# SelennLamson/AntsRL

Hardware: AMD Instinct MI355X
Metric: ant-steps/sec (ants x envs x steps/s), 256^2 grid (higher is better)
Workload: dtype f64 ant kinematics / f32 grids

## Files before the change

### antsrl_amd/_lib.py

```python
from __future__ import annotations

import ctypes as C
import os

from .config import AntsCfg, AntsGen, AntsInit

LIB_PATH = os.environ.get("ANTSRL_LIB") or os.path.join(os.path.dirname(os.path.abspath(__file__)), "lib",
                                                        "libantsrl_hip.so")

EXPORTS = ("antsrl_abi_version", "antsrl_cfg_size", "antsrl_last_error", "antsrl_workspace_bytes", "antsrl_create",
           "antsrl_destroy", "antsrl_reset", "antsrl_generate", "antsrl_step", "antsrl_observe", "antsrl_update", "antsrl_flush",
           "antsrl_step_update", "antsrl_set_timing_events", "antsrl_set_activation", "antsrl_policy_mlp", "antsrl_read_state", "antsrl_state_bytes",
           "antsrl_set_obs_format", "antsrl_query", "antsrl_bench_copy", "antsrl_set_inloop_policy", "antsrl_set_obs_row_stride", "antsrl_mem_alloc", "antsrl_mem_free",
           "antsrl_mem_trim", "antsrl_mem_stats", "antsrl_update_phase",
           "antsrl_perceptive_field", "antsrl_memnet_packed_bytes", "antsrl_memnet_pack", "antsrl_policy_memory",
           "antsrl_memtrain_sizes", "antsrl_memtrain_init", "antsrl_memtrain_unpack", "antsrl_memtrain_copy",
           "antsrl_memtrain_grad", "antsrl_memtrain_apply", "antsrl_memnet_packed_bytes_ex", "antsrl_memnet_pack_ex",
           "antsrl_policy_memory_ex", "antsrl_agent_select", "antsrl_replay_record_pre", "antsrl_replay_record_post",
           "antsrl_policy_memory_tiles", "antsrl_agent_plan", "antsrl_agent_select_actions",
           "antsrl_replay_record_pre_plain", "antsrl_replay_record_post_plain", "antsrl_lintrain_sizes",
           "antsrl_lintrain_grad", "antsrl_lintrain_apply", "antsrl_lintrain_step", "antsrl_exptrain_sizes",
           "antsrl_exptrain_grad", "antsrl_exptrain_apply", "antsrl_exptrain_step", "antsrl_rework_collapsed_bytes",
           "antsrl_rework_collapse", "antsrl_policy_rework", "antsrl_reworktrain_sizes", "antsrl_reworktrain_grad",
           "antsrl_reworktrain_apply", "antsrl_reworktrain_step", "antsrl_policy_rework_select")

_lib = None


class AntsMemNetShape(C.Structure):
    _fields_ = [(n, C.c_int32) for n in ("n_features", "agent_dim", "mem_size", "h1", "h2", "h3", "n_rot", "n_ph")]


class AntsReworkShape(C.Structure):
    _fields_ = [(n, C.c_int32) for n in ("n_features", "agent_dim", "g1", "g2", "g3", "r1", "r2", "r3", "p1", "n_rot", "n_ph")]


class AntsRecordSpec(C.Structure):
    _fields_ = [(n, C.c_int32) for n in ("n_envs", "n_ants", "env_id_base", "n_features", "agent_dim", "mem_size", "n_rot",
                                         "obs_format", "obs_pitch", "reserved")] + [
        (n, C.c_int64) for n in ("K", "head", "max_len")] + [(n, C.c_uint64) for n in ("seed", "step")]


class AntsrlError(RuntimeError):
    pass


def load() -> C.CDLL:
    global _lib
    if _lib is not None:
        return _lib
    if not os.path.exists(LIB_PATH):
        raise AntsrlError(
            "libantsrl_hip.so is missing (%s): build it with `python -m antsrl_amd.build` "
            "(hipcc, gfx950).  There is no CPU fallback." % LIB_PATH)
    import torch
    lib = C.CDLL(LIB_PATH)
    vp, i32 = C.c_void_p, C.c_int
    lib.antsrl_abi_version.restype = i32
    lib.antsrl_last_error.restype = C.c_char_p
    lib.antsrl_workspace_bytes.argtypes = [C.POINTER(AntsCfg), C.POINTER(C.c_size_t)]
    lib.antsrl_create.argtypes = [C.POINTER(AntsCfg), vp, C.c_size_t, C.POINTER(vp)]
    lib.antsrl_destroy.argtypes = [vp]
    lib.antsrl_destroy.restype = None
    lib.antsrl_reset.argtypes = [vp, C.POINTER(AntsInit), vp]
    lib.antsrl_generate.argtypes = [vp, C.POINTER(AntsGen), C.c_uint64, vp]
    lib.antsrl_step.argtypes = [vp, vp, vp, vp, vp, vp, vp, vp]
    lib.antsrl_observe.argtypes = [vp, vp, vp, vp, vp]
    lib.antsrl_update.argtypes = [vp, vp, vp]
    lib.antsrl_flush.argtypes = [vp, vp]
    lib.antsrl_update_phase.argtypes = [vp, i32, vp, vp]
    lib.antsrl_perceptive_field.argtypes = [vp, vp, vp]
    lib.antsrl_step_update.argtypes = [vp, vp, vp, vp, vp, vp, vp, vp, vp]
    lib.antsrl_set_timing_events.argtypes = [vp, C.POINTER(vp)]
    lib.antsrl_set_activation.argtypes = [vp, vp, C.c_double, vp]
    lib.antsrl_policy_mlp.argtypes = [vp, vp, vp, C.c_int64, C.c_int32, vp, vp, vp, vp, vp, vp, vp, vp, vp, vp]
    lib.antsrl_read_state.argtypes = [vp, i32, vp, vp]
    lib.antsrl_state_bytes.argtypes = [vp, i32, C.POINTER(C.c_size_t)]
    lib.antsrl_query.argtypes = [vp, i32, C.POINTER(C.c_longlong)]
    lib.antsrl_set_inloop_policy.argtypes = [vp, i32] + [vp] * 9
    lib.antsrl_bench_copy.argtypes = [vp, vp, C.c_size_t, vp]
    lib.antsrl_set_obs_row_stride.argtypes = [vp, i32]
    lib.antsrl_mem_alloc.argtypes = [C.c_size_t, i32, C.POINTER(vp)]
    lib.antsrl_mem_free.argtypes = [vp]
    lib.antsrl_mem_trim.argtypes = []
    lib.antsrl_mem_stats.argtypes = [C.POINTER(C.c_size_t)] * 4
    lib.antsrl_memnet_packed_bytes.argtypes = [C.POINTER(AntsMemNetShape), C.POINTER(C.c_size_t)]
    lib.antsrl_memnet_pack.argtypes = [C.POINTER(AntsMemNetShape), C.POINTER(vp), vp, vp]
    lib.antsrl_policy_memory.argtypes = [C.POINTER(AntsMemNetShape), vp, vp, i32, vp, vp, C.c_int64, vp, vp, vp, vp, vp]
    lib.antsrl_memnet_packed_bytes_ex.argtypes = [C.POINTER(AntsMemNetShape), i32, C.POINTER(C.c_size_t)]
    lib.antsrl_memnet_pack_ex.argtypes = [C.POINTER(AntsMemNetShape), i32, C.POINTER(vp), vp, vp]
    lib.antsrl_policy_memory_ex.argtypes = [C.POINTER(AntsMemNetShape), i32, vp, vp, i32, vp, vp, C.c_int64, vp, vp, vp,
                                            vp, vp]
    lib.antsrl_policy_memory_tiles.argtypes = [C.POINTER(AntsMemNetShape), i32, vp, vp, i32, vp, vp, C.c_int64, vp, vp, vp,
                                               vp, vp, vp, vp]
    sz = C.POINTER(C.c_size_t)
    lib.antsrl_memtrain_sizes.argtypes = [C.POINTER(AntsMemNetShape), C.c_int64, sz, sz, sz, sz]
    lib.antsrl_memtrain_init.argtypes = [C.POINTER(AntsMemNetShape), C.POINTER(vp), vp, vp]
    lib.antsrl_memtrain_unpack.argtypes = [C.POINTER(AntsMemNetShape), vp, C.POINTER(vp), vp]
    lib.antsrl_memtrain_copy.argtypes = [C.POINTER(AntsMemNetShape), vp, vp, vp]
    lib.antsrl_memtrain_grad.argtypes = [C.POINTER(AntsMemNetShape), vp, vp, vp, vp, vp, vp, vp, vp, vp, vp, C.c_int64,
                                         C.c_float, vp, vp, vp, vp]
    lib.antsrl_memtrain_apply.argtypes = [C.POINTER(AntsMemNetShape), vp, vp, C.c_int64, C.c_double, C.c_double,
                                          C.c_double, C.c_double, vp]
    lib.antsrl_agent_select.argtypes = [C.c_uint64, C.c_uint64, i32, i32, i32, C.c_double, i32, i32, i32, vp, vp, vp, vp,
                                        vp, vp]
    lib.antsrl_agent_plan.argtypes = [C.c_uint64, C.c_uint64, i32, i32, i32, C.c_double, vp, vp, vp]
    lib.antsrl_replay_record_pre.argtypes = [C.POINTER(AntsRecordSpec)] + [vp] * 9
    lib.antsrl_replay_record_post.argtypes = [C.POINTER(AntsRecordSpec)] + [vp] * 10
    lib.antsrl_agent_select_actions.argtypes = [C.c_uint64, C.c_uint64, i32, i32, i32, C.c_double, i32, i32, vp, vp, vp, vp]
    lib.antsrl_replay_record_pre_plain.argtypes = [C.POINTER(AntsRecordSpec)] + [vp] * 8
    lib.antsrl_replay_record_post_plain.argtypes = [C.POINTER(AntsRecordSpec)] + [vp] * 9
    lib.antsrl_lintrain_sizes.argtypes = [i32, C.c_int64, sz, sz, C.POINTER(C.c_int32)]
    lib.antsrl_lintrain_grad.argtypes = [i32] + [vp] * 11 + [C.c_int64, vp, C.c_int64, C.c_float, vp, vp, vp, vp]
    lib.antsrl_lintrain_apply.argtypes = [vp, vp, vp, vp, C.c_int64, C.c_double, C.c_double, C.c_double, C.c_double, vp]
    lib.antsrl_lintrain_step.argtypes = [i32] + [vp] * 13 + [C.c_int64, vp, C.c_int64, C.c_float, C.c_int64, C.c_double,
                                                             C.c_double, C.c_double, C.c_double, vp, vp, vp, vp]
    lib.antsrl_exptrain_sizes.argtypes = [i32, C.c_int64, sz, sz, C.POINTER(C.c_int32)]
    lib.antsrl_exptrain_grad.argtypes = [i32] + [vp] * 9 + [C.c_int64, vp, C.c_int64, C.c_float, vp, vp, vp, vp]
    lib.antsrl_exptrain_apply.argtypes = [i32, vp, vp, vp, vp, C.c_int64, C.c_double, C.c_double, C.c_double, C.c_double, vp]
    lib.antsrl_exptrain_step.argtypes = [i32] + [vp] * 11 + [C.c_int64, vp, C.c_int64, C.c_float, C.c_int64, C.c_double,
                                                             C.c_double, C.c_double, C.c_double, vp, vp, vp, vp]
    lib.antsrl_rework_collapsed_bytes.argtypes = [C.POINTER(AntsReworkShape), sz]
    lib.antsrl_rework_collapse.argtypes = [C.POINTER(AntsReworkShape), C.POINTER(vp), vp, vp]
    lib.antsrl_policy_rework.argtypes = [C.POINTER(AntsReworkShape), vp, vp, i32, vp, C.c_int64, vp, vp, vp, vp]
    rs = C.POINTER(AntsReworkShape)
    lib.antsrl_policy_rework_select.argtypes = [rs, vp, vp, i32, vp, C.c_uint64, C.c_uint64, i32, i32, i32, C.c_double, vp, vp,
                                                vp, vp, vp]
    lib.antsrl_reworktrain_sizes.argtypes = [rs, C.c_int64, sz, sz, C.POINTER(C.c_int32)]
    lib.antsrl_reworktrain_grad.argtypes = [rs] + [vp] * 9 + [C.c_int64, vp, C.c_int64, C.c_float, vp, vp, vp, vp]
    lib.antsrl_reworktrain_apply.argtypes = [rs, vp, vp, vp, vp, C.c_int64, C.c_double, C.c_double, C.c_double, C.c_double, vp]
    lib.antsrl_reworktrain_step.argtypes = [rs] + [vp] * 11 + [C.c_int64, vp, C.c_int64, C.c_float, C.c_int64, C.c_double,
                                                               C.c_double, C.c_double, C.c_double, vp, vp, vp, vp]
    for name in EXPORTS:
        getattr(lib, name)
    lib.antsrl_cfg_size.restype = C.c_size_t
    from .config import ABI_VERSION
    if lib.antsrl_abi_version() != ABI_VERSION:
        raise AntsrlError("ABI version mismatch: library %d, binding %d" % (lib.antsrl_abi_version(), ABI_VERSION))
    if lib.antsrl_cfg_size() != C.sizeof(AntsCfg):
        raise AntsrlError("AntsCfg layout mismatch: library %d bytes, binding %d" % (
            lib.antsrl_cfg_size(), C.sizeof(AntsCfg)))
    _lib = lib
    return lib


def hip_runtime() -> C.CDLL:
    load()
    for line in open("/proc/self/maps"):
        path = line.split()[-1]
        if "libamdhip64" in path:
            return C.CDLL(path)
    raise AntsrlError("no libamdhip64 mapped in this process")


def check(rc: int, what: str = "antsrl") -> None:
    if rc != 0:
        msg = load().antsrl_last_error().decode("utf-8", "replace")
        raise AntsrlError("%s failed (%d): %s" % (what, rc, msg))


def ptr(t):
    return None if t is None else C.c_void_p(t.data_ptr())


def stream(device):
    import torch
    return C.c_void_p(torch.cuda.current_stream(device).cuda_stream)


class HipEvents:

    def __init__(self, n):
        self.hip = hip_runtime()
        self.ev = []
        for _ in range(n):
            e = C.c_void_p()
            rc = self.hip.hipEventCreate(C.byref(e))
            assert rc == 0, "hipEventCreate failed: %d" % rc
            self.ev.append(e)

    def elapsed_ms(self, a, b):
        ms = C.c_float()
        rc = self.hip.hipEventElapsedTime(C.byref(ms), self.ev[a], self.ev[b])
        assert rc == 0, "hipEventElapsedTime failed: %d" % rc
        return ms.value

    def destroy(self):
        for e in self.ev:
            self.hip.hipEventDestroy(e)
```

### antsrl_amd/batched.py

```python
from __future__ import annotations

import ctypes as C
from typing import Dict, Optional

import numpy as np
import torch

from . import _lib
from . import config as cfgmod
from . import vmm
from .config import AntsCfg, AntsInit

_STATE_DTYPES = {
    cfgmod.S_ANTS_XYT: torch.float64, cfgmod.S_PREV_XY: torch.float64, cfgmod.S_HOLDING: torch.float32,
    cfgmod.S_MANDIBLES: torch.uint8, cfgmod.S_ACTIVATION: torch.float32, cfgmod.S_PHERO: torch.float32,
    cfgmod.S_FOOD: torch.float32, cfgmod.S_EXPLORED: torch.uint8, cfgmod.S_ANTHILL_FOOD: torch.float64,
    cfgmod.S_ROCK_CENTERS: torch.float64, cfgmod.S_TIMESTEP: torch.int32, cfgmod.S_REWARD_STATE: torch.uint8,
    cfgmod.S_WALLS: torch.uint8, cfgmod.S_ANTHILL_AREA: torch.uint8, cfgmod.S_SEED: torch.float32,
    cfgmod.S_ANTHILL_XYR: torch.int32, cfgmod.S_ROCK_RW: torch.float64,
    cfgmod.S_PHERO_C0: torch.float32, cfgmod.S_PHERO_C1: torch.float32, cfgmod.S_PHERO_C2: torch.float32,
    cfgmod.S_PHERO_C3: torch.float32,
}


import contextlib

_NULL_CTX = contextlib.nullcontext()
_RAW_STREAM = getattr(torch._C, "_cuda_getCurrentRawStream", None)


def _ptr(t: Optional[torch.Tensor]):
    return None if t is None else C.c_void_p(t.data_ptr())


def placement_levels_seen(times) -> bool:
    ok = [t for t in times if t < 1.25 * min(times)]
    return max(ok) >= 1.06 * min(ok)


class BatchedAntsEnv:
    def __init__(self, cfg: AntsCfg, device: Optional[torch.device] = None, obs_dtype: torch.dtype = torch.float32,
                 obs_row_stride=None, pieced_memory: bool = True):
        if obs_dtype not in (torch.float32, torch.bfloat16):
            raise ValueError("obs_dtype must be torch.float32 or torch.bfloat16")
        if not torch.cuda.is_available():
            raise _lib.AntsrlError("BatchedAntsEnv needs an MI355X (torch.cuda.is_available() is False); "
                                   "there is no CPU fallback")
        self.lib = _lib.load()
        self.cfg = cfg.copy()
        self.device = torch.device(device if device is not None else "cuda:%d" % torch.cuda.current_device())
        self._dev_index = self.device.index if self.device.index is not None else torch.cuda.current_device()
        need = C.c_size_t()
        _lib.check(self.lib.antsrl_workspace_bytes(C.byref(self.cfg), C.byref(need)), "workspace_bytes")
        self.workspace_bytes = need.value
        with torch.cuda.device(self.device):
            big = (lambda n: vmm.empty_u8(n, self.device)) if pieced_memory else (lambda n: torch.empty(n, dtype=torch.uint8, device=self.device))
            self._pieced = bool(pieced_memory)
            self._h = None
            self._make_handle(torch.empty(need.value + 256, dtype=torch.uint8, device=self.device))
            E, N, P, K = cfg.n_envs, cfg.n_ants, cfg.pside, cfg.n_channels
            esz = 4 if obs_dtype == torch.float32 else 2
            row = P * P * K
            if obs_row_stride not in (None, "line"):
                raise ValueError("obs_row_stride must be None or 'line'")
            pitch = row if obs_row_stride is None else (row * esz + 127) // 128 * 128 // esz
            sizes = [("agent_state", E * N * 2 * 4), ("reward", E * N * 4), ("done", E), ("obs", E * N * pitch * esz)]
            offs, total = {}, 0
            for name, nbytes in sizes:
                offs[name] = total
                total += (nbytes + 255) // 256 * 256
            self._out_sizes, self._out_offs, self._out_total, self._small_bytes = sizes, offs, total, offs["obs"]
            self._obs_dtype, self._obs_pitch_row = obs_dtype, (pitch, row)
            if obs_dtype == torch.bfloat16:
                _lib.check(self.lib.antsrl_set_obs_format(self._h, 1), "set_obs_format")
            if pitch != row:
                _lib.check(self.lib.antsrl_set_obs_row_stride(self._h, pitch), "set_obs_row_stride")
            self.obs_row_pitch = pitch
            self._bind_outputs(big(total + 256).zero_())
        self._keep = None
        self._loaded = None
        self._host_out = None
        self._host_act = None
        self._act_event = None

    def __del__(self):
        h = getattr(self, "_h", None)
        if h:
            self.lib.antsrl_destroy(h)
            self._h = None

    def _bind_outputs(self, flat: torch.Tensor) -> None:
        c = self.cfg
        E, N, P, K = c.n_envs, c.n_ants, c.pside, c.n_channels
        sizes, offs, total = self._out_sizes, self._out_offs, self._out_total
        pitch, row = self._obs_pitch_row
        base = (-flat.data_ptr()) % 256
        self._out_flat = flat[base:base + total]

        def piece(name, nbytes, dtype, shape):
            return self._out_flat[offs[name]:offs[name] + nbytes].view(dtype).view(shape)
        if pitch == row:
            self.obs = piece("obs", sizes[3][1], self._obs_dtype, (E, N, P, P, K))
            self.obs_padded = None
        else:
            self.obs_padded = piece("obs", sizes[3][1], self._obs_dtype, (E, N, pitch))
            self.obs = self.obs_padded[..., :row].unflatten(-1, (P, P, K))
        self.agent_state = piece("agent_state", sizes[0][1], torch.float32, (E, N, 2))
        self.reward = piece("reward", sizes[1][1], torch.float32, (E, N))
        self.done = piece("done", sizes[2][1], torch.uint8, (E,))
        self._host_out = None

    def _make_handle(self, ws: torch.Tensor) -> None:
        if getattr(self, "_h", None):
            self.lib.antsrl_destroy(self._h)
        self._ws = ws
        self._ws_ptr = ws.data_ptr() + (-ws.data_ptr()) % 256
        self._h = C.c_void_p()
        _lib.check(self.lib.antsrl_create(C.byref(self.cfg), C.c_void_p(self._ws_ptr), self.workspace_bytes, C.byref(self._h)), "create")
        if getattr(self, "_obs_dtype", torch.float32) == torch.bfloat16:
            _lib.check(self.lib.antsrl_set_obs_format(self._h, 1), "set_obs_format")
        pitch, row = getattr(self, "_obs_pitch_row", (0, 0))
        if pitch != row:
            _lib.check(self.lib.antsrl_set_obs_row_stride(self._h, pitch), "set_obs_row_stride")

    def tune_placement(self, age: int = 150, steps: int = 30, verbose: bool = False, extra_outputs: int = 4,
                       walk_spacers: int = 3, spacer_gib: float = 24.0, force_walk: bool = False):
        if self._out_total < vmm.SMALL_BYTES:
            return None
        if self._loaded:
            raise _lib.AntsrlError("tune_placement() must run right after construction: this handle has already been %s" % self._loaded)
        c = self.cfg
        E, N = c.n_envs, c.n_ants
        dev = self.device

        def torch_u8(n):
            return torch.empty(n, dtype=torch.uint8, device=dev)
        with torch.cuda.device(dev):
            g = torch.Generator(device=dev)
            g.manual_seed(7)
            rot = torch.randint(-1, 2, (4, E, N), generator=g, device=dev, dtype=torch.int8)
            ph = torch.randint(0, 3, (4, E, N), generator=g, device=dev, dtype=torch.int8) if c.n_phero == 2 else [None] * 4
            e0, e1 = torch.cuda.Event(enable_timing=True), torch.cuda.Event(enable_timing=True)

            def scratch_episode():
                self.generate(cfgmod.make_gen(), episode_seed=0x7A11)
                for t in range(age):
                    self.step_update(rot[t % 4], ph[t % 4], None)

            NEV, PSTEPS = cfgmod.TIMING_EVENTS, 8
            evs = _lib.HipEvents(NEV * PSTEPS)
            prc_times = []

            def measure():
                for t in range(4):
                    self.step_update(rot[t % 4], ph[t % 4], None)
                e0.record()
                for t in range(steps):
                    self.step_update(rot[t % 4], ph[t % 4], None)
                e1.record()
                for t in range(PSTEPS):
                    self.set_timing_events([evs.ev[NEV * t + i].value for i in range(NEV)])
                    self.step_update(rot[t % 4], ph[t % 4], None)
                torch.cuda.current_stream(dev).synchronize()
                prc_times.append(float(np.mean([evs.elapsed_ms(NEV * t + 2, NEV * t + 3) for t in range(PSTEPS)])))
                return e0.elapsed_time(e1) / steps
            own_ws, own_out = self._ws, self._out_flat
            n_ws, n_out = self.workspace_bytes + 256, self._out_total + 256
            pairs, times = [], []
            for ws_kind in ("own", "other"):
                if ws_kind == "other":
                    self._make_handle(vmm.empty_u8(n_ws, dev))
                scratch_episode()
                for out_kind in ("own", "other"):
                    if out_kind == "other":
                        self._bind_outputs((torch_u8(n_out) if self._pieced else vmm.empty_u8(n_out, dev)).zero_())
                    elif ws_kind == "other":
                        self._bind_outputs(own_out)
                    pairs.append((self._ws, self._out_flat))
                    times.append(measure())
            labels = ["ws torch / out %s" % ("pieced" if self._pieced else "torch"),
                      "ws torch / out %s" % ("torch" if self._pieced else "pieced"),
                      "ws pieced / out %s" % ("pieced" if self._pieced else "torch"),
                      "ws pieced / out %s" % ("torch" if self._pieced else "pieced")]
            if extra_outputs > 0 and self._pieced:
                self._make_handle(own_ws)
                scratch_episode()
                for k in range(int(extra_outputs)):
                    self._bind_outputs(vmm.empty_u8(n_out, dev).zero_())
                    pairs.append((self._ws, self._out_flat))
                    times.append(measure())
                    labels.append("ws torch / out pieced (draw %d)" % (k + 2))
            spacers = []
            walked = 0
            both_levels = placement_levels_seen
            while self._pieced and walked < int(walk_spacers) and (force_walk or not both_levels(prc_times)):
                free_b = torch.cuda.mem_get_info(dev)[0]
                want = int(min(spacer_gib * 2 ** 30, free_b / 5))
                if want < (4 << 30):
                    break
                try:
                    spacers.append(torch_u8(want))
                    spacers.append(vmm.empty_u8(want, dev))
                except (RuntimeError, _lib.AntsrlError):
                    break
                walked += 1
                depth = sum(x.numel() for x in spacers) / 2 ** 30
                if self._ws.data_ptr() != own_ws.data_ptr():
                    self._make_handle(own_ws)
                scratch_episode()
                for kind, mk in (("pieced", lambda: vmm.empty_u8(n_out, dev)), ("torch", lambda: torch_u8(n_out))):
                    self._bind_outputs(mk().zero_())
                    pairs.append((self._ws, self._out_flat))
                    times.append(measure())
                    labels.append("ws torch / out %s (walk %d: +%.0f GiB)" % (kind, walked, depth))
                self._make_handle(torch_u8(n_ws))
                scratch_episode()
                self._bind_outputs(own_out)
                pairs.append((self._ws, self._out_flat))
                times.append(measure())
                labels.append("ws torch (walk %d: +%.0f GiB) / out %s" % (walked, depth, "pieced" if self._pieced else "torch"))
            best = min(range(len(times)), key=prc_times.__getitem__)
            evs.destroy()
            if verbose:
                print("tune_placement: ms/step per (workspace, outputs) pair %s -> %d" % (["%.4f" % t for t in times], best))
            ws, out = pairs[best]
            del pairs, spacers
            if ws.data_ptr() != self._ws.data_ptr():
                self._make_handle(ws)
            self._bind_outputs(out)
            if walked:
                vmm.trim()
            torch.cuda.empty_cache()
            self._out_flat.zero_()
            del own_ws, own_out, ws, out
        self.placement_trials = dict(ms_per_step=[round(t, 5) for t in times], observation_kernel_ms=[round(t, 5) for t in prc_times],
                                     chosen=best, pairs=labels, both_levels_seen=bool(both_levels(prc_times)), walk_steps=walked)
        self._loaded = None
        return times

    @property
    def _obs_buf(self):
        return self.obs if self.obs_padded is None else self.obs_padded

    def _stream(self):
        if _RAW_STREAM is not None:
            return C.c_void_p(_RAW_STREAM(self._dev_index))
        return C.c_void_p(torch.cuda.current_stream(self.device).cuda_stream)

    def _on_device(self):
        return _NULL_CTX if torch.cuda.current_device() == self._dev_index else torch.cuda.device(self.device)

    def _dev(self, a, dtype, shape=None):
        if a is None:
            return None
        t = torch.as_tensor(np.ascontiguousarray(a) if isinstance(a, np.ndarray) else a)
        t = t.to(device=self.device, dtype=dtype).contiguous()
        if shape is not None:
            assert tuple(t.shape) == tuple(shape), "expected shape %s, got %s" % (shape, tuple(t.shape))
        return t

    def reset(self, init: Dict[str, object]) -> None:
        c = self.cfg
        E, N, W, H, Cn, R = c.n_envs, c.n_ants, c.w, c.h, c.n_phero, c.n_rocks
        t = dict(
            ants_xyt=self._dev(init["ants_xyt"], torch.float64, (E, N, 3)),
            seed=self._dev(init["seed"], torch.float64, (E, N)),
            walls=self._dev(init["walls"], torch.uint8, (E, W, H)),
            food=self._dev(init["food"], torch.float32, (E, W, H)),
            anthill_xyr=self._dev(init["anthill_xyr"], torch.int32, (E, 3)),
            rocks=self._dev(init.get("rocks"), torch.float64, (E, R, 4)) if R > 0 else None,
            phero=self._dev(init.get("phero"), torch.float32, (E, Cn, W, H)),
        )
        ai = AntsInit(*[None if t[k] is None else t[k].data_ptr()
                        for k in ("ants_xyt", "seed", "walls", "food", "anthill_xyr", "rocks", "phero")])
        with torch.cuda.device(self.device):
            _lib.check(self.lib.antsrl_reset(self._h, C.byref(ai), self._stream()), "reset")
        self._loaded = "reset"
        self._keep = t

    def generate(self, gen=None, episode_seed: int = 0, walls=None) -> None:
        g = gen if gen is not None else cfgmod.make_gen()
        if walls is not None:
            c = self.cfg
            self._gen_walls = self._dev(np.asarray(walls).astype(np.uint8) if not torch.is_tensor(walls) else walls,
                                        torch.uint8, (c.n_envs, c.w, c.h))
            g.walls_input = self._gen_walls.data_ptr()
        with torch.cuda.device(self.device):
            _lib.check(self.lib.antsrl_generate(self._h, C.byref(g), int(episode_seed), self._stream()), "generate")
        self._loaded = "given an episode (generate)"

    def _actions(self, rotation, phero):
        c = self.cfg
        if isinstance(rotation, np.ndarray) and isinstance(phero, np.ndarray):
            n = c.n_envs * c.n_ants
            if self._host_act is None:
                self._host_act = torch.empty((2, c.n_envs, c.n_ants), dtype=torch.int8, pin_memory=True)
                self._dev_act = torch.empty((2, c.n_envs, c.n_ants), dtype=torch.int8, device=self.device)
                self._act_event = torch.cuda.Event()
            else:
                self._act_event.synchronize()
            assert rotation.size == n and phero.size == n, "expected %d actions per array" % n
            h = self._host_act.numpy()
            h[0] = self._integral(rotation, "rotation").reshape(c.n_envs, c.n_ants)
            h[1] = self._integral(phero, "pheromone").reshape(c.n_envs, c.n_ants)
            with torch.cuda.device(self.device):
                self._dev_act.copy_(self._host_act, non_blocking=True)
                self._act_event.record()
            return self._dev_act[0], self._dev_act[1]
        rot = self._dev(self._integral(rotation, "rotation"), torch.int8, (c.n_envs, c.n_ants))
        ph = self._dev(self._integral(phero, "pheromone"), torch.int8, (c.n_envs, c.n_ants))
        return rot, ph

    validate_actions = True

    def _integral(self, a, what):
        if a is None:
            return None
        if torch.is_tensor(a):
            if a.dtype == torch.int8 or a.numel() == 0:
                return a
            if self.validate_actions:
                fl = a.is_floating_point()
                frac = (a != a.round()).any() if fl else torch.zeros((), dtype=torch.bool, device=a.device)
                lo, hi, bad = torch.stack([a.min().to(torch.float64), a.max().to(torch.float64), frac.to(torch.float64)]).tolist()
                if bad:
                    raise ValueError("%s actions must be whole numbers (the kernels take them as int8)" % what)
                if lo < -128 or hi > 127:
                    raise ValueError("%s actions out of the int8 range" % what)
            return a.to(torch.int8) if a.is_floating_point() else a
        arr = np.asarray(a)
        if arr.dtype.kind == "f":
            if not np.array_equal(arr, np.rint(arr)):
                raise ValueError("%s actions must be whole numbers (the kernels take them as int8)" % what)
            arr = arr.astype(np.int64)
        if arr.size and (arr.min() < -128 or arr.max() > 127):
            raise ValueError("%s actions out of the int8 range" % what)
        return arr

    def outputs_to_host(self, want_obs: bool = True):
        if self.obs.dtype != torch.float32 and want_obs:
            raise _lib.AntsrlError("outputs_to_host: bfloat16 observations have no numpy dtype; use the device tensors")
        base, o = self._out_flat.data_ptr(), self._out_offs
        if any(t.data_ptr() != base + o[k] for k, t in (("obs", self._obs_buf), ("agent_state", self.agent_state),
                                                         ("reward", self.reward), ("done", self.done))):
            return (self.obs.cpu().numpy() if want_obs else None, self.agent_state.cpu().numpy(),
                    self.reward.cpu().numpy(), self.done.cpu().numpy())
        if self._host_out is None:
            self._host_out = torch.empty((self._out_flat.numel(),), dtype=torch.uint8, pin_memory=True)
        n = self._out_flat.numel() if want_obs else self._small_bytes
        with torch.cuda.device(self.device):
            self._host_out[:n].copy_(self._out_flat[:n], non_blocking=True)
            torch.cuda.current_stream(self.device).synchronize()
        hb, o = self._host_out.numpy(), self._out_offs

        def piece(name, t):
            nb = t.numel() * t.element_size()
            return hb[o[name]:o[name] + nb].view(np.float32 if t.dtype == torch.float32 else np.uint8).reshape(tuple(t.shape)).copy()
        obs_h = None
        if want_obs:
            obs_h = piece("obs", self._obs_buf)
            if self.obs_padded is not None:
                c = self.cfg
                obs_h = np.ascontiguousarray(obs_h[..., :c.pside * c.pside * c.n_channels]).reshape(tuple(self.obs.shape))
        return (obs_h, piece("agent_state", self.agent_state),
                piece("reward", self.reward), piece("done", self.done))

    def step(self, rotation, phero, want_obs: bool = True):
        rot, ph = self._actions(rotation, phero)
        with self._on_device():
            _lib.check(self.lib.antsrl_step(self._h, _ptr(rot), _ptr(ph), _ptr(self._obs_buf if want_obs else None),
                                            _ptr(self.agent_state), _ptr(self.reward), _ptr(self.done),
                                            self._stream()), "step")
        return self.obs, self.agent_state, self.reward, self.done

    def observe(self, want_obs: bool = True):
        with self._on_device():
            _lib.check(self.lib.antsrl_observe(self._h, _ptr(self._obs_buf if want_obs else None),
                                               _ptr(self.agent_state), _ptr(self.reward), self._stream()),
                       "observe")
        return self.obs, self.agent_state, self.reward

    def update(self, wall_jitter=None) -> None:
        c = self.cfg
        j = self._dev(wall_jitter, torch.float64, (c.n_envs, c.n_ants))
        with self._on_device():
            _lib.check(self.lib.antsrl_update(self._h, _ptr(j), self._stream()), "update")

    def update_phase(self, phase: int, wall_jitter=None) -> None:
        c = self.cfg
        j = self._dev(wall_jitter, torch.float64, (c.n_envs, c.n_ants)) if phase == cfgmod.PHASE_WALLS else None
        with self._on_device():
            _lib.check(self.lib.antsrl_update_phase(self._h, int(phase), _ptr(j), self._stream()), "update_phase")

    def flush(self) -> None:
        with self._on_device():
            _lib.check(self.lib.antsrl_flush(self._h, self._stream()), "flush")

    def step_update(self, rotation, phero, wall_jitter=None, want_obs: bool = True):
        c = self.cfg
        rot, ph = self._actions(rotation, phero)
        j = self._dev(wall_jitter, torch.float64, (c.n_envs, c.n_ants))
        with self._on_device():
            _lib.check(self.lib.antsrl_step_update(self._h, _ptr(rot), _ptr(ph), _ptr(j),
                                                   _ptr(self._obs_buf if want_obs else None), _ptr(self.agent_state),
                                                   _ptr(self.reward), _ptr(self.done), self._stream()),
                       "step_update")
        return self.obs, self.agent_state, self.reward, self.done

    def set_timing_events(self, events) -> None:
        if events is None:
            _lib.check(self.lib.antsrl_set_timing_events(self._h, None), "set_timing_events")
        else:
            n = cfgmod.TIMING_EVENTS
            assert len(events) == n, "antsrl_set_timing_events takes %d events" % n
            arr = (C.c_void_p * n)(*[C.c_void_p(int(e)) for e in events])
            _lib.check(self.lib.antsrl_set_timing_events(self._h, arr), "set_timing_events")

    def query(self, what: int) -> int:
        v = C.c_longlong()
        _lib.check(self.lib.antsrl_query(self._h, int(what), C.byref(v)), "query")
        return int(v.value)

    def set_activation(self, act, new_deposit_strength: float = 0.0) -> None:
        c = self.cfg
        a = self._dev(act, torch.float32, (c.n_envs, c.n_ants, c.n_phero))
        with torch.cuda.device(self.device):
            _lib.check(self.lib.antsrl_set_activation(self._h, _ptr(a), float(new_deposit_strength),
                                                      self._stream()), "set_activation")
        self._loaded = "given an activation matrix"

    def perceptive_field(self) -> torch.Tensor:
        c = self.cfg
        out = torch.empty((c.n_envs, c.w, c.h), dtype=torch.uint8, device=self.device)
        with self._on_device():
            _lib.check(self.lib.antsrl_perceptive_field(self._h, _ptr(out), self._stream()), "perceptive_field")
        return out.to(torch.bool)

    def read_state(self, which: int) -> torch.Tensor:
        c = self.cfg
        E, N, W, H, Cn, R = c.n_envs, c.n_ants, c.w, c.h, c.n_phero, c.n_rocks
        shapes = {
            cfgmod.S_ANTS_XYT: (E, N, 3), cfgmod.S_PREV_XY: (E, N, 2), cfgmod.S_HOLDING: (E, N),
            cfgmod.S_MANDIBLES: (E, N), cfgmod.S_ACTIVATION: (E, N, Cn), cfgmod.S_PHERO: (E, Cn, W, H),
            cfgmod.S_FOOD: (E, W, H), cfgmod.S_EXPLORED: (E, W, H), cfgmod.S_ANTHILL_FOOD: (E,),
            cfgmod.S_ROCK_CENTERS: (E, R, 2), cfgmod.S_TIMESTEP: (E,), cfgmod.S_REWARD_STATE: (E, N),
            cfgmod.S_WALLS: (E, W, H), cfgmod.S_ANTHILL_AREA: (E, W, H), cfgmod.S_SEED: (E, N),
            cfgmod.S_ANTHILL_XYR: (E, 3), cfgmod.S_ROCK_RW: (E, R, 2),
            cfgmod.S_PHERO_C0: (E, W, H), cfgmod.S_PHERO_C1: (E, W, H), cfgmod.S_PHERO_C2: (E, W, H),
            cfgmod.S_PHERO_C3: (E, W, H),
        }
        if cfgmod.S_PHERO_C0 <= which <= cfgmod.S_PHERO_C3 and which - cfgmod.S_PHERO_C0 >= Cn:
            raise _lib.AntsrlError("pheromone channel %d of %d" % (which - cfgmod.S_PHERO_C0, Cn))
        out = torch.empty(shapes[which], dtype=_STATE_DTYPES[which], device=self.device)
        if out.numel():
            with torch.cuda.device(self.device):
                _lib.check(self.lib.antsrl_read_state(self._h, which, _ptr(out), self._stream()), "read_state")
        return out
```

### antsrl_amd/config.py

```python
from __future__ import annotations

import ctypes as C
import math
from typing import Optional, Sequence

import numpy as np

ABI_VERSION = 5
MAX_CHANNELS = 16
MAX_PSIDE = 15
MAX_PCELLS = MAX_PSIDE * MAX_PSIDE
MAX_FILTER_RADIUS = 3
MAX_FILTER_TAPS = 49
MAX_PHERO = 4

CH_ANTS, CH_PHERO, CH_ANTHILL, CH_WALLS, CH_FOOD, CH_ROCKS = range(6)
REWARD_NONE, REWARD_EXPLORATION, REWARD_FOOD, REWARD_ALL = range(4)
PHERO_AUTO, PHERO_EXPLICIT_SWEEP = 0, 1
ACT_AUTO, ACT_CELL_META, ACT_SINGLE_KERNEL = 0, 1, 2
TIMING_EVENTS = 5
Q_CELL_META, Q_SCALED_UNITS, Q_INTERLEAVED, Q_FILTER_SEPARABLE, Q_PERCEIVE_RUN, Q_TIMESTEP, Q_DEFERRED_UPDATE = range(7)

(S_ANTS_XYT, S_PREV_XY, S_HOLDING, S_MANDIBLES, S_ACTIVATION, S_PHERO, S_FOOD, S_EXPLORED,
 S_ANTHILL_FOOD, S_ROCK_CENTERS, S_TIMESTEP, S_REWARD_STATE, S_WALLS, S_ANTHILL_AREA,
 S_SEED, S_ANTHILL_XYR, S_ROCK_RW, S_PHERO_C0, S_PHERO_C1, S_PHERO_C2, S_PHERO_C3) = range(21)


class AntsCfg(C.Structure):
    _fields_ = [
        ("abi_version", C.c_int32),
        ("n_envs", C.c_int32),
        ("n_ants", C.c_int32),
        ("w", C.c_int32),
        ("h", C.c_int32),
        ("n_phero", C.c_int32),
        ("n_rocks", C.c_int32),
        ("max_time", C.c_int32),
        ("perception_radius", C.c_int32),
        ("n_channels", C.c_int32),
        ("channel_kind", C.c_int32 * MAX_CHANNELS),
        ("channel_arg", C.c_int32 * MAX_CHANNELS),
        ("has_mask", C.c_int32),
        ("mask", C.c_uint8 * MAX_PCELLS),
        ("_pad0", C.c_uint8 * 7),
        ("delta", C.c_double),
        ("fwd_delta", C.c_double),
        ("max_speed", C.c_double),
        ("max_rot_speed", C.c_double),
        ("carry_speed_reduction", C.c_double),
        ("backward_speed_reduction", C.c_double),
        ("max_hold", C.c_double),
        ("has_max_val", C.c_int32),
        ("filter_radius", C.c_int32),
        ("phero_max_val", C.c_double),
        ("deposit_strength", C.c_double),
        ("phero_threshold", C.c_double),
        ("filter", C.c_double * MAX_FILTER_TAPS),
        ("reward_kind", C.c_int32),
        ("phero_mode", C.c_int32),
        ("reward_threshold", C.c_double),
        ("fct_explore", C.c_double),
        ("fct_food", C.c_double),
        ("fct_anthill", C.c_double),
        ("fct_explore_holding", C.c_double),
        ("fct_headinganthill", C.c_double),
        ("rng_seed", C.c_uint64),
        ("act_path", C.c_int32),
        ("env_id_base", C.c_int32),
        ("n_envs_total", C.c_int32),
        ("_pad1", C.c_int32),
    ]

    @property
    def pside(self) -> int:
        return 2 * self.perception_radius + 1

    def copy(self) -> "AntsCfg":
        out = AntsCfg()
        C.memmove(C.byref(out), C.byref(self), C.sizeof(AntsCfg))
        return out

    def obs_shape(self):
        p = self.pside
        return (self.n_envs, self.n_ants, p, p, self.n_channels)


class AntsGen(C.Structure):
    _fields_ = [("wall_density", C.c_double), ("n_food_discs", C.c_int32), ("food_rmin", C.c_int32),
                ("food_rmax", C.c_int32), ("auto_reset", C.c_int32), ("wall_kind", C.c_int32),
                ("perlin_octaves", C.c_int32), ("perlin_scale", C.c_double), ("perlin_persistence", C.c_double),
                ("perlin_lacunarity", C.c_double), ("rng_kind", C.c_int32), ("_pad", C.c_int32),
                ("walls_input", C.c_void_p)]


WALLS_BERNOULLI, WALLS_PERLIN, WALLS_INPUT = 0, 1, 2
PHASE_WALLS, PHASE_ROCKS_PHEROMONE, PHASE_ANTS, PHASE_ANTHILL = 0, 1, 2, 3
RNG_COUNTER, RNG_REFERENCE = 0, 1


def make_gen(wall_density=0.05, n_food_discs=20, food_rmin=5, food_rmax=10, auto_reset=False, walls="bernoulli",
             perlin_scale=22.0, perlin_octaves=2, perlin_persistence=0.5, perlin_lacunarity=2.0, rng="counter",
             walls_input_ptr=None) -> AntsGen:
    kind = {"bernoulli": WALLS_BERNOULLI, "perlin": WALLS_PERLIN, "input": WALLS_INPUT}[walls]
    return AntsGen(wall_density, n_food_discs, food_rmin, food_rmax, 1 if auto_reset else 0, kind,
                   int(perlin_octaves), float(perlin_scale), float(perlin_persistence), float(perlin_lacunarity),
                   {"counter": RNG_COUNTER, "reference": RNG_REFERENCE}[rng], 0, walls_input_ptr)


class AntsInit(C.Structure):
    _fields_ = [
        ("ants_xyt", C.c_void_p),
        ("seed", C.c_void_p),
        ("walls", C.c_void_p),
        ("food", C.c_void_p),
        ("anthill_xyr", C.c_void_p),
        ("rocks", C.c_void_p),
        ("phero", C.c_void_p),
    ]


DEFAULT_MASK = np.array([[0, 0, 1, 1, 1, 0, 0],
                         [0, 1, 1, 1, 1, 1, 0],
                         [1, 1, 1, 1, 1, 1, 1],
                         [1, 1, 1, 1, 1, 1, 1],
                         [1, 1, 1, 1, 1, 1, 1],
                         [0, 1, 1, 1, 1, 1, 0],
                         [0, 0, 1, 1, 1, 0, 0]], dtype=np.uint8)


def diffuse_filter(diffuse_factor: float = 0.0, evap_factor: float = 0.001) -> np.ndarray:
    f = np.ones((3, 3)) * diffuse_factor
    f[1, 1] = 1 - 8 * diffuse_factor
    f *= 1 - evap_factor
    return f


def default_channels(n_phero: int, n_rocks: int):
    kinds = [CH_ANTS] + [CH_PHERO] * n_phero + [CH_ANTHILL, CH_WALLS, CH_FOOD]
    args = [0] + list(range(n_phero)) + [0, 0, 0]
    if n_rocks > 0:
        kinds.append(CH_ROCKS)
        args.append(0)
    return kinds, args


def make_cfg(n_envs: int, n_ants: int, w: int, h: int, *, n_phero: int = 2, n_rocks: int = 0,
             max_time: int = 2000, mask: Optional[np.ndarray] = DEFAULT_MASK,
             perception_radius: Optional[int] = None, fwd_delta: float = 4.0, delta: float = 1.1,
             channels: Optional[Sequence] = None,
             max_speed: float = 1.0, max_rot_speed: float = 40 / 180 * np.pi,
             carry_speed_reduction: float = 0.05, backward_speed_reduction: float = 0.5,
             max_hold: float = 5.0, phero_max_val: Optional[float] = 255.0,
             deposit_strength: float = 1.0, phero_threshold: float = 0.01,
             filt: Optional[np.ndarray] = None, reward_kind: int = REWARD_EXPLORATION,
             reward_threshold: float = 1.0, fct_explore: float = 1.0, fct_food: float = 1.0,
             fct_anthill: float = 5.0, fct_explore_holding: float = 0.0,
             fct_headinganthill: float = 1.0, rng_seed: int = 0x5EED,
             phero_mode: int = PHERO_AUTO, act_path: int = ACT_AUTO, env_id_base: int = 0,
             n_envs_total: int = 0) -> AntsCfg:
    c = AntsCfg()
    c.abi_version = ABI_VERSION
    c.n_envs, c.n_ants, c.w, c.h = n_envs, n_ants, w, h
    c.n_phero, c.n_rocks, c.max_time = n_phero, n_rocks, max_time
    if mask is not None:
        mask = np.asarray(mask)
        assert mask.ndim == 2 and mask.shape[0] == mask.shape[1] and mask.shape[0] % 2 == 1
        r = mask.shape[0] // 2 if perception_radius is None else perception_radius
        assert mask.shape[0] == 2 * r + 1
        c.has_mask = 1
        flat = mask.astype(np.uint8).reshape(-1)
        for i, v in enumerate(flat):
            c.mask[i] = int(v)
    else:
        r = 3 if perception_radius is None else perception_radius
        c.has_mask = 0
    assert 2 * r + 1 <= MAX_PSIDE
    c.perception_radius = r
    if channels is None:
        kinds, args = default_channels(n_phero, n_rocks)
    else:
        kinds = [k if isinstance(k, int) else k[0] for k in channels]
        args = [0 if isinstance(k, int) else k[1] for k in channels]
    assert len(kinds) <= MAX_CHANNELS
    c.n_channels = len(kinds)
    for i, (k, a) in enumerate(zip(kinds, args)):
        c.channel_kind[i] = k
        c.channel_arg[i] = a
    c.delta, c.fwd_delta = delta, fwd_delta
    c.max_speed, c.max_rot_speed = max_speed, max_rot_speed
    c.carry_speed_reduction, c.backward_speed_reduction = carry_speed_reduction, backward_speed_reduction
    c.max_hold = max_hold
    c.has_max_val = 0 if phero_max_val is None else 1
    c.phero_max_val = 0.0 if phero_max_val is None else phero_max_val
    c.deposit_strength = deposit_strength
    c.phero_threshold = phero_threshold
    if filt is None:
        filt = diffuse_filter()
    filt = np.asarray(filt, dtype=np.float64)
    assert filt.ndim == 2 and filt.shape[0] == filt.shape[1] and filt.shape[0] % 2 == 1
    fr = filt.shape[0] // 2
    off = filt.copy()
    off[fr, fr] = 0.0
    if not off.any():
        filt = filt[fr:fr + 1, fr:fr + 1]
        fr = 0
    assert fr <= MAX_FILTER_RADIUS
    c.filter_radius = fr
    for i, v in enumerate(filt.reshape(-1)):
        c.filter[i] = float(v)
    c.reward_kind = reward_kind
    c.reward_threshold = reward_threshold
    c.fct_explore, c.fct_food, c.fct_anthill = fct_explore, fct_food, fct_anthill
    c.fct_explore_holding, c.fct_headinganthill = fct_explore_holding, fct_headinganthill
    c.rng_seed = rng_seed
    c.phero_mode = phero_mode
    c.act_path = act_path
    c.env_id_base = env_id_base
    c.n_envs_total = n_envs_total
    return c


def mask_array(cfg: AntsCfg) -> Optional[np.ndarray]:
    if not cfg.has_mask:
        return None
    p = cfg.pside
    return np.array(list(cfg.mask[: p * p]), dtype=bool).reshape(p, p)


__all__ = [n for n in dir() if n.isupper() or n in (
    "AntsCfg", "AntsInit", "AntsGen", "make_gen", "make_cfg", "diffuse_filter", "default_channels", "mask_array")]
_ = math


def uses_scaled_units(cfg: AntsCfg) -> bool:
    return (cfg.phero_mode == PHERO_AUTO and cfg.filter_radius == 0 and 0.5 < cfg.filter[0] <= 1.0
            and cfg.phero_threshold >= 0.0)
```

### antsrl_amd/csrc/antsrl_capi.hip

```cpp
#include <hip/hip_runtime.h>
#include <stdarg.h>
#include <stdio.h>
#include <math.h>
#include <stdlib.h>
#include <string.h>
#include <new>

#include "antsrl_device.h"
#include "antsrl_fail.h"

hipError_t antsrl_launch_act(const KP &p, const int8_t *rot, const int8_t *ph, int cur, float *obs,
                             float *agent_state, float *reward, uint8_t *done, int flags, hipStream_t st);
bool antsrl_act_fits(const KP &p);
bool antsrl_act_needs_hbm_maps(const KP &p);
hipError_t antsrl_launch_sweep(const KP &p, int cur, hipStream_t st);
hipError_t antsrl_launch_update(const KP &p, const double *jitter, int out_buf, hipStream_t st, int phases = 15);
hipError_t antsrl_launch_collect_full(const KP &p, hipStream_t st);
hipError_t antsrl_launch_reset(const KP &p, const AntsInit *in, hipStream_t st);
hipError_t antsrl_launch_set_activation(const KP &p, const float *act, hipStream_t st);
hipError_t antsrl_launch_read_state(const KP &p, int which, int cur, void *dst, hipStream_t st);
hipError_t antsrl_launch_perceptive_field(const KP &p, uint8_t *dst, hipStream_t st);
hipError_t antsrl_launch_generate(const KP &p, const AntsGen &g, uint64_t seed, hipStream_t st);
hipError_t antsrl_launch_phero_wall_clear(const KP &p, hipStream_t st, int buf = 0);
hipError_t antsrl_launch_phero_renorm(const KP &p, hipStream_t st);
bool antsrl_meta_supported(const KP &p);
hipError_t antsrl_launch_move(const KP &p, const int8_t *rot, const int8_t *ph, uint8_t *done, int do_step, uint32_t seq,
                              hipStream_t st);
hipError_t antsrl_launch_perceive(const KP &p, int cur, float *obs, float *agent_state, float *reward, int flags,
                                  uint32_t seq, hipStream_t st, const PolArgs *pol, uint32_t obs_pitch);
bool antsrl_inloop_policy_supported(const KP &p);
hipError_t antsrl_launch_policy_pack(unsigned char *pack, const float *w1, const float *b1, const float *w2, const float *b2,
                                     const float *w3, const float *b3, int F, hipStream_t st);
hipError_t antsrl_launch_meta_rebase(const KP &p, hipStream_t st);
bool antsrl_update_move_supported(const KP &p);
hipError_t antsrl_launch_update_move(const KP &p, int out_buf, double g_dep, double inv_g_dep, const int8_t *rot,
                                     const int8_t *ph, uint8_t *done, uint32_t seq, hipStream_t st, bool with_frames);
int antsrl_perceive_run(const KP &p);
hipError_t antsrl_launch_copy16(void *dst, const void *src, size_t bytes, hipStream_t st);

struct AntsHandle {
    AntsCfg cfg;
    KP p;
    int cur;
    int steps_since_update;
    bool need_full_collect;
    bool is_reset;
    bool episode_over;
    size_t ws_bytes;
    AntsGen gen;
    bool has_gen;
    uint64_t episode_seed;
    int host_timestep;
    long long sweeps;
    bool obs_bf16;
    uint32_t obs_pitch;
    bool need_wall_clear;
    hipEvent_t ev[ANTSRL_TIMING_EVENTS];
    bool ev_armed;
    uint32_t obs_seq;
    PolArgs pol;
    bool pend_update;
    KP pend_p;
    int pend_out_buf;
    int phase_next;
};

static thread_local char g_err[512] = "";

int fail(int code, const char *fmt, ...)
{
    va_list ap;
    va_start(ap, fmt);
    vsnprintf(g_err, sizeof(g_err), fmt, ap);
    va_end(ap);
    return code;
}

int hip_fail(hipError_t e, const char *what)
{
    return fail(ANTSRL_E_DEVICE, "%s: %s", what, hipGetErrorString(e));
}

extern "C" int antsrl_abi_version(void) { return ANTSRL_ABI_VERSION; }
extern "C" size_t antsrl_cfg_size(void) { return sizeof(AntsCfg); }
extern "C" const char *antsrl_last_error(void) { return g_err; }

static void fill_kp(const AntsCfg *c, KP *p);

static int validate(const AntsCfg *c)
{
    if (!c) return fail(ANTSRL_E_INVALID, "cfg is NULL");
    if (c->abi_version != ANTSRL_ABI_VERSION)
        return fail(ANTSRL_E_INVALID, "AntsCfg.abi_version %d != library %d", c->abi_version, ANTSRL_ABI_VERSION);
    if (c->n_envs < 1 || c->n_ants < 1 || c->w < 1 || c->h < 1)
        return fail(ANTSRL_E_INVALID, "n_envs, n_ants, w, h must be >= 1");
    if ((long long)c->w * c->h > (1ll << 30)) return fail(ANTSRL_E_INVALID, "grid too large");
    if (c->n_envs > 65535)
        return fail(ANTSRL_E_INVALID, "n_envs must be <= 65535 per handle (shard larger batches over handles / GPUs)");
    if (c->n_phero < 1 || c->n_phero > ANTSRL_MAX_PHERO)
        return fail(ANTSRL_E_INVALID, "n_phero must be in 1..%d", ANTSRL_MAX_PHERO);
    if (c->n_rocks < 0 || c->n_rocks > 32) return fail(ANTSRL_E_INVALID, "n_rocks must be in 0..32");
    if (c->perception_radius < 0 || 2 * c->perception_radius + 1 > ANTSRL_MAX_PSIDE)
        return fail(ANTSRL_E_INVALID, "perception side must be <= %d", ANTSRL_MAX_PSIDE);
    if (c->n_channels < 1 || c->n_channels > ANTSRL_MAX_CHANNELS)
        return fail(ANTSRL_E_INVALID, "n_channels must be in 1..%d", ANTSRL_MAX_CHANNELS);
    for (int k = 0; k < c->n_channels; ++k) {
        const int kind = c->channel_kind[k];
        if (kind < ANTSRL_CH_ANTS || kind > ANTSRL_CH_ROCKS) return fail(ANTSRL_E_INVALID, "bad channel kind");
        if (kind == ANTSRL_CH_PHERO && (c->channel_arg[k] < 0 || c->channel_arg[k] >= c->n_phero))
            return fail(ANTSRL_E_INVALID, "pheromone channel index out of range");
        if (kind == ANTSRL_CH_PHERO && !c->has_max_val)
            return fail(ANTSRL_E_INVALID, "a perceived pheromone needs max_val (RL_api.py:125 divides by it)");
        if (kind == ANTSRL_CH_ROCKS && c->n_rocks == 0)
            return fail(ANTSRL_E_INVALID, "rocks perceived but n_rocks == 0");
    }
    if (c->filter_radius < 0 || c->filter_radius > ANTSRL_MAX_FILTER_RADIUS)
        return fail(ANTSRL_E_INVALID, "filter_radius must be in 0..%d", ANTSRL_MAX_FILTER_RADIUS);
    if (c->reward_kind < ANTSRL_REWARD_NONE || c->reward_kind > ANTSRL_REWARD_ALL)
        return fail(ANTSRL_E_INVALID, "bad reward_kind");
    if (c->has_max_val && !(c->phero_max_val > 0)) return fail(ANTSRL_E_INVALID, "phero_max_val must be > 0");
    if (c->act_path < ANTSRL_ACT_AUTO || c->act_path > ANTSRL_ACT_SINGLE_KERNEL) return fail(ANTSRL_E_INVALID, "bad act_path");
    if (c->env_id_base < 0 || (long long)c->env_id_base + c->n_envs > 0x7fffffffll)
        return fail(ANTSRL_E_INVALID, "env_id_base must be >= 0 and env_id_base + n_envs must fit 31 bits");
    if (c->n_envs_total != 0 && (long long)c->n_envs_total < (long long)c->env_id_base + c->n_envs)
        return fail(ANTSRL_E_INVALID, "n_envs_total %d < env_id_base + n_envs = %lld (0 = that sum)", c->n_envs_total,
                    (long long)c->env_id_base + c->n_envs);
    if (c->act_path == ANTSRL_ACT_CELL_META) {
        KP kp;
        fill_kp(c, &kp);
        if (!kp.meta)
            return fail(ANTSRL_E_UNSUPPORTED, "ANTSRL_ACT_CELL_META needs 2 pheromone channels, the generator's channel order "
                                              "([Ants, Phero0, Phero1, Anthill, Walls, Food(, Rocks)]), a perception of 128..368 values "
                                              "per ant over at most 64 cells, and at most 4096 ants per env");
    }
    return ANTSRL_OK;
}

static bool use_scaled(const AntsCfg *c)
{
    return c->phero_mode == ANTSRL_PHERO_AUTO && c->filter_radius == 0 && c->filter[0] > 0.5 &&
           c->filter[0] <= 1.0 && c->phero_threshold >= 0.0;
}

static bool use_interleaved(const AntsCfg *c)
{
    return use_scaled(c) && c->n_phero == 2;
}

static size_t carve(const AntsCfg *c, DState *s, unsigned char *base)
{
    const size_t E = c->n_envs, N = c->n_ants, G = (size_t)c->w * c->h, Cn = c->n_phero, R = c->n_rocks;
    const size_t words = (G + 31) / 32;
    size_t off = 0;
    auto take = [&](size_t bytes) -> unsigned char * {
        unsigned char *ptr = base ? base + off : nullptr;
        off = (off + bytes + 255) / 256 * 256;
        return ptr;
    };
    KP kp;
    fill_kp(c, &kp);
    DState d;
    d.x = (double *)take(8 * E * N); d.y = (double *)take(8 * E * N); d.theta = (double *)take(8 * E * N);
    d.prev_x = (double *)take(8 * E * N); d.prev_y = (double *)take(8 * E * N);
    d.prev_dist = (double *)take(8 * E * N);
    d.holding = (float *)take(4 * E * N); d.seed = (float *)take(4 * E * N);
    d.prev_holding = (float *)take(4 * E * N);
    d.activation = (float *)take(4 * E * N * Cn);
    d.mandibles = (uint8_t *)take(E * N); d.reward_state = (uint8_t *)take(E * N);
    d.dirty_cell = (int32_t *)take(4 * E * N);
    d.walldep_cell = (int32_t *)take(4 * E * N);
    if (use_interleaved(c)) {
        d.phero[0] = d.phero[1] = (float *)take(16 * E * G);
        d.food = d.phero[0] ? d.phero[0] + 2 : nullptr;
    } else {
        d.phero[0] = (float *)take(4 * E * G * Cn);
        d.phero[1] = use_scaled(c) ? d.phero[0] : (float *)take(4 * E * G * Cn);
        d.food = (float *)take(4 * E * G * (size_t)kp.fs);
    }
    d.walls_bits = (uint32_t *)take(4 * E * words); d.area_bits = (uint32_t *)take(4 * E * words);
    d.explored_bits = (uint32_t *)take(4 * E * words);
    d.big_pres = d.big_old = nullptr;
    if (!kp.meta && antsrl_act_needs_hbm_maps(kp)) {
        d.big_pres = (uint32_t *)take(4 * E * words);
        d.big_old = (uint32_t *)take(4 * E * words);
    }
    d.primed_cur = kp.meta ? (uint8_t *)take(E) : nullptr;
    d.frames = kp.meta ? (AntFrame *)take(sizeof(AntFrame) * E * N) : nullptr;
    d.anthill_xyr = (int32_t *)take(4 * E * 3);
    d.anthill_food = (double *)take(8 * E);
    d.rock_cx = (double *)take(8 * E * (R ? R : 1)); d.rock_cy = (double *)take(8 * E * (R ? R : 1));
    d.rock_r = (double *)take(8 * E * (R ? R : 1)); d.rock_w = (double *)take(8 * E * (R ? R : 1));
    d.timestep = (int32_t *)take(4 * E);
    d.reward_primed = (uint8_t *)take(E);
    d.gen_discs = (int32_t *)take(4 * E * ANTSRL_MAX_FOOD_DISCS * 3);
    d.gen_perlin = (int32_t *)take(4 * E * 2);
    d.pol_pack = (unsigned char *)take(ANTSRL_POL_PACK_BYTES);
    if (s) *s = d;
    return off;
}

static void fill_kp(const AntsCfg *c, KP *p)
{
    memset(p, 0, sizeof(*p));
    p->E = c->n_envs; p->N = c->n_ants; p->W = c->w; p->H = c->h; p->C = c->n_phero; p->R = c->n_rocks;
    p->K = c->n_channels; p->r = c->perception_radius; p->P = 2 * p->r + 1; p->PP = p->P * p->P;
    p->words = (int)(((size_t)c->w * c->h + 31) / 32);
    int ht = 64;
    while (ht < 2 * c->n_ants) ht <<= 1;
    p->HT = ht;
    p->has_mask = c->has_mask; p->has_max_val = c->has_max_val; p->reward_kind = c->reward_kind;
    p->max_time = c->max_time; p->filter_radius = c->filter_radius;
    p->explore_on = c->reward_kind == ANTSRL_REWARD_EXPLORATION ||
                    (c->reward_kind == ANTSRL_REWARD_ALL &&
                     (c->fct_explore != 0.0 || c->fct_explore_holding != 0.0));
    for (int k = 0; k < ANTSRL_MAX_CHANNELS; ++k) {
        p->ch_kind[k] = c->channel_kind[k];
        p->ch_arg[k] = c->channel_arg[k];
    }
    p->mand_first = p->mand_last = 0;
    for (int k = 0; k < c->n_channels; ++k) {
        const int op = c->channel_kind[k] == ANTSRL_CH_FOOD ? 1 : c->channel_kind[k] == ANTSRL_CH_ANTHILL ? 2 : 0;
        if (op && op != p->mand_last) {
            p->mand_first = p->mand_last;
            p->mand_last = op;
        }
    }
    memcpy(p->mask, c->mask, ANTSRL_MAX_PCELLS);
    p->delta = c->delta; p->fwd_delta = c->fwd_delta; p->max_speed = c->max_speed;
    p->max_rot_speed = c->max_rot_speed; p->carry = c->carry_speed_reduction;
    p->backward = c->backward_speed_reduction; p->max_hold = c->max_hold;
    p->max_val = c->phero_max_val; p->deposit_strength = c->deposit_strength;
    p->threshold = c->phero_threshold; p->reward_threshold = c->reward_threshold;
    p->fct_explore = c->fct_explore; p->fct_food = c->fct_food; p->fct_anthill = c->fct_anthill;
    p->fct_explore_holding = c->fct_explore_holding; p->fct_heading = c->fct_headinganthill;
    memcpy(p->filter, c->filter, sizeof(p->filter));
    {
        const int S = 2 * c->filter_radius + 1;
        for (int a = 0; a < S; ++a)
            for (int b = 0; b < S; ++b) {
                const double f = c->filter[a * S + b];
                const float hi = (float)f;
                p->ftap[(b * S + a) * 2 + 0] = hi;
                p->ftap[(b * S + a) * 2 + 1] = (float)(f - (double)hi);
            }
    }
    {
        const int S = 2 * c->filter_radius + 1;
        p->filter_sep = 0;
        if (S > 1) {
            int i0 = 0, j0 = 0;
            double big = 0.0;
            for (int a = 0; a < S; ++a)
                for (int b = 0; b < S; ++b)
                    if (fabs(c->filter[a * S + b]) > big) { big = fabs(c->filter[a * S + b]); i0 = a; j0 = b; }
            bool sep = big > 0.0;
            double u[2 * ANTSRL_MAX_FILTER_RADIUS + 1], v[2 * ANTSRL_MAX_FILTER_RADIUS + 1];
            for (int a = 0; a < S && sep; ++a) u[a] = c->filter[a * S + j0];
            for (int b = 0; b < S && sep; ++b) v[b] = c->filter[i0 * S + b] / c->filter[i0 * S + j0];
            for (int a = 0; a < S && sep; ++a)
                for (int b = 0; b < S; ++b)
                    if (fabs(u[a] * v[b] - c->filter[a * S + b]) > 1e-15 * big) sep = false;
            if (sep) {
                p->filter_sep = 1;
                for (int k = 0; k < S; ++k) {
                    const float uh = (float)u[k], vh = (float)v[k];
                    p->fsep_u[2 * k] = uh; p->fsep_u[2 * k + 1] = (float)(u[k] - (double)uh);
                    p->fsep_v[2 * k] = vh; p->fsep_v[2 * k + 1] = (float)(v[k] - (double)vh);
                }
            }
        }
    }
    p->rng_seed = c->rng_seed;
    p->env_id_base = (uint32_t)c->env_id_base;
    p->scaled = use_scaled(c) ? 1 : 0;
    p->ps = use_interleaved(c) ? 4 : c->n_phero;
    p->fs = use_interleaved(c) ? 4 : 1;
    p->g_now = p->g_dep = p->inv_g_dep = 1.0;
    p->meta = antsrl_meta_supported(*p) && c->act_path != ANTSRL_ACT_SINGLE_KERNEL ? 1 : 0;
    if (p->meta && p->fs == 1) p->fs = 2;
    p->tiled = (p->meta && p->ps == 4 && p->fs == 4 && (c->w & 1) == 0 && (c->h & 3) == 0) ? 1 : 0;
    p->ftile = (p->meta && p->fs == 2 && (c->w & 3) == 0 && (c->h & 3) == 0) ? 1 : 0;
}

static void set_decay(AntsHandle *h)
{
    if (!h->p.scaled) return;
    const double f0 = h->cfg.filter[0];
    h->p.g_now = pow(f0, (double)h->sweeps);
    h->p.g_dep = pow(f0, (double)(h->sweeps + 1));
    h->p.inv_g_dep = 1.0 / h->p.g_dep;
}

extern "C" int antsrl_workspace_bytes(const AntsCfg *cfg, size_t *bytes)
{
    int rc = validate(cfg);
    if (rc) return rc;
    if (!bytes) return fail(ANTSRL_E_INVALID, "bytes is NULL");
    *bytes = carve(cfg, nullptr, nullptr);
    return ANTSRL_OK;
}

extern "C" int antsrl_create(const AntsCfg *cfg, void *workspace, size_t workspace_bytes, AntsHandle **out)
{
    int rc = validate(cfg);
    if (rc) return rc;
    if (!out) return fail(ANTSRL_E_INVALID, "out is NULL");
    if (!workspace) return fail(ANTSRL_E_INVALID, "workspace is NULL");
    if (((uintptr_t)workspace & 255) != 0) return fail(ANTSRL_E_INVALID, "workspace must be 256-byte aligned");
    const size_t need = carve(cfg, nullptr, nullptr);
    if (workspace_bytes < need)
        return fail(ANTSRL_E_NOMEM, "workspace too small: %zu < %zu bytes", workspace_bytes, need);
    AntsHandle *h = new (std::nothrow) AntsHandle();
    if (!h) return fail(ANTSRL_E_NOMEM, "out of host memory");
    h->cfg = *cfg;
    fill_kp(cfg, &h->p);
    carve(cfg, &h->p.s, (unsigned char *)workspace);
    h->cur = 0; h->steps_since_update = 0; h->need_full_collect = true; h->is_reset = false; h->episode_over = false; h->pend_update = false;
    h->phase_next = 0;
    h->pol = PolArgs{};
    h->sweeps = 0; h->need_wall_clear = false;
    h->has_gen = false; h->episode_seed = 0; h->host_timestep = 1; h->obs_bf16 = false; h->obs_pitch = 0;
    h->ws_bytes = need;
    h->ev_armed = false;
    h->obs_seq = 0;
    if (!h->p.meta && !antsrl_act_fits(h->p)) {
        delete h;
        return fail(ANTSRL_E_UNSUPPORTED,
                    "%d ants with a %dx%d perception need more than 160 KiB of LDS per workgroup "
                    "(per-ant frames, the collision hash and the row staging are kept in LDS)", cfg->n_ants,
                    2 * cfg->perception_radius + 1, 2 * cfg->perception_radius + 1);
    }
    *out = h;
    return ANTSRL_OK;
}

extern "C" void antsrl_destroy(AntsHandle *h) { delete h; }

extern "C" int antsrl_reset(AntsHandle *h, const AntsInit *init, void *stream)
{
    if (!h || !init) return fail(ANTSRL_E_INVALID, "NULL handle or init");
    if (!init->ants_xyt || !init->seed || !init->walls || !init->food || !init->anthill_xyr)
        return fail(ANTSRL_E_INVALID, "AntsInit: ants_xyt, seed, walls, food, anthill_xyr are required");
    if (h->p.R > 0 && !init->rocks) return fail(ANTSRL_E_INVALID, "AntsInit.rocks is NULL but n_rocks > 0");
    h->pend_update = false;
    h->phase_next = 0;
    hipError_t e = antsrl_launch_reset(h->p, init, (hipStream_t)stream);
    if (e != hipSuccess) return hip_fail(e, "reset");
    h->p.deposit_strength = h->cfg.deposit_strength;
    h->cur = 0; h->steps_since_update = 0; h->need_full_collect = true; h->is_reset = true; h->episode_over = false;
    h->sweeps = 0; h->need_wall_clear = h->p.scaled && init->phero != nullptr;
    h->host_timestep = 1; h->obs_seq = 0;
    set_decay(h);
    return ANTSRL_OK;
}

static int check_gen_seed(const AntsHandle *h, const AntsGen &g, uint64_t seed)
{
    const uint64_t top = (uint64_t)h->p.env_id_base + (uint64_t)h->p.E;
    const uint64_t lim = 0xFFFFFFFFull / 5u;
    if (g.rng_kind == ANTSRL_RNG_REFERENCE && (top > lim || seed > lim - top))
        return fail(ANTSRL_E_INVALID, "ANTSRL_RNG_REFERENCE: (episode_seed + env_id_base + n_envs) * 5 must stay below 2^32 (np.random.seed)");
    return ANTSRL_OK;
}

static int do_generate(AntsHandle *h, uint64_t seed, hipStream_t st)
{
    int rc = check_gen_seed(h, h->gen, seed);
    if (rc) return rc;
    h->pend_update = false;
    h->phase_next = 0;
    hipError_t e = antsrl_launch_generate(h->p, h->gen, seed, st);
    if (e != hipSuccess) return hip_fail(e, "generate");
    h->p.deposit_strength = h->cfg.deposit_strength;
    h->cur = 0; h->steps_since_update = 0; h->need_full_collect = true; h->is_reset = true; h->episode_over = false;
    h->sweeps = 0; h->need_wall_clear = false; h->host_timestep = 1; h->obs_seq = 0;
    h->episode_seed = seed;
    set_decay(h);
    return ANTSRL_OK;
}

extern "C" int antsrl_generate(AntsHandle *h, const AntsGen *gen, uint64_t episode_seed, void *stream)
{
    if (!h || !gen) return fail(ANTSRL_E_INVALID, "NULL handle or gen");
    if (gen->n_food_discs < 0 || gen->n_food_discs > ANTSRL_MAX_FOOD_DISCS)
        return fail(ANTSRL_E_INVALID, "n_food_discs must be in 0..%d", ANTSRL_MAX_FOOD_DISCS);
    if (gen->food_rmin < 0 || gen->food_rmax < gen->food_rmin) return fail(ANTSRL_E_INVALID, "bad food radii");
    if (gen->wall_kind == ANTSRL_WALLS_BERNOULLI) {
        if (!(gen->wall_density >= 0.0 && gen->wall_density <= 1.0)) return fail(ANTSRL_E_INVALID, "bad wall_density");
    } else if (gen->wall_kind == ANTSRL_WALLS_PERLIN) {
        if (!(gen->wall_density >= -1.0 && gen->wall_density <= 1.0) || gen->perlin_octaves < 1 || gen->perlin_octaves > 8 ||
            !(gen->perlin_scale > 0.0) || !(gen->perlin_persistence > 0.0) || !(gen->perlin_lacunarity > 0.0))
            return fail(ANTSRL_E_INVALID, "bad Perlin wall parameters (density in [-1, 1], 1..8 octaves, positive "
                                          "scale / persistence / lacunarity)");
    } else if (gen->wall_kind == ANTSRL_WALLS_INPUT) {
        if (!gen->walls_input) return fail(ANTSRL_E_INVALID, "ANTSRL_WALLS_INPUT needs AntsGen.walls_input");
    } else {
        return fail(ANTSRL_E_INVALID, "bad wall_kind %d", gen->wall_kind);
    }
    if (gen->rng_kind != ANTSRL_RNG_COUNTER && gen->rng_kind != ANTSRL_RNG_REFERENCE)
        return fail(ANTSRL_E_INVALID, "bad rng_kind %d", gen->rng_kind);
    if (gen->rng_kind == ANTSRL_RNG_REFERENCE) {
        if (gen->wall_kind == ANTSRL_WALLS_BERNOULLI && gen->wall_density != 0.0)
            return fail(ANTSRL_E_UNSUPPORTED, "the reference has no Bernoulli walls generator: with ANTSRL_RNG_REFERENCE use "
                                              "ANTSRL_WALLS_PERLIN, ANTSRL_WALLS_INPUT or wall_density 0");
    }
    int rc = check_gen_seed(h, *gen, episode_seed);
    if (rc) return rc;
    h->gen = *gen;
    h->has_gen = true;
    return do_generate(h, episode_seed, (hipStream_t)stream);
}

static int bf16_unsupported()
{
    return fail(ANTSRL_E_UNSUPPORTED, "bfloat16 observations on the single-kernel path (k_act) need 2 pheromone channels, the "
                                      "generator's channel order ([Ants, Phero0, Phero1, Anthill, Walls, Food(, Rocks)]), a perception of "
                                      "at most 64 cells and a grid whose bit maps fit LDS (up to ~600k cells); the cell-meta path "
                                      "(ANTSRL_Q_CELL_META) has no grid limit");
}

extern "C" int antsrl_set_obs_format(AntsHandle *h, int format)
{
    if (!h) return fail(ANTSRL_E_INVALID, "NULL handle");
    if (format != ANTSRL_OBS_F32 && format != ANTSRL_OBS_BF16) return fail(ANTSRL_E_INVALID, "bad observation format %d", format);
    if ((format == ANTSRL_OBS_BF16) != h->obs_bf16) h->obs_pitch = 0;
    h->obs_bf16 = format == ANTSRL_OBS_BF16;
    if (!h->obs_bf16) h->pol = PolArgs{};
    return ANTSRL_OK;
}

extern "C" int antsrl_set_obs_row_stride(AntsHandle *h, int32_t stride_elems)
{
    if (!h) return fail(ANTSRL_E_INVALID, "NULL handle");
    const int32_t row = h->p.PP * h->p.K, esz = h->obs_bf16 ? 2 : 4;
    if (stride_elems == 0 || stride_elems == row) {
        h->obs_pitch = 0;
        return ANTSRL_OK;
    }
    if (stride_elems < row || ((long long)stride_elems * esz) % 128 != 0 || stride_elems > row + 128 / esz)
        return fail(ANTSRL_E_INVALID, "obs row stride %d: 0 (dense) or the row's %d elements rounded up to whole 128-byte lines (%d)",
                    stride_elems, row, (row * esz + 127) / 128 * 128 / esz);
    if (!h->p.meta) return fail(ANTSRL_E_UNSUPPORTED, "antsrl_set_obs_row_stride needs the cell-meta path (ANTSRL_Q_CELL_META)");
    if (h->pol.pack)
        return fail(ANTSRL_E_UNSUPPORTED, "a padded observation row stride and the in-loop policy exclude each other (the net reads a "
                                          "dense tile image): switch the policy off first (antsrl_set_inloop_policy with w1 == NULL)");
    h->obs_pitch = (uint32_t)stride_elems;
    return ANTSRL_OK;
}

static int flush_pending(AntsHandle *h, hipStream_t st)
{
    if (!h->pend_update) return ANTSRL_OK;
    h->pend_update = false;
    hipError_t e = antsrl_launch_update(h->pend_p, nullptr, h->pend_out_buf, st);
    if (e != hipSuccess) return hip_fail(e, "deferred update");
    return ANTSRL_OK;
}

static int not_reset(const AntsHandle *h)
{
    if (h->episode_over)
        return fail(ANTSRL_E_INVALID, "the episode is over and its auto-reset was refused (episode seed past np.random.seed's 32 bits): "
                                      "call antsrl_reset or antsrl_generate");
    return fail(ANTSRL_E_INVALID, "antsrl_reset has not been called on this handle");
}

static int mid_update(const AntsHandle *h)
{
    return fail(ANTSRL_E_INVALID, "an Environment.update is in progress (antsrl_update_phase %d of 4 is next): finish it first", h->phase_next);
}

static int meta_observe(AntsHandle *h, const int8_t *rot, const int8_t *ph, float *obs, float *agent_state,
                        float *reward, uint8_t *done, bool stepping, hipStream_t st, bool timed)
{
    hipError_t e;
    if (obs && h->obs_pitch != 0 && h->obs_pitch != (uint32_t)(h->p.PP * h->p.K) && h->pol.pack && h->obs_bf16)
        return fail(ANTSRL_E_UNSUPPORTED, "a padded observation row stride and the in-loop policy exclude each other");
    if (h->obs_seq >= META_NEVER - 2) {
        e = antsrl_launch_meta_rebase(h->p, st);
        if (e != hipSuccess) return hip_fail(e, "explored-stamp rebase");
        h->obs_seq = 0;
    }
    h->obs_seq++;
    bool frames = false;
    if (h->pend_update && stepping) {
        h->pend_update = false;
        frames = h->pol.pack != nullptr;
        e = antsrl_launch_update_move(h->p, h->pend_out_buf, h->pend_p.g_dep, h->pend_p.inv_g_dep, rot, ph, done, h->obs_seq, st, frames);
        if (e != hipSuccess) return hip_fail(e, "update + move");
    } else {
        int rc = flush_pending(h, st);
        if (rc) return rc;
        e = antsrl_launch_move(h->p, rot, ph, done, stepping ? 1 : 0, h->obs_seq, st);
        if (e != hipSuccess) return hip_fail(e, "move");
    }
    if (timed) (void)hipEventRecord(h->ev[2], st);
    e = antsrl_launch_perceive(h->p, h->cur, obs, agent_state, reward,
                               (stepping ? ACT_STEP : 0) | (obs ? ACT_HAS_OBS : 0) | (frames ? ACT_FRAMES : 0) |
                                   ((obs || h->pol.pack) && h->obs_bf16 ? ACT_OBS_BF16 : 0),
                               h->obs_seq, st, &h->pol, h->obs_pitch);
    if (e == hipErrorNotSupported)
        return fail(ANTSRL_E_UNSUPPORTED, "a padded observation row stride and the in-loop policy exclude each other (the net reads a dense tile image)");
    if (e != hipSuccess) return hip_fail(e, "perceive");
    return ANTSRL_OK;
}

static int do_step(AntsHandle *h, const int8_t *rot, const int8_t *ph, float *obs, float *agent_state,
                   float *reward, uint8_t *done, hipStream_t st, bool timed = false)
{
    if (ph && h->p.C != 2)
        return fail(ANTSRL_E_INVALID, "pheromone actions need exactly 2 pheromone channels (ants.py:89-96)");
    if (h->steps_since_update > 0) h->need_full_collect = true;
    if (h->p.meta) {
        int rc = meta_observe(h, rot, ph, obs, agent_state, reward, done, true, st, timed);
        if (rc) return rc;
        h->steps_since_update++;
        return ANTSRL_OK;
    }
    if (obs && h->obs_pitch) return fail(ANTSRL_E_UNSUPPORTED, "antsrl_set_obs_row_stride needs the cell-meta path (ANTSRL_Q_CELL_META)");
    if (timed) (void)hipEventRecord(h->ev[2], st);
    hipError_t e = antsrl_launch_act(h->p, rot, ph, h->cur, obs, agent_state, reward, done,
                                     ACT_STEP | (obs ? ACT_HAS_OBS : 0) | (obs && h->obs_bf16 ? ACT_OBS_BF16 : 0), st);
    if (e == hipErrorNotSupported) return bf16_unsupported();
    if (e != hipSuccess) return hip_fail(e, "step");
    h->steps_since_update++;
    return ANTSRL_OK;
}

static int do_update(AntsHandle *h, const double *jitter, hipStream_t st, bool sweep_done, bool may_defer)
{
    hipError_t e;
    int frc = flush_pending(h, st);
    if (frc) return frc;
    if (h->p.scaled) {
        if (h->p.g_dep < 1e-20) {
            e = antsrl_launch_phero_renorm(h->p, st);
            if (e != hipSuccess) return hip_fail(e, "pheromone renorm");
            h->sweeps = 0;
            set_decay(h);
        }
        if (h->need_wall_clear) {
            e = antsrl_launch_phero_wall_clear(h->p, st);
            if (e != hipSuccess) return hip_fail(e, "pheromone wall clear");
            h->need_wall_clear = false;
        }
    } else if (!sweep_done) {
        e = antsrl_launch_sweep(h->p, h->cur, st);
        if (e != hipSuccess) return hip_fail(e, "pheromone sweep");
    }
    if (may_defer && !jitter && !h->need_full_collect && antsrl_update_move_supported(h->p)) {
        h->pend_update = true;
        h->pend_p = h->p;
        h->pend_out_buf = h->p.scaled ? 0 : h->cur ^ 1;
    } else {
        e = antsrl_launch_update(h->p, jitter, h->p.scaled ? 0 : h->cur ^ 1, st);
        if (e != hipSuccess) return hip_fail(e, "update");
    }
    if (h->p.scaled) {
        h->sweeps++;
        set_decay(h);
    }
    if (h->need_full_collect) {
        e = antsrl_launch_collect_full(h->p, st);
        if (e != hipSuccess) return hip_fail(e, "anthill collect");
        h->need_full_collect = false;
    }
    if (!h->p.scaled) h->cur ^= 1;
    h->steps_since_update = 0;
    h->host_timestep++;
    return ANTSRL_OK;
}

extern "C" int antsrl_step(AntsHandle *h, const int8_t *rotation, const int8_t *phero, float *obs,
                           float *agent_state, float *reward, uint8_t *done, void *stream)
{
    if (!h) return fail(ANTSRL_E_INVALID, "NULL handle");
    if (!h->is_reset) return not_reset(h);
    if (h->phase_next) return mid_update(h);
    if (!agent_state || !reward || !done) return fail(ANTSRL_E_INVALID, "agent_state, reward, done are required");
    return do_step(h, rotation, phero, obs, agent_state, reward, done, (hipStream_t)stream);
}

extern "C" int antsrl_observe(AntsHandle *h, float *obs, float *agent_state, float *reward, void *stream)
{
    if (!h) return fail(ANTSRL_E_INVALID, "NULL handle");
    if (!h->is_reset) return not_reset(h);
    if (h->phase_next) return mid_update(h);
    if (h->p.meta)
        return meta_observe(h, nullptr, nullptr, obs, agent_state, reward, nullptr, false, (hipStream_t)stream, false);
    if (obs && h->obs_pitch) return fail(ANTSRL_E_UNSUPPORTED, "antsrl_set_obs_row_stride needs the cell-meta path (ANTSRL_Q_CELL_META)");
    hipError_t e = antsrl_launch_act(h->p, nullptr, nullptr, h->cur, obs, agent_state, reward, nullptr,
                                     obs ? ACT_HAS_OBS | (h->obs_bf16 ? ACT_OBS_BF16 : 0) : 0, (hipStream_t)stream);
    if (e == hipErrorNotSupported) return bf16_unsupported();
    if (e != hipSuccess) return hip_fail(e, "observe");
    return ANTSRL_OK;
}

extern "C" int antsrl_update(AntsHandle *h, const double *wall_jitter, void *stream)
{
    if (!h) return fail(ANTSRL_E_INVALID, "NULL handle");
    if (!h->is_reset) return not_reset(h);
    if (h->phase_next) return mid_update(h);
    return do_update(h, wall_jitter, (hipStream_t)stream, false, true);
}

extern "C" int antsrl_update_phase(AntsHandle *h, int phase, const double *wall_jitter, void *stream)
{
    if (!h) return fail(ANTSRL_E_INVALID, "NULL handle");
    if (!h->is_reset) return not_reset(h);
    if (phase < ANTSRL_PHASE_WALLS || phase > ANTSRL_PHASE_ANTHILL) return fail(ANTSRL_E_INVALID, "bad phase %d", phase);
    if (phase != h->phase_next)
        return fail(ANTSRL_E_INVALID, "antsrl_update_phase: phase %d is next, got %d (WALLS, ROCKS_PHEROMONE, ANTS, ANTHILL in order)", h->phase_next, phase);
    hipStream_t st = (hipStream_t)stream;
    hipError_t e;
    if (phase == ANTSRL_PHASE_WALLS) {
        int frc = flush_pending(h, st);
        if (frc) return frc;
        if (h->p.scaled) {
            if (h->p.g_dep < 1e-20) {
                e = antsrl_launch_phero_renorm(h->p, st);
                if (e != hipSuccess) return hip_fail(e, "pheromone renorm");
                h->sweeps = 0;
                set_decay(h);
            }
            if (h->need_wall_clear) {
                e = antsrl_launch_phero_wall_clear(h->p, st);
                if (e != hipSuccess) return hip_fail(e, "pheromone wall clear");
                h->need_wall_clear = false;
            }
        } else {
            e = antsrl_launch_phero_wall_clear(h->p, st, h->cur);
            if (e != hipSuccess) return hip_fail(e, "pheromone wall clear");
        }
        e = antsrl_launch_update(h->p, wall_jitter, h->p.scaled ? 0 : h->cur, st, 1 );
        if (e != hipSuccess) return hip_fail(e, "update: walls");
    } else if (phase == ANTSRL_PHASE_ROCKS_PHEROMONE) {
        e = antsrl_launch_update(h->p, nullptr, h->p.scaled ? 0 : h->cur, st, 2 );
        if (e != hipSuccess) return hip_fail(e, "update: rocks");
        if (h->p.scaled) {
            h->sweeps++;
            set_decay(h);
        } else {
            e = antsrl_launch_sweep(h->p, h->cur, st);
            if (e != hipSuccess) return hip_fail(e, "pheromone sweep");
            h->cur ^= 1;
        }
    } else if (phase == ANTSRL_PHASE_ANTS) {
        KP kp = h->p;
        if (kp.scaled) {
            kp.g_dep = kp.g_now;
            kp.inv_g_dep = 1.0 / kp.g_dep;
        }
        e = antsrl_launch_update(kp, nullptr, kp.scaled ? 0 : h->cur, st, 4 );
        if (e != hipSuccess) return hip_fail(e, "update: ants");
    } else {
        e = antsrl_launch_update(h->p, nullptr, h->p.scaled ? 0 : h->cur, st, 8 );
        if (e != hipSuccess) return hip_fail(e, "update: anthill");
        if (h->need_full_collect) {
            e = antsrl_launch_collect_full(h->p, st);
            if (e != hipSuccess) return hip_fail(e, "anthill collect");
            h->need_full_collect = false;
        }
        h->steps_since_update = 0;
        h->host_timestep++;
    }
    h->phase_next = (phase + 1) % 4;
    return ANTSRL_OK;
}

extern "C" int antsrl_flush(AntsHandle *h, void *stream)
{
    if (!h) return fail(ANTSRL_E_INVALID, "NULL handle");
    return flush_pending(h, (hipStream_t)stream);
}

extern "C" int antsrl_step_update(AntsHandle *h, const int8_t *rotation, const int8_t *phero,
                                  const double *wall_jitter, float *obs, float *agent_state, float *reward,
                                  uint8_t *done, void *stream)
{
    if (!h) return fail(ANTSRL_E_INVALID, "NULL handle");
    if (!h->is_reset) return not_reset(h);
    if (h->phase_next) return mid_update(h);
    if (!agent_state || !reward || !done) return fail(ANTSRL_E_INVALID, "agent_state, reward, done are required");
    hipStream_t st = (hipStream_t)stream;
    const bool timed = h->ev_armed;
    h->ev_armed = false;
    if (timed) (void)hipEventRecord(h->ev[0], st);
    const bool sweep_late = !h->p.scaled && h->pend_update;
    if (!h->p.scaled && !sweep_late) {
        hipError_t e = antsrl_launch_sweep(h->p, h->cur, st);
        if (e != hipSuccess) return hip_fail(e, "pheromone sweep");
    }
    if (timed) (void)hipEventRecord(h->ev[1], st);
    int rc = do_step(h, rotation, phero, obs, agent_state, reward, done, st, timed);
    if (rc) return rc;
    if (timed) (void)hipEventRecord(h->ev[3], st);
    if (sweep_late) {
        hipError_t e = antsrl_launch_sweep(h->p, h->cur, st);
        if (e != hipSuccess) return hip_fail(e, "pheromone sweep");
    }
    const bool was_done = h->host_timestep == h->cfg.max_time;
    const bool regen = was_done && h->has_gen && h->gen.auto_reset;
    rc = do_update(h, wall_jitter, st, true, !regen);
    if (timed) (void)hipEventRecord(h->ev[4], st);
    if (rc == ANTSRL_OK && regen) {
        const uint64_t total = h->cfg.n_envs_total ? (uint64_t)h->cfg.n_envs_total : (uint64_t)h->p.env_id_base + (uint64_t)h->p.E;
        rc = do_generate(h, h->episode_seed + (h->gen.rng_kind == ANTSRL_RNG_REFERENCE ? total : 1u), st);
        if (rc != ANTSRL_OK) {
            h->is_reset = false;
            h->episode_over = true;
        }
    }
    return rc;
}

extern "C" int antsrl_query(const AntsHandle *h, int what, long long *value)
{
    if (!h || !value) return fail(ANTSRL_E_INVALID, "NULL handle or value");
    switch (what) {
    case ANTSRL_Q_CELL_META: *value = h->p.meta; break;
    case ANTSRL_Q_SCALED_UNITS: *value = h->p.scaled; break;
    case ANTSRL_Q_INTERLEAVED: *value = h->p.ps == 4 && h->p.fs == 4; break;
    case ANTSRL_Q_FILTER_SEPARABLE: *value = h->p.filter_sep; break;
    case ANTSRL_Q_PERCEIVE_RUN: *value = h->p.meta ? antsrl_perceive_run(h->p) : 0; break;
    case ANTSRL_Q_TIMESTEP: *value = h->host_timestep; break;
    case ANTSRL_Q_DEFERRED_UPDATE: *value = antsrl_update_move_supported(h->p); break;
    default: return fail(ANTSRL_E_INVALID, "bad query selector %d", what);
    }
    return ANTSRL_OK;
}

extern "C" int antsrl_bench_copy(void *dst, const void *src, size_t bytes, void *stream)
{
    if (!dst || !src || (bytes & 15) || ((uintptr_t)dst & 15) || ((uintptr_t)src & 15))
        return fail(ANTSRL_E_INVALID, "bench_copy: 16-byte aligned pointers and a multiple of 16 bytes");
    hipError_t e = antsrl_launch_copy16(dst, src, bytes, (hipStream_t)stream);
    if (e != hipSuccess) return hip_fail(e, "bench_copy");
    return ANTSRL_OK;
}

extern "C" int antsrl_set_timing_events(AntsHandle *h, void *const *events)
{
    if (!h) return fail(ANTSRL_E_INVALID, "NULL handle");
    h->ev_armed = events != nullptr;
    if (events)
        for (int i = 0; i < ANTSRL_TIMING_EVENTS; ++i) h->ev[i] = (hipEvent_t)events[i];
    return ANTSRL_OK;
}

extern "C" int antsrl_set_activation(AntsHandle *h, const float *act, double new_deposit_strength, void *stream)
{
    if (!h || !act) return fail(ANTSRL_E_INVALID, "NULL handle or act");
    if (!h->is_reset) return not_reset(h);
    if (h->phase_next) return mid_update(h);
    int frc = flush_pending(h, (hipStream_t)stream);
    if (frc) return frc;
    hipError_t e = antsrl_launch_set_activation(h->p, act, (hipStream_t)stream);
    if (e != hipSuccess) return hip_fail(e, "set_activation");
    if (new_deposit_strength > 0) h->p.deposit_strength = new_deposit_strength;
    return ANTSRL_OK;
}

hipError_t antsrl_launch_policy(const float *obs, const float *agent_state, const float *w1, const float *b1,
                                const float *w2, const float *b2, const float *w3, const float *b3, int8_t *rot,
                                int8_t *ph, float *logits, int M, int F, hipStream_t st, bool obs_bf16);

extern "C" int antsrl_policy_mlp(AntsHandle *h, const float *obs, const float *agent_state, int64_t n_ants,
                                 int32_t n_features, const float *w1, const float *b1, const float *w2,
                                 const float *b2, const float *w3, const float *b3, int8_t *rotation,
                                 int8_t *pheromone, float *logits, void *stream)
{
    if (!obs || !agent_state || !w1 || !b1 || !w2 || !b2 || !rotation)
        return fail(ANTSRL_E_INVALID, "policy_mlp: obs, agent_state, w1, b1, w2, b2, rotation are required");
    if ((w3 == nullptr) != (b3 == nullptr) || (pheromone && !w3))
        return fail(ANTSRL_E_INVALID, "policy_mlp: w3/b3 go together and are needed for a pheromone output");
    if (n_ants < 1 || n_ants > 0x7fffffff || n_features < 1 || n_features + 2 > 1024)
        return fail(ANTSRL_E_INVALID, "policy_mlp: n_ants >= 1 and 1 <= n_features <= 1022");
    hipError_t e = antsrl_launch_policy(obs, agent_state, w1, b1, w2, b2, w3, b3, rotation, pheromone, logits,
                                        (int)n_ants, n_features, (hipStream_t)stream, h && h->obs_bf16);
    if (e != hipSuccess) return hip_fail(e, "policy_mlp");
    return ANTSRL_OK;
}

extern "C" int antsrl_set_inloop_policy(AntsHandle *h, int32_t n_features, const float *w1, const float *b1, const float *w2,
                                        const float *b2, const float *w3, const float *b3, int8_t *rotation_next,
                                        int8_t *pheromone_next, void *stream)
{
    if (!h) return fail(ANTSRL_E_INVALID, "NULL handle");
    if (!w1) {
        h->pol = PolArgs{};
        return ANTSRL_OK;
    }
    if (!b1 || !w2 || !b2 || !rotation_next)
        return fail(ANTSRL_E_INVALID, "inloop_policy: w1, b1, w2, b2, rotation_next are required");
    if ((w3 == nullptr) != (b3 == nullptr) || (pheromone_next && !w3))
        return fail(ANTSRL_E_INVALID, "inloop_policy: w3/b3 go together and are needed for a pheromone output");
    if (n_features != h->p.PP * h->p.K)
        return fail(ANTSRL_E_INVALID, "inloop_policy: n_features must be P*P*K = %d", h->p.PP * h->p.K);
    if (!h->obs_bf16 || !antsrl_inloop_policy_supported(h->p))
        return fail(ANTSRL_E_UNSUPPORTED, "inloop_policy needs the cell-meta path (ANTSRL_Q_CELL_META) with bfloat16 "
                                          "observations (antsrl_set_obs_format) — use antsrl_policy_mlp otherwise");
    if (h->obs_pitch != 0 && h->obs_pitch != (uint32_t)(h->p.PP * h->p.K))
        return fail(ANTSRL_E_UNSUPPORTED, "the in-loop policy and a padded observation row stride exclude each other (the net reads a "
                                          "dense tile image): antsrl_set_obs_row_stride(h, 0) first");
    hipError_t e = antsrl_launch_policy_pack(h->p.s.pol_pack, w1, b1, w2, b2, w3, b3, n_features, (hipStream_t)stream);
    if (e != hipSuccess) return hip_fail(e, "inloop_policy pack");
    h->pol.pack = h->p.s.pol_pack;
    h->pol.rot = rotation_next;
    h->pol.ph = pheromone_next;
    h->pol.ks = (n_features + 15) / 16;
    return ANTSRL_OK;
}

static size_t state_bytes(const AntsHandle *h, int which)
{
    const size_t E = h->p.E, N = h->p.N, G = (size_t)h->p.W * h->p.H, C = h->p.C, R = h->p.R;
    switch (which) {
    case ANTSRL_S_ANTS_XYT: return 8 * E * N * 3;
    case ANTSRL_S_PREV_XY: return 8 * E * N * 2;
    case ANTSRL_S_HOLDING: case ANTSRL_S_SEED: return 4 * E * N;
    case ANTSRL_S_MANDIBLES: case ANTSRL_S_REWARD_STATE: return E * N;
    case ANTSRL_S_ACTIVATION: return 4 * E * N * C;
    case ANTSRL_S_PHERO: return 4 * E * C * G;
    case ANTSRL_S_FOOD: return 4 * E * G;
    case ANTSRL_S_EXPLORED: case ANTSRL_S_WALLS: case ANTSRL_S_ANTHILL_AREA: return E * G;
    case ANTSRL_S_ANTHILL_FOOD: return 8 * E;
    case ANTSRL_S_ROCK_CENTERS: return 8 * E * R * 2;
    case ANTSRL_S_TIMESTEP: return 4 * E;
    case ANTSRL_S_ANTHILL_XYR: return 4 * E * 3;
    case ANTSRL_S_ROCK_RW: return 8 * E * R * 2;
    case ANTSRL_S_PHERO_C0: case ANTSRL_S_PHERO_C1: case ANTSRL_S_PHERO_C2: case ANTSRL_S_PHERO_C3:
        return (size_t)(which - ANTSRL_S_PHERO_C0) < C ? 4 * E * G : 0;
    default: return 0;
    }
}

extern "C" int antsrl_state_bytes(const AntsHandle *h, int which, size_t *bytes)
{
    if (!h || !bytes) return fail(ANTSRL_E_INVALID, "NULL handle or bytes");
    if (which < 0 || which >= ANTSRL_S_COUNT_) return fail(ANTSRL_E_INVALID, "bad state selector %d", which);
    *bytes = state_bytes(h, which);
    return ANTSRL_OK;
}

extern "C" int antsrl_perceptive_field(AntsHandle *h, uint8_t *dst, void *stream)
{
    if (!h || !dst) return fail(ANTSRL_E_INVALID, "NULL handle or dst");
    if (!h->is_reset) return not_reset(h);
    hipError_t e = antsrl_launch_perceptive_field(h->p, dst, (hipStream_t)stream);
    if (e != hipSuccess) return hip_fail(e, "perceptive_field");
    return ANTSRL_OK;
}

extern "C" int antsrl_read_state(AntsHandle *h, int which, void *dst, void *stream)
{
    if (!h || !dst) return fail(ANTSRL_E_INVALID, "NULL handle or dst");
    if (!h->is_reset) return not_reset(h);
    if (which < 0 || which >= ANTSRL_S_COUNT_) return fail(ANTSRL_E_INVALID, "bad state selector %d", which);
    if (state_bytes(h, which) == 0) return ANTSRL_OK;
    int frc = flush_pending(h, (hipStream_t)stream);
    if (frc) return frc;
    hipError_t e = antsrl_launch_read_state(h->p, which, h->cur, dst, (hipStream_t)stream);
    if (e != hipSuccess) return hip_fail(e, "read_state");
    return ANTSRL_OK;
}
```

### antsrl_amd/csrc/antsrl_device.h

```cpp
#pragma once
#include <stdint.h>
#include "../../include/antsrl.h"

#define META_PRES_MASK 0xFFFFu
#define META_WALL 0x10000u
#define META_AREA 0x20000u
#define META_STAMP_SHIFT 18
#define META_NEVER 0x3FFFu

struct __align__(16) AntFrame { double cx, cy, ct, st; };
#define UMFWD_WIN 0x100
struct UmFwd {
    double x, y, th;
    double th_new, sn, cs;
    float food, hold;
    uint32_t meta;
    int m, rot, pa;
    int rec;
    int pre;
    int has_rot;
    int ts;
    uint8_t primed;
    uint32_t frm_off;
};

struct DState {
    double *x, *y, *theta, *prev_x, *prev_y;
    double *prev_dist;
    float *holding, *seed, *prev_holding;
    float *activation;
    uint8_t *mandibles, *reward_state;
    int32_t *dirty_cell;
    int32_t *walldep_cell;
    float *phero[2];
    float *food;
    uint32_t *walls_bits, *area_bits, *explored_bits;
    uint32_t *big_pres, *big_old;
    int32_t *anthill_xyr;
    double *anthill_food;
    double *rock_cx, *rock_cy, *rock_r, *rock_w;
    int32_t *timestep;
    uint8_t *reward_primed;
    int32_t *gen_discs;
    int32_t *gen_perlin;
    uint8_t *primed_cur;
    AntFrame *frames;
    unsigned char *pol_pack;
};

#define ANTSRL_POL_MAX_KSTEPS 64
#define ANTSRL_POL_WPACK_BYTES (ANTSRL_POL_MAX_KSTEPS * 64 * 16)
#define ANTSRL_POL_A2PACK_BYTES (2 * 64 * 16)
#define ANTSRL_POL_LANEPACK_FLOATS (48 * 64 + 8)
#define ANTSRL_POL_PACK_BYTES (ANTSRL_POL_WPACK_BYTES + ANTSRL_POL_A2PACK_BYTES + 4 * ANTSRL_POL_LANEPACK_FLOATS)
struct PolArgs {
    const unsigned char *pack;
    int8_t *rot, *ph;
    int ks;
    int _pad;
};

struct KP {
    DState s;
    int32_t E, N, W, H, C, R, K, P, PP, r, words;
    int32_t HT;
    int32_t has_mask, has_max_val, reward_kind, max_time, filter_radius, explore_on;
    int32_t ch_kind[ANTSRL_MAX_CHANNELS], ch_arg[ANTSRL_MAX_CHANNELS];
    int32_t mand_first, mand_last;
    uint8_t mask[ANTSRL_MAX_PCELLS + 7];
    double delta, fwd_delta, max_speed, max_rot_speed, carry, backward, max_hold;
    double max_val, deposit_strength, threshold, reward_threshold;
    double fct_explore, fct_food, fct_anthill, fct_explore_holding, fct_heading;
    double filter[ANTSRL_MAX_FILTER_TAPS];
    uint64_t rng_seed;
    uint32_t env_id_base, _pad0;
    int32_t scaled, _pad;
    int32_t ps, fs;
    int32_t meta;
    int32_t tiled;
    int32_t ftile;
    int32_t _pad3;
    double g_now;
    double g_dep;
    double inv_g_dep;
    float ftap[2 * ANTSRL_MAX_FILTER_TAPS];
    int32_t filter_sep, _pad2;
    float fsep_u[2 * (2 * ANTSRL_MAX_FILTER_RADIUS + 1)], fsep_v[2 * (2 * ANTSRL_MAX_FILTER_RADIUS + 1)];
};

#define ACT_STEP 1
#define ACT_HAS_OBS 2
#define ACT_OBS_BF16 8
#define ACT_FRAMES 16
```

### antsrl_amd/csrc/antsrl_layout.h

```cpp
#pragma once
#include <stdint.h>

#if !defined(__HIPCC__) && !defined(__host__)
#define __host__
#define __device__
#endif

__host__ __device__ inline uint32_t tiled_slot(const int x, const int y, const int H)
{
    return (uint32_t)((((x >> 1) * (H >> 2) + (y >> 2)) << 3) + ((x & 1) << 2) + (y & 3));
}

__host__ __device__ inline uint32_t tiled44_slot(const int x, const int y, const int H)
{
    return (uint32_t)((((x >> 2) * (H >> 2) + (y >> 2)) << 4) + ((x & 3) << 2) + (y & 3));
}
```

### antsrl_amd/csrc/antsrl_sweep.hip

```cpp
#include "antsrl_util.h"

#define SW0_UNROLL 4
template <int C>
__global__ void __launch_bounds__(256)
k_sweep0(const KP p, const float *__restrict__ in, float *__restrict__ out)
{
    const uint32_t per_env = (uint32_t)((size_t)p.W * p.H * C / 4);
    const size_t e = blockIdx.y;
    const uint32_t *walls = p.s.walls_bits + e * p.words;
    const float4 *src = reinterpret_cast<const float4 *>(in) + e * per_env;
    float4 *dst = reinterpret_cast<float4 *>(out) + e * per_env;
    const double f0 = p.filter[0], thr = p.threshold;
    const float mx = (float)p.max_val;
    const bool clip = p.has_max_val && p.N > 0;
    const uint32_t v0 = blockIdx.x * (256 * SW0_UNROLL) + threadIdx.x;
    float4 a[SW0_UNROLL];
#pragma unroll
    for (int u = 0; u < SW0_UNROLL; ++u) {
        const uint32_t v = v0 + u * 256;
        if (v < per_env) a[u] = src[v];
    }
#pragma unroll
    for (int u = 0; u < SW0_UNROLL; ++u) {
        const uint32_t v = v0 + u * 256;
        if (v >= per_env) continue;
        float r[4] = {a[u].x, a[u].y, a[u].z, a[u].w};
#pragma unroll
        for (int j = 0; j < 4; ++j) {
            const uint32_t cell = (v * 4 + j) / C;
            const double o = (double)r[j] * f0;
            float f = (o < thr) ? 0.0f : (float)o;
            if (test_bit(walls, cell)) f = 0.0f;
            if (clip) f = fminf(f, mx);
            r[j] = f;
        }
        store_stream(dst + v, make_float4(r[0], r[1], r[2], r[3]));
    }
}

template <int C>
__global__ void __launch_bounds__(256)
k_sweep0_scalar(const KP p, const float *__restrict__ in, float *__restrict__ out, const size_t n)
{
    const size_t per_env = (size_t)p.W * p.H * C;
    const double f0 = p.filter[0], thr = p.threshold;
    const bool clip = p.has_max_val && p.N > 0;
    for (size_t v = (size_t)blockIdx.x * blockDim.x + threadIdx.x; v < n; v += (size_t)gridDim.x * blockDim.x) {
        const size_t e = v / per_env;
        const uint32_t cell = (uint32_t)((v - e * per_env) / C);
        const double o = (double)in[v] * f0;
        float f = (o < thr) ? 0.0f : (float)o;
        if (test_bit(p.s.walls_bits + e * p.words, cell)) f = 0.0f;
        if (clip) f = fminf(f, (float)p.max_val);
        out[v] = f;
    }
}

__global__ void __launch_bounds__(256) k_phero_wall_clear(const KP p, const int buf)
{
    const size_t G = (size_t)p.W * p.H, n = (size_t)p.E * G;
    for (size_t i = (size_t)blockIdx.x * blockDim.x + threadIdx.x; i < n; i += (size_t)gridDim.x * blockDim.x) {
        const size_t e = i / G, g = i - e * G;
        if (test_bit(p.s.walls_bits + e * p.words, (uint32_t)g))
            for (int c = 0; c < p.C; ++c) p.s.phero[buf][(e * G + prec_cell(p, (uint32_t)g)) * p.ps + c] = 0.0f;
    }
}

__global__ void __launch_bounds__(256) k_phero_renorm(const KP p)
{
    const size_t n = (size_t)p.E * p.W * p.H * p.C;
    for (size_t i = (size_t)blockIdx.x * blockDim.x + threadIdx.x; i < n; i += (size_t)gridDim.x * blockDim.x) {
        const size_t j = (i / p.C) * p.ps + (i % p.C);
        const double v = (double)p.s.phero[0][j] * p.g_now;
        p.s.phero[0][j] = v < p.threshold ? 0.0f : (float)v;
    }
}

__device__ __forceinline__ float wave_shr1(float v)
{
    return __builtin_bit_cast(float, __builtin_amdgcn_update_dpp(0, __builtin_bit_cast(int, v), 0x138, 0xF, 0xF, true));
}
__device__ __forceinline__ float wave_shl1(float v)
{
    return __builtin_bit_cast(float, __builtin_amdgcn_update_dpp(0, __builtin_bit_cast(int, v), 0x130, 0xF, 0xF, true));
}

template <int C, int R, bool SEP>
__global__ void __launch_bounds__(256)
k_sweep_march(const KP p, const float *__restrict__ in, float *__restrict__ out, const int seg_rows, const int nstrips, const int nsegs)
{
    constexpr int S = 2 * R + 1, OUTW = 64 - 2 * R, NA = 2 * S - 1;
    const int lane = threadIdx.x & 63, wave = threadIdx.x >> 6;
    const int e = blockIdx.y, W = p.W, H = p.H;
    const int unit = blockIdx.x * 4 + wave, strip = unit % nstrips, segi = unit / nstrips;
    __shared__ float taps[2 * ANTSRL_MAX_FILTER_TAPS];
    if (!SEP && threadIdx.x < 2 * S * S) taps[threadIdx.x] = p.ftap[threadIdx.x];
    if (SEP && threadIdx.x < 2 * S) {
        taps[threadIdx.x] = p.fsep_u[threadIdx.x];
        taps[2 * S + threadIdx.x] = p.fsep_v[threadIdx.x];
    }
    __syncthreads();
    if (segi >= nsegs) return;
    const int y = strip * OUTW - R + lane;
    const bool col_in = y >= 0 && y < H;
    const bool col_out = lane >= R && lane < 64 - R && y < H;
    const int yc = col_in ? y : 0;
    const float colmask = col_in ? 1.0f : 0.0f;
    const size_t G = (size_t)W * H;
    const float *src = in + (size_t)e * G * C;
    float *dst = out + (size_t)e * G * C;
    const uint32_t *walls = p.s.walls_bits + (size_t)e * p.words;
    const bool clip = p.has_max_val && p.N > 0;
    const float thr = (float)p.threshold, mx = (float)p.max_val;
    float acc[NA][C];
#pragma unroll
    for (int j = 0; j < NA; ++j)
#pragma unroll
        for (int c = 0; c < C; ++c) acc[j][c] = 0.0f;

    const int x_lo = segi * seg_rows, x_hi = min(x_lo + seg_rows, W);
    float nv[S][C];
    uint32_t nword[S], ncell[S];
#define MARCH_LOAD(XI0)                                                                              \
    {                                                                                                \
        _Pragma("unroll") for (int s = 0; s < S; ++s)                                                \
        {                                                                                            \
                \
            const int xc = min(max(min((XI0) + s, x_hi + R - 1), 0), W - 1);                        \
            ncell[s] = (uint32_t)(xc * H + yc);                                                      \
            nword[s] = walls[ncell[s] >> 5];                                                         \
        }                                                                                            \
        _Pragma("unroll") for (int s = 0; s < S; ++s)                                                \
        {                                                                                            \
            if (C == 2) {                                                                            \
                const float2 t = *reinterpret_cast<const float2 *>(src + (size_t)ncell[s] * 2);      \
                nv[s][0] = t.x; nv[s][C - 1] = t.y;                                                  \
            } else {                                                                                 \
                _Pragma("unroll") for (int c = 0; c < C; ++c) nv[s][c] = src[(size_t)ncell[s] * C + c]; \
            }                                                                                        \
        }                                                                                            \
    }
    MARCH_LOAD(x_lo - R)
    for (int xi0 = x_lo - R; xi0 < x_hi + R; xi0 += S) {
        float v[S][C];
        uint32_t wword[S];
        uint32_t cellv[S];
#pragma unroll
        for (int s = 0; s < S; ++s) {
            cellv[s] = ncell[s]; wword[s] = nword[s];
#pragma unroll
            for (int c = 0; c < C; ++c) v[s][c] = nv[s][c];
        }
        MARCH_LOAD(xi0 + S)
#pragma unroll
        for (int s = 0; s < S; ++s) {
            const float keep = colmask * (float)(1u - ((wword[s] >> (cellv[s] & 31)) & 1u)) *
                               ((xi0 + s >= 0 && xi0 + s < W) ? 1.0f : 0.0f);
#pragma unroll
            for (int c = 0; c < C; ++c) v[s][c] *= keep;
        }
        if (SEP) {
            float hrow[S][C];
#pragma unroll
            for (int s = 0; s < S; ++s)
#pragma unroll
                for (int c = 0; c < C; ++c) {
                    float h = fmaf(taps[2 * S + 2 * R], v[s][c], 0.0f);
                    h = fmaf(taps[2 * S + 2 * R + 1], v[s][c], h);
                    float up = v[s][c], dn = v[s][c];
#pragma unroll
                    for (int d = 1; d <= R; ++d) {
                        up = wave_shr1(up);
                        dn = wave_shl1(dn);
                        h = fmaf(taps[2 * S + 2 * (R + d)], up, h);
                        h = fmaf(taps[2 * S + 2 * (R + d) + 1], up, h);
                        h = fmaf(taps[2 * S + 2 * (R - d)], dn, h);
                        h = fmaf(taps[2 * S + 2 * (R - d) + 1], dn, h);
                    }
                    hrow[s][c] = h;
                }
#pragma unroll
            for (int a = 0; a < S; ++a) {
                const float uh = taps[2 * a], ul = taps[2 * a + 1];
#pragma unroll
                for (int s = 0; s < S; ++s)
#pragma unroll
                    for (int c = 0; c < C; ++c) {
                        acc[s + a][c] = fmaf(uh, hrow[s][c], acc[s + a][c]);
                        acc[s + a][c] = fmaf(ul, hrow[s][c], acc[s + a][c]);
                    }
            }
        } else
#pragma unroll 1
        for (int b = 0; b < S; ++b) {
            float sh[S][C];
#pragma unroll
            for (int s = 0; s < S; ++s)
#pragma unroll
                for (int c = 0; c < C; ++c) sh[s][c] = __shfl(v[s][c], lane - (b - R));
            const float *tp = taps + 2 * b * S;
#pragma unroll
            for (int a = 0; a < S; ++a) {
                const float fh = tp[2 * a], fl = tp[2 * a + 1];
#pragma unroll
                for (int s = 0; s < S; ++s)
#pragma unroll
                    for (int c = 0; c < C; ++c) {
                        acc[s + a][c] = fmaf(fh, sh[s][c], acc[s + a][c]);
                        acc[s + a][c] = fmaf(fl, sh[s][c], acc[s + a][c]);
                    }
            }
        }
#pragma unroll
        for (int j = 0; j < S; ++j) {
            const int x = xi0 - R + j;
            if (x >= x_lo && x < x_hi && col_out) {
                float r[C];
#pragma unroll
                for (int c = 0; c < C; ++c) {
                    float f = acc[j][c] < thr ? 0.0f : acc[j][c];
                    if (clip) f = fminf(f, mx);
                    r[c] = f;
                }
                const size_t o = ((size_t)x * H + y) * C;
                if (C == 2) {
                    typedef float vf2_t __attribute__((ext_vector_type(2)));
                    __builtin_nontemporal_store(vf2_t{r[0], r[C - 1]}, reinterpret_cast<vf2_t *>(dst + o));
                } else {
#pragma unroll
                    for (int c = 0; c < C; ++c) dst[o + c] = r[c];
                }
            }
        }
#pragma unroll
        for (int j = 0; j < NA; ++j)
#pragma unroll
            for (int c = 0; c < C; ++c) acc[j][c] = (j + S < NA) ? acc[j + S][c] : 0.0f;
    }
#undef MARCH_LOAD
}


__global__ void __launch_bounds__(256)
k_sweep_r1x2(const KP p, const float *__restrict__ in, float *__restrict__ out, const int seg_rows, const int nstrips, const int nsegs)
{
    constexpr int S = 3, NA = 5;
    const int lane = threadIdx.x & 63, wave = threadIdx.x >> 6;
    const int e = blockIdx.y, W = p.W, H = p.H;
    const int unit = blockIdx.x * 4 + wave, strip = unit % nstrips, segi = unit / nstrips;
    __shared__ float taps[2 * 9];
    if (threadIdx.x < 18) taps[threadIdx.x] = p.ftap[threadIdx.x];
    __syncthreads();
    if (segi >= nsegs) return;
    const int y = strip * 128 + 2 * lane;
    const bool col_in = y < H;
    const int yc = col_in ? y : 0;
    const float colmask = col_in ? 1.0f : 0.0f;
    const int yh = lane < 32 ? strip * 128 - 1 : strip * 128 + 128;
    const bool halo_in = yh >= 0 && yh < H;
    const int yhc = halo_in ? yh : 0;
    const float halomask = halo_in ? 1.0f : 0.0f;
    const size_t G = (size_t)W * H;
    const float *src = in + (size_t)e * G * 2;
    float *dst = out + (size_t)e * G * 2;
    const uint32_t *walls = p.s.walls_bits + (size_t)e * p.words;
    const bool clip = p.has_max_val && p.N > 0;
    const float thr = (float)p.threshold, mx = (float)p.max_val;
    float acc[NA][4];
#pragma unroll
    for (int j = 0; j < NA; ++j)
#pragma unroll
        for (int c = 0; c < 4; ++c) acc[j][c] = 0.0f;
    const int x_lo = segi * seg_rows, x_hi = min(x_lo + seg_rows, W);
    float4 nv[S];
    float2 nh[S];
    uint32_t nword[S], nhword[S], ncell[S], nhcell[S];
#define R1_LOAD(XI0)                                                                                 \
    {                                                                                                \
        _Pragma("unroll") for (int s = 0; s < S; ++s)                                                \
        {                                                                                            \
                 \
            const int xc = min(max(min((XI0) + s, x_hi), 0), W - 1);                                \
            ncell[s] = (uint32_t)(xc * H + yc);                                                      \
            nhcell[s] = (uint32_t)(xc * H + yhc);                                                    \
            nword[s] = walls[ncell[s] >> 5];                                                         \
            nhword[s] = walls[nhcell[s] >> 5];                                                       \
        }                                                                                            \
        _Pragma("unroll") for (int s = 0; s < S; ++s)                                                \
        {                                                                                            \
            nv[s] = *reinterpret_cast<const float4 *>(src + (size_t)ncell[s] * 2);                   \
            nh[s] = *reinterpret_cast<const float2 *>(src + (size_t)nhcell[s] * 2);                  \
        }                                                                                            \
    }
    R1_LOAD(x_lo - 1)
    for (int xi0 = x_lo - 1; xi0 < x_hi + 1; xi0 += S) {
        float v[S][4], hv[S][2];
#pragma unroll
        for (int s = 0; s < S; ++s) {
            const float rowm = (xi0 + s >= 0 && xi0 + s < W) ? 1.0f : 0.0f;
            const uint32_t sh0 = ncell[s] & 31u;
            const float k0 = colmask * rowm * (float)(1u - ((nword[s] >> sh0) & 1u));
            const float k1 = colmask * rowm * (float)(1u - ((nword[s] >> (sh0 + 1u)) & 1u));
            const float kh = halomask * rowm * (float)(1u - ((nhword[s] >> (nhcell[s] & 31u)) & 1u));
            v[s][0] = nv[s].x * k0; v[s][1] = nv[s].y * k0; v[s][2] = nv[s].z * k1; v[s][3] = nv[s].w * k1;
            hv[s][0] = nh[s].x * kh; hv[s][1] = nh[s].y * kh;
        }
        R1_LOAD(xi0 + S)
#pragma unroll
        for (int s = 0; s < S; ++s) {
            float lft[2], rgt[2];
#pragma unroll
            for (int c = 0; c < 2; ++c) {
                const float l = wave_shr1(v[s][2 + c]), r = wave_shl1(v[s][c]);
                const float hl = __builtin_bit_cast(float, __builtin_amdgcn_readlane(__builtin_bit_cast(int, hv[s][c]), 0));
                const float hr = __builtin_bit_cast(float, __builtin_amdgcn_readlane(__builtin_bit_cast(int, hv[s][c]), 63));
                lft[c] = lane == 0 ? hl : l;
                rgt[c] = lane == 63 ? hr : r;
            }
#pragma unroll
            for (int a = 0; a < S; ++a) {
                const float f0h = taps[2 * (0 * S + a)], f0l = taps[2 * (0 * S + a) + 1];
                const float f1h = taps[2 * (1 * S + a)], f1l = taps[2 * (1 * S + a) + 1];
                const float f2h = taps[2 * (2 * S + a)], f2l = taps[2 * (2 * S + a) + 1];
#pragma unroll
                for (int c = 0; c < 2; ++c) {
                    float t0 = acc[s + a][c], t1 = acc[s + a][2 + c];
                    t0 = fmaf(f0h, v[s][2 + c], t0); t0 = fmaf(f0l, v[s][2 + c], t0);
                    t0 = fmaf(f1h, v[s][c], t0);     t0 = fmaf(f1l, v[s][c], t0);
                    t0 = fmaf(f2h, lft[c], t0);      t0 = fmaf(f2l, lft[c], t0);
                    t1 = fmaf(f0h, rgt[c], t1);      t1 = fmaf(f0l, rgt[c], t1);
                    t1 = fmaf(f1h, v[s][2 + c], t1); t1 = fmaf(f1l, v[s][2 + c], t1);
                    t1 = fmaf(f2h, v[s][c], t1);     t1 = fmaf(f2l, v[s][c], t1);
                    acc[s + a][c] = t0; acc[s + a][2 + c] = t1;
                }
            }
        }
#pragma unroll
        for (int j = 0; j < S; ++j) {
            const int x = xi0 - 1 + j;
            if (x >= x_lo && x < x_hi && col_in) {
                float r[4];
#pragma unroll
                for (int c = 0; c < 4; ++c) {
                    float f = acc[j][c] < thr ? 0.0f : acc[j][c];
                    if (clip) f = fminf(f, mx);
                    r[c] = f;
                }
                store_stream(reinterpret_cast<float4 *>(dst + ((size_t)x * H + y) * 2), make_float4(r[0], r[1], r[2], r[3]));
            }
        }
#pragma unroll
        for (int j = 0; j < NA; ++j)
#pragma unroll
            for (int c = 0; c < 4; ++c) acc[j][c] = (j + S < NA) ? acc[j + S][c] : 0.0f;
    }
#undef R1_LOAD
}

#define SEP2_HL 4
template <int R>
__global__ void __launch_bounds__(256)
k_sweep_sep2(const KP p, const float *__restrict__ in, float *__restrict__ out, const int seg_rows, const int nstrips, const int nsegs)
{
    constexpr int HL = SEP2_HL, S = 2 * R + 1, OUTW = 128 - 4 * HL;
    const int lane = threadIdx.x & 63, wave = threadIdx.x >> 6;
    const int e = blockIdx.y, W = p.W, H = p.H;
    const int unit = blockIdx.x * 4 + wave, strip = unit % nstrips, segi = unit / nstrips;
    __shared__ float taps[4 * S];
    if (threadIdx.x < 2 * S) {
        taps[threadIdx.x] = p.fsep_u[threadIdx.x];
        taps[2 * S + threadIdx.x] = p.fsep_v[threadIdx.x];
    }
    __syncthreads();
    if (segi >= nsegs) return;
    const int y = strip * OUTW - 2 * HL + 2 * lane;
    const bool col_in = y >= 0 && y < H;
    const bool col_out = lane >= HL && lane < 64 - HL && y < H;
    const int yc = col_in ? y : 0;
    const float colmask = col_in ? 1.0f : 0.0f;
    const size_t G = (size_t)W * H;
    const float *src = in + (size_t)e * G * 2;
    float *dst = out + (size_t)e * G * 2;
    const uint32_t *walls = p.s.walls_bits + (size_t)e * p.words;
    const bool clip = p.has_max_val && p.N > 0;
    const float thr = (float)p.threshold, mx = (float)p.max_val;
    float uh[S], ul[S], vh[S], vl[S];
#pragma unroll
    for (int a = 0; a < S; ++a) {
        uh[a] = __builtin_bit_cast(float, __builtin_amdgcn_readfirstlane(__builtin_bit_cast(int, taps[2 * a])));
        ul[a] = __builtin_bit_cast(float, __builtin_amdgcn_readfirstlane(__builtin_bit_cast(int, taps[2 * a + 1])));
        vh[a] = __builtin_bit_cast(float, __builtin_amdgcn_readfirstlane(__builtin_bit_cast(int, taps[2 * S + 2 * a])));
        vl[a] = __builtin_bit_cast(float, __builtin_amdgcn_readfirstlane(__builtin_bit_cast(int, taps[2 * S + 2 * a + 1])));
    }
    typedef float v2f __attribute__((ext_vector_type(2)));
#define FMA2(t, q, r) __builtin_elementwise_fma((v2f)(t), (q), (r))
#define SHR2(q) (v2f){wave_shr1((q).x), wave_shr1((q).y)}
#define SHL2(q) (v2f){wave_shl1((q).x), wave_shl1((q).y)}
    v2f acc[S][2];
#pragma unroll
    for (int j = 0; j < S; ++j) acc[j][0] = acc[j][1] = (v2f)(0.0f);
    const int x_lo = segi * seg_rows, x_hi = min(x_lo + seg_rows, W), nrows = x_hi - x_lo;
    const int x0 = x_lo - R;
    float4 nv[S];
    uint32_t nword[S], ncell[S];
#define SEP2_LOAD1(I0, s)                                                                            \
    {                                                                                                \
         \
        const int xc = min(max(x0 + min((I0) + (s), nrows + 2 * R - 1), 0), W - 1);                \
        ncell[s] = (uint32_t)(xc * H + yc);                                                          \
        nword[s] = walls[ncell[s] >> 5];                                                             \
        nv[s] = *reinterpret_cast<const float4 *>(src + (size_t)ncell[s] * 2);                       \
    }
#pragma unroll
    for (int s = 0; s < S; ++s) SEP2_LOAD1(0, s)
    for (int i0 = 0; i0 < nrows + 2 * R; i0 += S) {
#pragma unroll
        for (int s = 0; s < S; ++s) {
            const int xin = x0 + (i0 + s);
            const float rowm = (xin >= 0 && xin < W) ? 1.0f : 0.0f;
            const uint32_t sh0 = ncell[s] & 31u;
            const float k0 = colmask * rowm * (float)(1u - ((nword[s] >> sh0) & 1u));
            const float k1 = colmask * rowm * (float)(1u - ((nword[s] >> (sh0 + 1u)) & 1u));
            const v2f a0 = (v2f){nv[s].x, nv[s].y} * (v2f)(k0), a1 = (v2f){nv[s].z, nv[s].w} * (v2f)(k1);
            SEP2_LOAD1(i0 + S, s)
            const v2f m1_0 = SHR2(a0), m1_1 = SHR2(a1);
            const v2f p1_0 = SHL2(a0), p1_1 = SHL2(a1);
            v2f nb0[S], nb1[S];
            nb0[R] = a0; nb1[R] = a1;
            nb0[R + 1] = a1; nb1[R - 1] = a0;
            nb0[R - 1] = m1_1; nb1[R + 1] = p1_0;
            nb0[R - 2] = m1_0; nb0[R + 2] = p1_0;
            nb1[R - 2] = m1_1; nb1[R + 2] = p1_1;
            if constexpr (R == 3) {
                const v2f m2_1 = SHR2(m1_1);
                const v2f p2_0 = SHL2(p1_0);
                nb0[R - 3] = m2_1; nb0[R + 3] = p1_1;
                nb1[R - 3] = m1_0; nb1[R + 3] = p2_0;
            }
            v2f h0 = FMA2(vh[R], nb0[R], (v2f)(0.0f)), h1 = FMA2(vh[R], nb1[R], (v2f)(0.0f));
            h0 = FMA2(vl[R], nb0[R], h0); h1 = FMA2(vl[R], nb1[R], h1);
#pragma unroll
            for (int d = 1; d <= R; ++d) {
                h0 = FMA2(vh[R + d], nb0[R - d], h0); h1 = FMA2(vh[R + d], nb1[R - d], h1);
                h0 = FMA2(vl[R + d], nb0[R - d], h0); h1 = FMA2(vl[R + d], nb1[R - d], h1);
                h0 = FMA2(vh[R - d], nb0[R + d], h0); h1 = FMA2(vh[R - d], nb1[R + d], h1);
                h0 = FMA2(vl[R - d], nb0[R + d], h0); h1 = FMA2(vl[R - d], nb1[R + d], h1);
            }
#pragma unroll
            for (int a = 0; a < S; ++a) {
                const int slot = (s + a - R + 2 * S) % S;
                acc[slot][0] = FMA2(uh[a], h0, acc[slot][0]); acc[slot][1] = FMA2(uh[a], h1, acc[slot][1]);
                acc[slot][0] = FMA2(ul[a], h0, acc[slot][0]); acc[slot][1] = FMA2(ul[a], h1, acc[slot][1]);
            }
            {
                const int slot = (s - R + 2 * S) % S;
                const int io = i0 + s - 2 * R;
                if (io >= 0 && io < nrows && col_out) {
                    const int x = x_lo + io;
                    float r[4] = {acc[slot][0].x, acc[slot][0].y, acc[slot][1].x, acc[slot][1].y};
#pragma unroll
                    for (int c = 0; c < 4; ++c) {
                        r[c] = r[c] < thr ? 0.0f : r[c];
                        if (clip) r[c] = fminf(r[c], mx);
                    }
                    store_stream(reinterpret_cast<float4 *>(dst + ((size_t)x * H + y) * 2), make_float4(r[0], r[1], r[2], r[3]));
                }
                acc[slot][0] = acc[slot][1] = (v2f)(0.0f);
            }
        }
    }
#undef FMA2
#undef SHR2
#undef SHL2
#undef SEP2_LOAD1
}

template <int C>
static hipError_t launch_sweep_c(const KP &p, int cur, hipStream_t st)
{
    const float *in = p.s.phero[cur];
    float *out = p.s.phero[cur ^ 1];
    const size_t n = (size_t)p.E * p.W * p.H * C;
    if (p.filter_radius == 0) {
        if (((size_t)p.W * p.H * C) % 4 == 0) {
            const size_t per_env4 = (size_t)p.W * p.H * C / 4;
            const unsigned bx = (unsigned)((per_env4 + 256 * SW0_UNROLL - 1) / (256 * SW0_UNROLL));
            hipLaunchKernelGGL((k_sweep0<C>), dim3(bx, (unsigned)p.E), dim3(256), 0, st, p, in, out);
        } else {
            size_t blocks = (n + 255) / 256;
            if (blocks > 256 * 64) blocks = 256 * 64;
            hipLaunchKernelGGL((k_sweep0_scalar<C>), dim3((unsigned)blocks), dim3(256), 0, st, p, in, out, n);
        }
    } else {
        const int fr = p.filter_radius;
        const bool two_col = C == 2 && (p.H & 1) == 0;
        const int seg_rows = std::min(p.W, fr == 1 ? 16 : (two_col && p.filter_sep) || fr == 2 ? 32 : 64);
        const int nsegs = (p.W + seg_rows - 1) / seg_rows;
        if constexpr (C == 2) {
            if (fr == 1 && two_col) {
                const int strips2 = (p.H + 127) / 128;
                hipLaunchKernelGGL(k_sweep_r1x2, dim3((strips2 * nsegs + 3) / 4, p.E), dim3(256), 0, st, p, in, out, seg_rows, strips2, nsegs);
                return hipGetLastError();
            }
            if (fr >= 2 && p.filter_sep && two_col) {
                const int outw = 128 - 4 * SEP2_HL;
                const int strips2 = (p.H + outw - 1) / outw;
                const dim3 grid2((strips2 * nsegs + 3) / 4, p.E);
                if (fr == 2) hipLaunchKernelGGL((k_sweep_sep2<2>), grid2, dim3(256), 0, st, p, in, out, seg_rows, strips2, nsegs);
                else hipLaunchKernelGGL((k_sweep_sep2<3>), grid2, dim3(256), 0, st, p, in, out, seg_rows, strips2, nsegs);
                return hipGetLastError();
            }
        }
        const int strips = (p.H + (64 - 2 * fr) - 1) / (64 - 2 * fr);
        const dim3 grid((strips * nsegs + 3) / 4, p.E);
#define MARCH_GO(RR, SEPV) hipLaunchKernelGGL((k_sweep_march<C, RR, SEPV>), grid, dim3(256), 0, st, p, in, out, seg_rows, strips, nsegs)
        if (p.filter_sep) {
            if (fr == 1) MARCH_GO(1, true);
            else if (fr == 2) MARCH_GO(2, true);
            else MARCH_GO(3, true);
        } else if (fr == 1) MARCH_GO(1, false);
        else if (fr == 2) MARCH_GO(2, false);
        else MARCH_GO(3, false);
#undef MARCH_GO
    }
    return hipGetLastError();
}

hipError_t antsrl_launch_sweep(const KP &p, int cur, hipStream_t st)
{
    switch (p.C) {
    case 1: return launch_sweep_c<1>(p, cur, st);
    case 2: return launch_sweep_c<2>(p, cur, st);
    case 3: return launch_sweep_c<3>(p, cur, st);
    case 4: return launch_sweep_c<4>(p, cur, st);
    default: return hipErrorInvalidValue;
    }
}

hipError_t antsrl_launch_phero_wall_clear(const KP &p, hipStream_t st, int buf)
{
    hipLaunchKernelGGL(k_phero_wall_clear, dim3(grid_for((size_t)p.E * p.W * p.H)), dim3(256), 0, st, p, buf);
    return hipGetLastError();
}

hipError_t antsrl_launch_phero_renorm(const KP &p, hipStream_t st)
{
    hipLaunchKernelGGL(k_phero_renorm, dim3(grid_for((size_t)p.E * p.W * p.H * p.C)), dim3(256), 0, st, p);
    return hipGetLastError();
}
```

### antsrl_amd/csrc/antsrl_update_env.h

```cpp
#pragma once
#include "antsrl_util.h"

__device__ __forceinline__ uint32_t block_excl_scan_flag(bool flag, uint32_t *wave_tot, int lane, int wave,
                                                         int nwaves, uint32_t *block_total)
{
    const unsigned long long m = __ballot(flag);
    const uint32_t in_wave = (uint32_t)__popcll(m & ((1ull << lane) - 1ull));
    if (lane == 0) wave_tot[wave] = (uint32_t)__popcll(m);
    __syncthreads();
    uint32_t off = 0, tot = 0;
    for (int w = 0; w < nwaves; ++w) {
        const uint32_t t = wave_tot[w];
        if (w < wave) off += t;
        tot += t;
    }
    __syncthreads();
    *block_total = tot;
    return off + in_wave;
}

#define UPD_WALLS 1
#define UPD_ROCKS 2
#define UPD_ANTS 4
#define UPD_ANTHILL 8
#define UPD_ALL 15
template <int C>
__device__ __forceinline__ void update_env(const KP &p, const int e, const double *__restrict__ wall_jitter,
                                           const int out_buf, unsigned char *smem, const int phases = UPD_ALL)
{
    const int tid = threadIdx.x, T = blockDim.x;
    const int lane = tid & 63, wave = tid >> 6, nwaves = T >> 6;
    const int N = p.N, W = p.W, H = p.H, R = p.R;
    const size_t G = (size_t)W * H, eN = (size_t)e * N;
    uint32_t *hkeys = (uint32_t *)smem, *hvals = hkeys + p.HT;
    double *rk = (double *)(smem + align_up(8 * (size_t)p.HT, 16));
    double *red = rk + 2 * (R > 0 ? R : 1);
    uint32_t *wave_tot = (uint32_t *)(red + nwaves);

    const uint32_t *walls = p.s.walls_bits + (size_t)e * p.words;
    const FoodView food{p.s.food + (size_t)e * G * p.fs, p.fs};
    const size_t PS = (size_t)p.ps;
    float *out = p.s.phero[out_buf] + (size_t)e * G * PS;
    const int ts = p.s.timestep[e] + 1;

    for (int h = tid; h < p.HT; h += T) {
        hkeys[h] = HASH_EMPTY;
        hvals[h] = 0u;
    }

    uint32_t carry = 0;
    if (p.scaled && (phases & UPD_WALLS)) {
        for (int i = tid; i < N; i += T) {
            const int32_t wc = p.s.walldep_cell[eN + i];
            if (wc >= 0) {
                for (int c = 0; c < C; ++c) out[(size_t)wc * PS + c] = 0.0f;
                p.s.walldep_cell[eN + i] = -1;
            }
        }
    }
    for (int base = 0; (phases & UPD_WALLS) && base < N; base += T) {
        const int i = base + tid;
        bool hit = false;
        if (i < N) hit = test_bit(walls, (uint32_t)((int)p.s.x[eN + i] * H + (int)p.s.y[eN + i]));
        double u = 0.0;
        if (wall_jitter) {
            uint32_t tot;
            const uint32_t rank = carry + block_excl_scan_flag(hit, wave_tot, lane, wave, nwaves, &tot);
            carry += tot;
            if (hit) u = wall_jitter[eN + rank];
        } else if (hit) {
            u = jitter_u01(p.rng_seed, p.env_id_base + (uint32_t)e, (uint32_t)ts, (uint32_t)i);
        }
        if (hit) {
            p.s.x[eN + i] = p.s.prev_x[eN + i];
            p.s.y[eN + i] = p.s.prev_y[eN + i];
            p.s.theta[eN + i] += u - 0.5;
        }
    }
    __syncthreads();

    if (R > 0 && (phases & UPD_ROCKS)) {
        for (int q = wave; q < R; q += nwaves) {
            const double cx = p.s.rock_cx[(size_t)e * R + q], cy = p.s.rock_cy[(size_t)e * R + q];
            const double rad = p.s.rock_r[(size_t)e * R + q];
            const double rad2_hi = rad * rad * (1.0 + 1e-12) + 1e-300;
            double sx = 0.0, sy = 0.0;
            for (int base = 0; base < N; base += 64) {
                const int i = base + lane;
                double px = 0.0, py = 0.0;
                bool col = false;
                if (i < N) {
                    const double vx = cx - p.s.x[eN + i], vy = cy - p.s.y[eN + i];
                    const double d2 = vx * vx + vy * vy;
                    if (!(d2 > rad2_hi)) {
                        const double d = sqrt(d2);
                        const double f = 1 - rad / (d + 0.001);
                        px = vx * f; py = vy * f;
                        col = !(d > rad);
                    }
                }
                unsigned long long m = __ballot(col);
                while (m) {
                    const int l = __builtin_ctzll(m);
                    m &= m - 1;
                    sx += __shfl(px, l);
                    sy += __shfl(py, l);
                }
            }
            if (lane == 0) {
                const double wgt = p.s.rock_w[(size_t)e * R + q];
                rk[2 * q + 0] = cx - sx / wgt;
                rk[2 * q + 1] = cy - sy / wgt;
            }
        }
        __syncthreads();
        for (int q = tid; q < R; q += T) {
            p.s.rock_cx[(size_t)e * R + q] = rk[2 * q + 0];
            p.s.rock_cy[(size_t)e * R + q] = rk[2 * q + 1];
        }
        for (int i = tid; i < N; i += T) {
            const double x = p.s.x[eN + i], y = p.s.y[eN + i];
            double sx = 0.0, sy = 0.0;
            for (int q = 0; q < R; ++q) {
                const double vx = rk[2 * q + 0] - x, vy = rk[2 * q + 1] - y;
                const double rad = p.s.rock_r[(size_t)e * R + q];
                const double d2 = vx * vx + vy * vy;
                if (d2 > rad * rad * (1.0 + 1e-12) + 1e-300) continue;
                const double d = sqrt(d2);
                const double f = 1 - rad / (d + 0.001);
                double px = vx * f, py = vy * f;
                if (d > rad) { px = 0.0; py = 0.0; }
                sx += px; sy += py;
            }
            p.s.x[eN + i] = warp_coord(x + sx, (double)W);
            p.s.y[eN + i] = warp_coord(y + sy, (double)H);
        }
        __syncthreads();
    }

    for (int i = tid; (phases & UPD_ANTS) && i < N; i += T) {
        const double x = p.s.x[eN + i], y = p.s.y[eN + i];
        p.s.prev_x[eN + i] = x;
        p.s.prev_y[eN + i] = y;
        lww_insert(hkeys, hvals, (uint32_t)p.HT - 1, prec_xy(p, (int)x, (int)y), (uint32_t)i);
        p.s.reward_state[eN + i] = (uint8_t)((double)p.s.reward_state[eN + i] * 0.9);
    }
    __syncthreads();
    for (int i = tid; (phases & UPD_ANTS) && i < N; i += T) {
        const uint32_t cell_id = (uint32_t)((int)p.s.x[eN + i] * H + (int)p.s.y[eN + i]);
        const uint32_t cell = prec_xy(p, (int)p.s.x[eN + i], (int)p.s.y[eN + i]);
        if (lww_winner(hkeys, hvals, (uint32_t)p.HT - 1, cell) == (uint32_t)i) {
            if (!p.scaled) {
                for (int c = 0; c < C; ++c) {
                    const float a = p.s.activation[(eN + i) * C + c];
                    if (a != 0.0f) {
                        float v = out[(size_t)cell * PS + c] + a;
                        if (p.has_max_val) v = fminf(v, (float)p.max_val);
                        out[(size_t)cell * PS + c] = v;
                    }
                }
            } else {
                const bool on_wall = test_bit(walls, cell_id);
                bool wrote = false;
                for (int c = 0; c < C; ++c) {
                    const float a = p.s.activation[(eN + i) * C + c];
                    if (a != 0.0f) {
                        double v = (double)out[(size_t)cell * PS + c] * p.g_dep;
                        if (v < p.threshold || on_wall) v = 0.0;
                        v += (double)a;
                        if (p.has_max_val) v = fmin(v, p.max_val);
                        out[(size_t)cell * PS + c] = (float)(v * p.inv_g_dep);
                        wrote = true;
                    } else if (on_wall) {
                        out[(size_t)cell * PS + c] = 0.0f;
                    }
                }
                if (on_wall && wrote) p.s.walldep_cell[eN + i] = (int32_t)cell;
            }
        }
    }
    double gain = 0.0;
    for (int i = tid; (phases & UPD_ANTHILL) && i < N; i += T) {
        const int32_t dc = p.s.dirty_cell[eN + i];
        if (dc >= 0) {
            gain += (double)food[dc];
            food[dc] = 0.0f;
            p.s.dirty_cell[eN + i] = -1;
        }
    }
    for (int o = 32; o > 0; o >>= 1) gain += __shfl_down(gain, o);
    if (lane == 0) red[wave] = gain;
    __syncthreads();
    if (tid == 0 && (phases & UPD_ANTHILL)) {
        double s = 0.0;
        for (int w = 0; w < nwaves; ++w) s += red[w];
        if (s != 0.0) p.s.anthill_food[e] += s;
        p.s.timestep[e] = ts;
    }
}
```

### antsrl_amd/csrc/antsrl_update_one.h

```cpp
#pragma once
#include "antsrl_util.h"
#include "antsrl_update_env.h"

__host__ __device__ inline size_t update_one_lds_bytes(int HT, int R, int nwaves, int N)
{
    return align_up(8 * (size_t)HT, 16) + 48 * (size_t)(R > 0 ? R : 1) + 8 * (size_t)nwaves +
           align_up(4 * (size_t)nwaves, 8) + 16 * (size_t)N + align_up(4 * (size_t)R, 16) + 16;
}

template <int C, bool FWD_REC = false>
__device__ __forceinline__ void update_one_body(const KP &p, const int e, const double *__restrict__ wall_jitter, const int out_buf,
                                                unsigned char *smem, const double g_dep, const double inv_g_dep, UmFwd *fw = nullptr)
{
    const int tid = threadIdx.x, T = blockDim.x;
    const int lane = tid & 63, wave = __builtin_amdgcn_readfirstlane(tid >> 6), nwaves = T >> 6;
    const int N = p.N, W = p.W, H = p.H, R = p.R;
    const size_t G = (size_t)W * H, eN = (size_t)e * N;
    uint32_t *hkeys = (uint32_t *)smem, *hvals = hkeys + p.HT;
    double *rock = (double *)(smem + align_up(8 * (size_t)p.HT, 16));
    double *rk = rock + 4 * (R > 0 ? R : 1);
    double *red = rk + 2 * (R > 0 ? R : 1);
    uint32_t *wave_tot = (uint32_t *)(red + nwaves);
    double *sx = (double *)((unsigned char *)wave_tot + align_up(4 * (size_t)nwaves, 8)), *sy = sx + N;
    uint32_t *rk_hit = (uint32_t *)(sy + N);

    const uint32_t *walls = p.s.walls_bits + (size_t)e * p.words;
    const FoodView food{p.s.food + (size_t)e * G * p.fs, p.fs};
    const size_t PS = (size_t)p.ps;
    float *out = p.s.phero[out_buf] + (size_t)e * G * PS;
    const bool on = tid < N;
    const size_t a = eN + (on ? tid : 0);

    double x = p.s.x[a], y = p.s.y[a];
    const double px0 = STP_LD(p.s.prev_x[a]), py0 = STP_LD(p.s.prev_y[a]);
    const uint8_t rstate = STP_LD(p.s.reward_state[a]);
    const double theta0 = p.s.theta[a];
    float act[C];
#pragma unroll
    for (int c = 0; c < C; ++c) act[c] = STP_LD(p.s.activation[a * C + c]);
    const int32_t wc_l = STP_LD(p.s.walldep_cell[a]), dc_l = STP_LD(p.s.dirty_cell[a]);
    const int32_t wc = (p.scaled && on) ? wc_l : -1;
    const int32_t dc = on ? dc_l : -1;
    const int ts = p.s.timestep[e] + 1;
    if (tid < R) {
        rock[4 * tid + 0] = p.s.rock_cx[(size_t)e * R + tid];
        rock[4 * tid + 1] = p.s.rock_cy[(size_t)e * R + tid];
        rock[4 * tid + 2] = p.s.rock_r[(size_t)e * R + tid];
        rock[4 * tid + 3] = p.s.rock_w[(size_t)e * R + tid];
    }
    for (int h = tid; h < p.HT; h += T) {
        hkeys[h] = HASH_EMPTY;
        hvals[h] = 0u;
    }
    const float food_dc_l = food[dc_l >= 0 ? dc_l : 0];
    const float food_dc = dc >= 0 ? food_dc_l : 0.0f;

    const bool hit = on && test_bit(walls, (uint32_t)((int)x * H + (int)y));
    double u = 0.0;
    if (wall_jitter) {
        uint32_t tot;
        const uint32_t rank = block_excl_scan_flag(hit, wave_tot, lane, wave, nwaves, &tot);
        if (hit) u = wall_jitter[eN + rank];
    } else if (hit) {
        u = jitter_u01(p.rng_seed, p.env_id_base + (uint32_t)e, (uint32_t)ts, (uint32_t)tid);
    }
    bool moved = hit;
    if (hit) {
        x = px0;
        y = py0;
        if (!fw) p.s.theta[a] = theta0 + (u - 0.5);
    }
    if (fw) fw->th = hit ? theta0 + (u - 0.5) : theta0;

    if (R > 0) {
        if (on) {
            sx[tid] = x;
            sy[tid] = y;
        }
        __syncthreads();
        for (int q = wave; q < R; q += nwaves) {
            const double cx = rock[4 * q + 0], cy = rock[4 * q + 1], rad = rock[4 * q + 2];
            const double rad2_hi = rad * rad * (1.0 + 1e-12) + 1e-300;
            double sumx = 0.0, sumy = 0.0;
            bool any = false;
            for (int base = 0; base < N; base += 64) {
                const int i = base + lane;
                double px = 0.0, py = 0.0;
                bool col = false;
                if (i < N) {
                    const double vx = cx - sx[i], vy = cy - sy[i];
                    const double d2 = vx * vx + vy * vy;
                    if (!(d2 > rad2_hi)) {
                        const double d = sqrt(d2);
                        const double f = 1 - rad / (d + 0.001);
                        px = vx * f; py = vy * f;
                        col = !(d > rad);
                    }
                }
                unsigned long long m = __ballot(col);
                any |= m != 0;
                while (m) {
                    const int l = __builtin_ctzll(m);
                    m &= m - 1;
                    sumx += __shfl(px, l);
                    sumy += __shfl(py, l);
                }
            }
            if (lane == 0) {
                rk[2 * q + 0] = cx - sumx / rock[4 * q + 3];
                rk[2 * q + 1] = cy - sumy / rock[4 * q + 3];
                rk_hit[q] = any ? 1u : 0u;
            }
        }
        __syncthreads();
        if (tid < R) {
            p.s.rock_cx[(size_t)e * R + tid] = rk[2 * tid + 0];
            p.s.rock_cy[(size_t)e * R + tid] = rk[2 * tid + 1];
        }
        double ax = 0.0, ay = 0.0;
        for (int q = 0; q < R; ++q) {
            if (!rk_hit[q]) continue;
            const double vx = rk[2 * q + 0] - x, vy = rk[2 * q + 1] - y;
            const double rad = rock[4 * q + 2];
            const double d2 = vx * vx + vy * vy;
            if (d2 > rad * rad * (1.0 + 1e-12) + 1e-300) continue;
            const double d = sqrt(d2);
            const double f = 1 - rad / (d + 0.001);
            double px = vx * f, py = vy * f;
            if (d > rad) { px = 0.0; py = 0.0; }
            ax += px; ay += py;
        }
        x = warp_coord(x + ax, (double)W);
        y = warp_coord(y + ay, (double)H);
        moved = true;
    }

    __syncthreads();
    const uint32_t cell_id = (uint32_t)((int)x * H + (int)y);
    const uint32_t cell = prec_xy(p, (int)x, (int)y);
    float pold[C];
    constexpr bool fw_rec = FWD_REC && C == 2;
    if constexpr (fw_rec) {
        const stream_f4 rec = *reinterpret_cast<const stream_f4 *>(out + (size_t)cell * 4);
        pold[0] = rec.x;
        pold[C - 1] = rec.y;
        fw->food = rec.z;
        fw->meta = __float_as_uint(rec.w);
    } else {
#pragma unroll
        for (int c = 0; c < C; ++c) pold[c] = out[(size_t)cell * PS + c];
    }
    if (fw) {
        double th = fw->th;
        if (fw->has_rot) th = np_mod_d(th + (double)fw->rot * p.max_rot_speed, 2 * PI_D);
        fw->th_new = th;
        sincos(th, &fw->sn, &fw->cs);
        fw->pre = 1;
        fw->ts = ts;
        if (fw->frm_off) {
            double st2, ct2;
            sincos(th + PI_D * 0.5, &st2, &ct2);
            double *fs = reinterpret_cast<double *>(smem + fw->frm_off) + 2 * tid;
            fs[0] = ct2;
            fs[1] = st2;
        }
    }
    if (on) {
        if (moved && !fw) {
            p.s.x[a] = x;
            p.s.y[a] = y;
        }
        STP_ST(p.s.prev_x[a], x);
        STP_ST(p.s.prev_y[a], y);
        if (fw) {
            fw->x = x;
            fw->y = y;
        }
        lww_insert(hkeys, hvals, (uint32_t)p.HT - 1, cell, (uint32_t)tid);
        STP_ST(p.s.reward_state[a], (uint8_t)((double)rstate * 0.9));
    }
    __syncthreads();
    if (p.scaled) {
        if (wc >= 0) {
            for (int c = 0; c < C; ++c) out[(size_t)wc * PS + c] = 0.0f;
            p.s.walldep_cell[a] = -1;
        }
        __syncthreads();
    }
    if constexpr (fw_rec) {
        asm volatile("" : "+v"(pold[0]), "+v"(pold[C - 1]), "+v"(fw->food), "+v"(fw->meta));
    }
    double gain = 0.0;
    if (on) {
        const bool winner = lww_winner(hkeys, hvals, (uint32_t)p.HT - 1, cell) == (uint32_t)tid;
        if (fw && winner) fw->m |= UMFWD_WIN;
        if (winner) {
            if (!p.scaled) {
#pragma unroll
                for (int c = 0; c < C; ++c) {
                    if (act[c] != 0.0f) {
                        float v = pold[c] + act[c];
                        if (p.has_max_val) v = fminf(v, (float)p.max_val);
                        out[(size_t)cell * PS + c] = v;
                    }
                }
            } else {
                bool on_wall;
                if constexpr (fw_rec) on_wall = (fw->meta & META_WALL) != 0;
                else on_wall = test_bit(walls, cell_id);
                bool wrote = false;
#pragma unroll
                for (int c = 0; c < C; ++c) {
                    if (act[c] != 0.0f) {
                        double v = (double)pold[c] * g_dep;
                        if (v < p.threshold || on_wall) v = 0.0;
                        v += (double)act[c];
                        if (p.has_max_val) v = fmin(v, p.max_val);
                        out[(size_t)cell * PS + c] = (float)(v * inv_g_dep);
                        wrote = true;
                    } else if (on_wall) {
                        out[(size_t)cell * PS + c] = 0.0f;
                    }
                }
                if (on_wall && wrote) p.s.walldep_cell[a] = (int32_t)cell;
            }
        }
        if (dc >= 0) {
            gain = (double)food_dc;
            food[dc] = 0.0f;
            p.s.dirty_cell[a] = -1;
        }
    }
    for (int o = 32; o > 0; o >>= 1) gain += __shfl_down(gain, o);
    if (lane == 0) red[wave] = gain;
    __syncthreads();
    if (tid == 0) {
        double s2 = 0.0;
        for (int w = 0; w < nwaves; ++w) s2 += red[w];
        if (s2 != 0.0) p.s.anthill_food[e] += s2;
        p.s.timestep[e] = ts;
    }
}
```

### include/antsrl.h

```cpp
#ifndef ANTSRL_H
#define ANTSRL_H

#include <stddef.h>
#include <stdint.h>

#ifdef __cplusplus
extern "C" {
#endif

#define ANTSRL_ABI_VERSION 5

#define ANTSRL_MAX_CHANNELS 16
#define ANTSRL_MAX_PSIDE 15
#define ANTSRL_MAX_PCELLS (ANTSRL_MAX_PSIDE * ANTSRL_MAX_PSIDE)
#define ANTSRL_MAX_FILTER_RADIUS 3
#define ANTSRL_MAX_FILTER_TAPS 49
#define ANTSRL_MAX_PHERO 4

#define ANTSRL_OK 0
#define ANTSRL_E_INVALID (-1)
#define ANTSRL_E_NOMEM (-2)
#define ANTSRL_E_DEVICE (-3)
#define ANTSRL_E_UNSUPPORTED (-4)

enum {
    ANTSRL_CH_ANTS = 0,
    ANTSRL_CH_PHERO = 1,
    ANTSRL_CH_ANTHILL = 2,
    ANTSRL_CH_WALLS = 3,
    ANTSRL_CH_FOOD = 4,
    ANTSRL_CH_ROCKS = 5
};

enum { ANTSRL_PHERO_AUTO = 0, ANTSRL_PHERO_EXPLICIT_SWEEP = 1 };

enum { ANTSRL_ACT_AUTO = 0, ANTSRL_ACT_CELL_META = 1, ANTSRL_ACT_SINGLE_KERNEL = 2 };

enum {
    ANTSRL_REWARD_NONE = 0,
    ANTSRL_REWARD_EXPLORATION = 1,
    ANTSRL_REWARD_FOOD = 2,
    ANTSRL_REWARD_ALL = 3
};

typedef struct AntsCfg {
    int32_t abi_version;
    int32_t n_envs;
    int32_t n_ants;
    int32_t w, h;
    int32_t n_phero;
    int32_t n_rocks;
    int32_t max_time;

    int32_t perception_radius;
    int32_t n_channels;
    int32_t channel_kind[ANTSRL_MAX_CHANNELS];
    int32_t channel_arg[ANTSRL_MAX_CHANNELS];
    int32_t has_mask;
    uint8_t mask[ANTSRL_MAX_PCELLS];
    uint8_t _pad0[7];
    double delta;
    double fwd_delta;

    double max_speed, max_rot_speed, carry_speed_reduction, backward_speed_reduction;
    double max_hold;

    int32_t has_max_val;
    int32_t filter_radius;
    double phero_max_val;
    double deposit_strength;
    double phero_threshold;
    double filter[ANTSRL_MAX_FILTER_TAPS];

    int32_t reward_kind;
    int32_t phero_mode;
    double reward_threshold;
    double fct_explore, fct_food, fct_anthill, fct_explore_holding, fct_headinganthill;

    uint64_t rng_seed;

    int32_t act_path;

    int32_t env_id_base;
    int32_t n_envs_total;
    int32_t _pad1;
} AntsCfg;

typedef struct AntsInit {
    const double *ants_xyt;
    const double *seed;
    const uint8_t *walls;
    const float *food;
    const int32_t *anthill_xyr;
    const double *rocks;
    const float *phero;
} AntsInit;

#define ANTSRL_MAX_FOOD_DISCS 64
#define ANTSRL_WALLS_BERNOULLI 0
#define ANTSRL_WALLS_PERLIN 1
#define ANTSRL_WALLS_INPUT 2
#define ANTSRL_RNG_COUNTER 0
#define ANTSRL_RNG_REFERENCE 1
typedef struct AntsGen {
    double wall_density;
    int32_t n_food_discs;
    int32_t food_rmin, food_rmax;
    int32_t auto_reset;
    int32_t wall_kind;
    int32_t perlin_octaves;
    double perlin_scale;
    double perlin_persistence;
    double perlin_lacunarity;
    int32_t rng_kind;
    int32_t _pad;
    const uint8_t *walls_input;
} AntsGen;

typedef struct AntsHandle AntsHandle;

enum {
    ANTSRL_S_ANTS_XYT = 0,
    ANTSRL_S_PREV_XY = 1,
    ANTSRL_S_HOLDING = 2,
    ANTSRL_S_MANDIBLES = 3,
    ANTSRL_S_ACTIVATION = 4,
    ANTSRL_S_PHERO = 5,
    ANTSRL_S_FOOD = 6,
    ANTSRL_S_EXPLORED = 7,
    ANTSRL_S_ANTHILL_FOOD = 8,
    ANTSRL_S_ROCK_CENTERS = 9,
    ANTSRL_S_TIMESTEP = 10,
    ANTSRL_S_REWARD_STATE = 11,
    ANTSRL_S_WALLS = 12,
    ANTSRL_S_ANTHILL_AREA = 13,
    ANTSRL_S_SEED = 14,
    ANTSRL_S_ANTHILL_XYR = 15,
    ANTSRL_S_ROCK_RW = 16,
    ANTSRL_S_PHERO_C0 = 17,
    ANTSRL_S_PHERO_C1 = 18,
    ANTSRL_S_PHERO_C2 = 19,
    ANTSRL_S_PHERO_C3 = 20,
    ANTSRL_S_COUNT_
};

int antsrl_abi_version(void);

size_t antsrl_cfg_size(void);

const char *antsrl_last_error(void);

int antsrl_workspace_bytes(const AntsCfg *cfg, size_t *bytes);

int antsrl_create(const AntsCfg *cfg, void *workspace, size_t workspace_bytes, AntsHandle **out);

void antsrl_destroy(AntsHandle *h);

int antsrl_reset(AntsHandle *h, const AntsInit *init, void *stream);

int antsrl_generate(AntsHandle *h, const AntsGen *gen, uint64_t episode_seed, void *stream);

int antsrl_step(AntsHandle *h, const int8_t *rotation, const int8_t *phero, float *obs,
                float *agent_state, float *reward, uint8_t *done, void *stream);

int antsrl_observe(AntsHandle *h, float *obs, float *agent_state, float *reward, void *stream);

int antsrl_update(AntsHandle *h, const double *wall_jitter, void *stream);

enum { ANTSRL_PHASE_WALLS = 0, ANTSRL_PHASE_ROCKS_PHEROMONE = 1, ANTSRL_PHASE_ANTS = 2, ANTSRL_PHASE_ANTHILL = 3 };
int antsrl_update_phase(AntsHandle *h, int phase, const double *wall_jitter, void *stream);

int antsrl_flush(AntsHandle *h, void *stream);

int antsrl_step_update(AntsHandle *h, const int8_t *rotation, const int8_t *phero,
                       const double *wall_jitter, float *obs, float *agent_state, float *reward,
                       uint8_t *done, void *stream);

#define ANTSRL_TIMING_EVENTS 5
int antsrl_set_timing_events(AntsHandle *h, void *const *events);

enum {
    ANTSRL_Q_CELL_META = 0,
    ANTSRL_Q_SCALED_UNITS = 1,
    ANTSRL_Q_INTERLEAVED = 2,
    ANTSRL_Q_FILTER_SEPARABLE = 3,
    ANTSRL_Q_PERCEIVE_RUN = 4,
    ANTSRL_Q_TIMESTEP = 5,
    ANTSRL_Q_DEFERRED_UPDATE = 6,
    ANTSRL_Q_COUNT_
};
int antsrl_query(const AntsHandle *h, int what, long long *value);

int antsrl_bench_copy(void *dst, const void *src, size_t bytes, void *stream);

#define ANTSRL_MEM_PIECE_BYTES ((size_t)16 << 20)
int antsrl_mem_alloc(size_t bytes, int device, void **ptr);
int antsrl_mem_free(void *ptr);
int antsrl_mem_trim(void);
int antsrl_mem_stats(size_t *live_bytes, size_t *pooled_bytes, size_t *reserved_va_bytes, size_t *retired_va_bytes);

#define ANTSRL_OBS_F32 0
#define ANTSRL_OBS_BF16 1
int antsrl_set_obs_format(AntsHandle *h, int format);

int antsrl_set_obs_row_stride(AntsHandle *h, int32_t stride_elems);

int antsrl_set_activation(AntsHandle *h, const float *act, double new_deposit_strength,
                          void *stream);

int antsrl_policy_mlp(AntsHandle *h, const float *obs, const float *agent_state, int64_t n_ants, int32_t n_features,
                      const float *w1, const float *b1, const float *w2, const float *b2, const float *w3,
                      const float *b3, int8_t *rotation, int8_t *pheromone, float *logits, void *stream);

int antsrl_set_inloop_policy(AntsHandle *h, int32_t n_features, const float *w1, const float *b1, const float *w2,
                             const float *b2, const float *w3, const float *b3, int8_t *rotation_next,
                             int8_t *pheromone_next, void *stream);

typedef struct AntsMemNetShape {
    int32_t n_features, agent_dim, mem_size, h1, h2, h3, n_rot, n_ph;
} AntsMemNetShape;

int antsrl_memnet_packed_bytes(const AntsMemNetShape *s, size_t *bytes);

int antsrl_memnet_pack(const AntsMemNetShape *s, const float *const *params, void *packed, void *stream);

int antsrl_policy_memory(const AntsMemNetShape *s, const void *packed, const void *obs, int obs_format,
                         const float *agent_state, const float *mem_in, int64_t n_ants, float *mem_out, int8_t *rotation,
                         int8_t *pheromone, float *q_out, void *stream);

#define ANTSRL_MEMNET_BF16 0
#define ANTSRL_MEMNET_FP32 1

int antsrl_memnet_packed_bytes_ex(const AntsMemNetShape *s, int precision, size_t *bytes);

int antsrl_memnet_pack_ex(const AntsMemNetShape *s, int precision, const float *const *params, void *packed, void *stream);

int antsrl_policy_memory_ex(const AntsMemNetShape *s, int precision, const void *packed, const void *obs, int obs_format,
                            const float *agent_state, const float *mem_in, int64_t n_ants, float *mem_out,
                            int8_t *rotation, int8_t *pheromone, float *q_out, void *stream);

int antsrl_policy_memory_tiles(const AntsMemNetShape *s, int precision, const void *packed, const void *obs, int obs_format,
                               const float *agent_state, const float *mem_in, int64_t n_ants, float *mem_out,
                               int8_t *rotation, int8_t *pheromone, float *q_out, const int32_t *tiles,
                               const int32_t *n_live, void *stream);

int antsrl_memtrain_sizes(const AntsMemNetShape *s, int64_t B, size_t *params_floats, size_t *trained_floats,
                          size_t *state_bytes, size_t *workspace_bytes);

int antsrl_memtrain_init(const AntsMemNetShape *s, const float *const *params, void *state, void *stream);

int antsrl_memtrain_unpack(const AntsMemNetShape *s, const void *state, float *const *params, void *stream);

int antsrl_memtrain_copy(const AntsMemNetShape *s, const void *src_state, void *dst_state, void *stream);

int antsrl_memtrain_grad(const AntsMemNetShape *s, const void *state, const void *target_state, const float *states,
                         const float *agent_states, const int64_t *actions, const float *rewards, const float *new_states,
                         const float *new_agent_states, const uint8_t *dones, const int64_t *idx, int64_t B,
                         float discount, float *grads, float *loss_out, void *workspace, void *stream);

int antsrl_memtrain_apply(const AntsMemNetShape *s, void *state, const float *grads, int64_t step, double lr,
                          double beta1, double beta2, double eps, void *stream);

#define ANTSRL_DRAW_EXPLORE 0x45584C4FULL
#define ANTSRL_DRAW_ROTATION 0x524F5441ULL
#define ANTSRL_DRAW_PHEROMONE 0x50484552ULL
#define ANTSRL_DRAW_SAMPLE 0x53414D50ULL

int antsrl_agent_select(uint64_t seed, uint64_t step, int32_t env_id_base, int32_t n_envs, int32_t n_ants, double epsilon,
                        int32_t n_rot, int32_t n_ph, int32_t mem_size, int8_t *rotation, int8_t *pheromone,
                        const float *mem_old, float *mem_next, uint8_t *explored, void *stream);

int antsrl_agent_plan(uint64_t seed, uint64_t step, int32_t env_id_base, int32_t n_envs, int32_t n_ants, double epsilon,
                      int32_t *tiles, int32_t *n_live, void *stream);

typedef struct AntsRecordSpec {
    int32_t n_envs, n_ants, env_id_base;
    int32_t n_features, agent_dim, mem_size, n_rot;
    int32_t obs_format;
    int32_t obs_pitch;
    int32_t reserved;
    int64_t K, head, max_len;
    uint64_t seed, step;
} AntsRecordSpec;

int antsrl_replay_record_pre(const AntsRecordSpec *r, const void *obs, const float *agent_state, const float *memory,
                             const int8_t *rotation, const int8_t *pheromone, float *states, float *agent_states,
                             int64_t *actions, void *stream);
int antsrl_replay_record_post(const AntsRecordSpec *r, const void *obs, const float *agent_state, const float *memory,
                              const float *reward, const uint8_t *done, float *rewards, float *new_states,
                              float *new_agent_states, uint8_t *dones, void *stream);

int antsrl_agent_select_actions(uint64_t seed, uint64_t step, int32_t env_id_base, int32_t n_envs, int32_t n_ants,
                                double epsilon, int32_t n_rot, int32_t n_ph, int8_t *rotation, int8_t *pheromone,
                                uint8_t *explored, void *stream);
int antsrl_replay_record_pre_plain(const AntsRecordSpec *r, const void *obs, const float *agent_state,
                                   const int8_t *rotation, const int8_t *pheromone, float *states, float *agent_states,
                                   int64_t *actions, void *stream);
int antsrl_replay_record_post_plain(const AntsRecordSpec *r, const void *obs, const float *agent_state, const float *reward,
                                    const uint8_t *done, float *rewards, float *new_states, float *new_agent_states,
                                    uint8_t *dones, void *stream);

int antsrl_lintrain_sizes(int32_t n_features, int64_t B, size_t *trained_floats, size_t *workspace_bytes, int32_t *launches);
int antsrl_lintrain_grad(int32_t n_features, const float *w1, const float *b1, const float *heads, const float *target_l3,
                         const float *states, const float *agent_states, const int64_t *actions, const float *rewards,
                         const float *new_states, const float *new_agent_states, const uint8_t *dones, int64_t n_rows,
                         const int64_t *idx, int64_t B, float discount, float *grads, float *loss, void *workspace,
                         void *stream);
int antsrl_lintrain_apply(float *heads, float *adam_m, float *adam_v, const float *grads, int64_t step, double lr,
                          double beta1, double beta2, double eps, void *stream);
int antsrl_lintrain_step(int32_t n_features, const float *w1, const float *b1, float *heads, const float *target_l3,
                         float *adam_m, float *adam_v, const float *states, const float *agent_states,
                         const int64_t *actions, const float *rewards, const float *new_states,
                         const float *new_agent_states, const uint8_t *dones, int64_t n_rows, const int64_t *idx, int64_t B,
                         float discount, int64_t step, double lr, double beta1, double beta2, double eps, float *grads,
                         float *loss, void *workspace, void *stream);

int antsrl_exptrain_sizes(int32_t n_features, int64_t B, size_t *trained_floats, size_t *workspace_bytes, int32_t *launches);
int antsrl_exptrain_grad(int32_t n_features, const float *model, const float *target, const float *states,
                         const float *agent_states, const int64_t *actions, const float *rewards, const float *new_states,
                         const float *new_agent_states, const uint8_t *dones, int64_t n_rows, const int64_t *idx, int64_t B,
                         float discount, float *grads, float *loss, void *workspace, void *stream);
int antsrl_exptrain_apply(int32_t n_features, float *model, float *adam_m, float *adam_v, const float *grads, int64_t step,
                          double lr, double beta1, double beta2, double eps, void *stream);
int antsrl_exptrain_step(int32_t n_features, float *model, const float *target, float *adam_m, float *adam_v,
                         const float *states, const float *agent_states, const int64_t *actions, const float *rewards,
                         const float *new_states, const float *new_agent_states, const uint8_t *dones, int64_t n_rows,
                         const int64_t *idx, int64_t B, float discount, int64_t step, double lr, double beta1, double beta2,
                         double eps, float *grads, float *loss, void *workspace, void *stream);

typedef struct AntsReworkShape {
    int32_t n_features, agent_dim,
            g1, g2, g3,
            r1, r2, r3,
            p1,
            n_rot, n_ph;
} AntsReworkShape;

int antsrl_rework_collapsed_bytes(const AntsReworkShape *s, size_t *bytes);

int antsrl_rework_collapse(const AntsReworkShape *s, const float *const *params, void *collapsed, void *stream);

int antsrl_policy_rework(const AntsReworkShape *s, const void *collapsed, const void *obs, int obs_format,
                         const float *agent_state, int64_t n_ants, int8_t *rotation, int8_t *pheromone, float *q_out,
                         void *stream);

int antsrl_policy_rework_select(const AntsReworkShape *s, const void *collapsed, const void *obs, int obs_format,
                                const float *agent_state, uint64_t seed, uint64_t step, int32_t env_id_base,
                                int32_t n_envs, int32_t n_ants, double epsilon, int8_t *rotation, int8_t *pheromone,
                                uint8_t *explored, float *q_out, void *stream);

int antsrl_reworktrain_sizes(const AntsReworkShape *s, int64_t B, size_t *params_floats, size_t *workspace_bytes,
                             int32_t *launches);
int antsrl_reworktrain_grad(const AntsReworkShape *s, const float *model, const float *target_collapsed, const float *states,
                            const float *agent_states, const int64_t *actions, const float *rewards, const float *new_states,
                            const float *new_agent_states, const uint8_t *dones, int64_t n_rows, const int64_t *idx,
                            int64_t B, float discount, float *grads, float *loss, void *workspace, void *stream);
int antsrl_reworktrain_apply(const AntsReworkShape *s, float *model, float *adam_m, float *adam_v, const float *grads,
                             int64_t step, double lr, double beta1, double beta2, double eps, void *stream);
int antsrl_reworktrain_step(const AntsReworkShape *s, float *model, const float *target_collapsed, float *adam_m,
                            float *adam_v, const float *states, const float *agent_states, const int64_t *actions,
                            const float *rewards, const float *new_states, const float *new_agent_states,
                            const uint8_t *dones, int64_t n_rows, const int64_t *idx, int64_t B, float discount,
                            int64_t step, double lr, double beta1, double beta2, double eps, float *grads, float *loss,
                            void *workspace, void *stream);

int antsrl_read_state(AntsHandle *h, int which, void *dst, void *stream);

int antsrl_perceptive_field(AntsHandle *h, uint8_t *dst, void *stream);

int antsrl_state_bytes(const AntsHandle *h, int which, size_t *bytes);

#ifdef __cplusplus
}
#endif
#endif
```

Baseline: 2.678 billion.

## Skip pheromone sweep work for tiles with no nonzero pheromone blocks

Adds per-block activity flags (8x16 cells) to each pheromone buffer. Deposits set them, and the separable sweep kernel sets them for its outputs. A sweep wave whose input halo has no flagged blocks skips the filter, zero-fills only output blocks that were previously nonzero, and clears their flags. This targets bandwidth and compute spent convolving empty regions of the grid. In exchange it adds flag bookkeeping, memsets on reset and wall clear, and correctness risk if some write path fails to set a flag.

Measured after the change: 2.424 billion. 0.905x the previous value.

```diff
diff --git a/antsrl_amd/_lib.py b/antsrl_amd/_lib.py
--- a/antsrl_amd/_lib.py
+++ b/antsrl_amd/_lib.py
@@ -22,7 +22,8 @@
            "antsrl_lintrain_grad", "antsrl_lintrain_apply", "antsrl_lintrain_step", "antsrl_exptrain_sizes",
            "antsrl_exptrain_grad", "antsrl_exptrain_apply", "antsrl_exptrain_step", "antsrl_rework_collapsed_bytes",
            "antsrl_rework_collapse", "antsrl_policy_rework", "antsrl_reworktrain_sizes", "antsrl_reworktrain_grad",
-           "antsrl_reworktrain_apply", "antsrl_reworktrain_step", "antsrl_policy_rework_select")
+           "antsrl_reworktrain_apply", "antsrl_reworktrain_step", "antsrl_policy_rework_select", "antsrl_set_sweep_skip",
+           "antsrl_read_sweep_flags")
 
 _lib = None
 
@@ -80,6 +81,8 @@
     lib.antsrl_set_inloop_policy.argtypes = [vp, i32] + [vp] * 9
     lib.antsrl_bench_copy.argtypes = [vp, vp, C.c_size_t, vp]
     lib.antsrl_set_obs_row_stride.argtypes = [vp, i32]
+    lib.antsrl_set_sweep_skip.argtypes = [vp, i32]
+    lib.antsrl_read_sweep_flags.argtypes = [vp, i32, vp, vp, vp]
     lib.antsrl_mem_alloc.argtypes = [C.c_size_t, i32, C.POINTER(vp)]
     lib.antsrl_mem_free.argtypes = [vp]
     lib.antsrl_mem_trim.argtypes = []
diff --git a/antsrl_amd/batched.py b/antsrl_amd/batched.py
--- a/antsrl_amd/batched.py
+++ b/antsrl_amd/batched.py
@@ -122,6 +122,8 @@
         pitch, row = getattr(self, "_obs_pitch_row", (0, 0))
         if pitch != row:
             _lib.check(self.lib.antsrl_set_obs_row_stride(self._h, pitch), "set_obs_row_stride")
+        if not getattr(self, "_sweep_skip", True):
+            _lib.check(self.lib.antsrl_set_sweep_skip(self._h, 0), "set_sweep_skip")
 
     def tune_placement(self, age: int = 150, steps: int = 30, verbose: bool = False, extra_outputs: int = 4,
                        walk_spacers: int = 3, spacer_gib: float = 24.0, force_walk: bool = False):
@@ -429,6 +431,18 @@
                                                       self._stream()), "set_activation")
         self._loaded = "given an activation matrix"
 
+    def set_sweep_skip(self, on: bool) -> None:
+        _lib.check(self.lib.antsrl_set_sweep_skip(self._h, 1 if on else 0), "set_sweep_skip")
+        self._sweep_skip = bool(on)
+
+    def read_sweep_flags(self, which: int = 0, cells: bool = False):
+        c = self.cfg
+        fl = torch.empty((c.n_envs, (c.w + 7) // 8, (c.h + 15) // 16), dtype=torch.uint8, device=self.device)
+        mem = torch.empty((c.n_envs, c.w, c.h, c.n_phero), dtype=torch.float32, device=self.device) if cells else None
+        with torch.cuda.device(self.device):
+            _lib.check(self.lib.antsrl_read_sweep_flags(self._h, int(which), _ptr(fl), _ptr(mem), self._stream()), "read_sweep_flags")
+        return (fl, mem) if cells else fl
+
     def perceptive_field(self) -> torch.Tensor:
         c = self.cfg
         out = torch.empty((c.n_envs, c.w, c.h), dtype=torch.uint8, device=self.device)
diff --git a/antsrl_amd/config.py b/antsrl_amd/config.py
--- a/antsrl_amd/config.py
+++ b/antsrl_amd/config.py
@@ -19,7 +19,7 @@
 PHERO_AUTO, PHERO_EXPLICIT_SWEEP = 0, 1
 ACT_AUTO, ACT_CELL_META, ACT_SINGLE_KERNEL = 0, 1, 2
 TIMING_EVENTS = 5
-Q_CELL_META, Q_SCALED_UNITS, Q_INTERLEAVED, Q_FILTER_SEPARABLE, Q_PERCEIVE_RUN, Q_TIMESTEP, Q_DEFERRED_UPDATE = range(7)
+Q_CELL_META, Q_SCALED_UNITS, Q_INTERLEAVED, Q_FILTER_SEPARABLE, Q_PERCEIVE_RUN, Q_TIMESTEP, Q_DEFERRED_UPDATE, Q_SWEEP_FLAGS = range(8)
 
 (S_ANTS_XYT, S_PREV_XY, S_HOLDING, S_MANDIBLES, S_ACTIVATION, S_PHERO, S_FOOD, S_EXPLORED,
  S_ANTHILL_FOOD, S_ROCK_CENTERS, S_TIMESTEP, S_REWARD_STATE, S_WALLS, S_ANTHILL_AREA,
diff --git a/antsrl_amd/csrc/antsrl_capi.hip b/antsrl_amd/csrc/antsrl_capi.hip
--- a/antsrl_amd/csrc/antsrl_capi.hip
+++ b/antsrl_amd/csrc/antsrl_capi.hip
@@ -13,7 +13,8 @@
                              float *agent_state, float *reward, uint8_t *done, int flags, hipStream_t st);
 bool antsrl_act_fits(const KP &p);
 bool antsrl_act_needs_hbm_maps(const KP &p);
-hipError_t antsrl_launch_sweep(const KP &p, int cur, hipStream_t st);
+hipError_t antsrl_launch_sweep(const KP &p, int cur, hipStream_t st, bool skip);
+bool antsrl_sweep_has_flags(const KP &p);
 hipError_t antsrl_launch_update(const KP &p, const double *jitter, int out_buf, hipStream_t st, int phases = 15);
 hipError_t antsrl_launch_collect_full(const KP &p, hipStream_t st);
 hipError_t antsrl_launch_reset(const KP &p, const AntsInit *in, hipStream_t st);
@@ -63,6 +64,8 @@
     KP pend_p;
     int pend_out_buf;
     int phase_next;
+    bool skip_on;
+    bool flags_ones[2];
 };
 
 static thread_local char g_err[512] = "";
@@ -147,7 +150,7 @@
     return use_scaled(c) && c->n_phero == 2;
 }
 
-static size_t carve(const AntsCfg *c, DState *s, unsigned char *base)
+static size_t carve(const AntsCfg *c, DState *s, unsigned char *base, uint8_t **flags = nullptr)
 {
     const size_t E = c->n_envs, N = c->n_ants, G = (size_t)c->w * c->h, Cn = c->n_phero, R = c->n_rocks;
     const size_t words = (G + 31) / 32;
@@ -196,6 +199,13 @@
     d.gen_perlin = (int32_t *)take(4 * E * 2);
     d.pol_pack = (unsigned char *)take(ANTSRL_POL_PACK_BYTES);
     if (s) *s = d;
+    if (antsrl_sweep_has_flags(kp)) {
+        const size_t fb = E * (size_t)phflag_nbx(c->w) * phflag_nby(c->h);
+        unsigned char *f0 = take(fb), *f1 = take(fb);
+        if (flags) { flags[0] = f0; flags[1] = f1; }
+    } else if (flags) {
+        flags[0] = flags[1] = nullptr;
+    }
     return off;
 }
 
@@ -314,7 +324,9 @@
     if (!h) return fail(ANTSRL_E_NOMEM, "out of host memory");
     h->cfg = *cfg;
     fill_kp(cfg, &h->p);
-    carve(cfg, &h->p.s, (unsigned char *)workspace);
+    carve(cfg, &h->p.s, (unsigned char *)workspace, h->p.blk_flags);
+    h->skip_on = true;
+    h->flags_ones[0] = h->flags_ones[1] = false;
     h->cur = 0; h->steps_since_update = 0; h->need_full_collect = true; h->is_reset = false; h->episode_over = false; h->pend_update = false;
     h->phase_next = 0;
     h->pol = PolArgs{};
@@ -336,6 +348,29 @@
 
 extern "C" void antsrl_destroy(AntsHandle *h) { delete h; }
 
+static int flags_set_ones(AntsHandle *h, int buf, hipStream_t st)
+{
+    if (!h->p.blk_flags[buf] || h->flags_ones[buf]) return ANTSRL_OK;
+    const size_t fb = (size_t)h->p.E * phflag_nbx(h->p.W) * phflag_nby(h->p.H);
+    hipError_t e = hipMemsetAsync(h->p.blk_flags[buf], 1, fb, st);
+    if (e != hipSuccess) return hip_fail(e, "pheromone activity flags");
+    h->flags_ones[buf] = true;
+    return ANTSRL_OK;
+}
+
+static int launch_sweep(AntsHandle *h, hipStream_t st)
+{
+    const bool skip = h->skip_on && h->p.blk_flags[0] != nullptr;
+    if (!skip) {
+        int rc = flags_set_ones(h, h->cur ^ 1, st);
+        if (rc) return rc;
+    }
+    hipError_t e = antsrl_launch_sweep(h->p, h->cur, st, skip);
+    if (e != hipSuccess) return hip_fail(e, "pheromone sweep");
+    if (skip) h->flags_ones[h->cur ^ 1] = false;
+    return ANTSRL_OK;
+}
+
 extern "C" int antsrl_reset(AntsHandle *h, const AntsInit *init, void *stream)
 {
     if (!h || !init) return fail(ANTSRL_E_INVALID, "NULL handle or init");
@@ -346,6 +381,11 @@
     h->phase_next = 0;
     hipError_t e = antsrl_launch_reset(h->p, init, (hipStream_t)stream);
     if (e != hipSuccess) return hip_fail(e, "reset");
+    for (int b = 0; b < 2; ++b) {
+        h->flags_ones[b] = false;
+        int frc = flags_set_ones(h, b, (hipStream_t)stream);
+        if (frc) return frc;
+    }
     h->p.deposit_strength = h->cfg.deposit_strength;
     h->cur = 0; h->steps_since_update = 0; h->need_full_collect = true; h->is_reset = true; h->episode_over = false;
     h->sweeps = 0; h->need_wall_clear = h->p.scaled && init->phero != nullptr;
@@ -371,6 +411,11 @@
     h->phase_next = 0;
     hipError_t e = antsrl_launch_generate(h->p, h->gen, seed, st);
     if (e != hipSuccess) return hip_fail(e, "generate");
+    for (int b = 0; b < 2; ++b) {
+        h->flags_ones[b] = false;
+        int frc = flags_set_ones(h, b, st);
+        if (frc) return frc;
+    }
     h->p.deposit_strength = h->cfg.deposit_strength;
     h->cur = 0; h->steps_since_update = 0; h->need_full_collect = true; h->is_reset = true; h->episode_over = false;
     h->sweeps = 0; h->need_wall_clear = false; h->host_timestep = 1; h->obs_seq = 0;
@@ -545,8 +590,8 @@
             h->need_wall_clear = false;
         }
     } else if (!sweep_done) {
-        e = antsrl_launch_sweep(h->p, h->cur, st);
-        if (e != hipSuccess) return hip_fail(e, "pheromone sweep");
+        int src = launch_sweep(h, st);
+        if (src) return src;
     }
     if (may_defer && !jitter && !h->need_full_collect && antsrl_update_move_supported(h->p)) {
         h->pend_update = true;
@@ -631,6 +676,8 @@
         } else {
             e = antsrl_launch_phero_wall_clear(h->p, st, h->cur);
             if (e != hipSuccess) return hip_fail(e, "pheromone wall clear");
+            int frc2 = flags_set_ones(h, h->cur, st);
+            if (frc2) return frc2;
         }
         e = antsrl_launch_update(h->p, wall_jitter, h->p.scaled ? 0 : h->cur, st, 1 );
         if (e != hipSuccess) return hip_fail(e, "update: walls");
@@ -641,8 +688,8 @@
             h->sweeps++;
             set_decay(h);
         } else {
-            e = antsrl_launch_sweep(h->p, h->cur, st);
-            if (e != hipSuccess) return hip_fail(e, "pheromone sweep");
+            int src = launch_sweep(h, st);
+            if (src) return src;
             h->cur ^= 1;
         }
     } else if (phase == ANTSRL_PHASE_ANTS) {
@@ -688,16 +735,16 @@
     if (timed) (void)hipEventRecord(h->ev[0], st);
     const bool sweep_late = !h->p.scaled && h->pend_update;
     if (!h->p.scaled && !sweep_late) {
-        hipError_t e = antsrl_launch_sweep(h->p, h->cur, st);
-        if (e != hipSuccess) return hip_fail(e, "pheromone sweep");
+        int src = launch_sweep(h, st);
+        if (src) return src;
     }
     if (timed) (void)hipEventRecord(h->ev[1], st);
     int rc = do_step(h, rotation, phero, obs, agent_state, reward, done, st, timed);
     if (rc) return rc;
     if (timed) (void)hipEventRecord(h->ev[3], st);
     if (sweep_late) {
-        hipError_t e = antsrl_launch_sweep(h->p, h->cur, st);
-        if (e != hipSuccess) return hip_fail(e, "pheromone sweep");
+        int src = launch_sweep(h, st);
+        if (src) return src;
     }
     const bool was_done = h->host_timestep == h->cfg.max_time;
     const bool regen = was_done && h->has_gen && h->gen.auto_reset;
@@ -725,6 +772,7 @@
     case ANTSRL_Q_PERCEIVE_RUN: *value = h->p.meta ? antsrl_perceive_run(h->p) : 0; break;
     case ANTSRL_Q_TIMESTEP: *value = h->host_timestep; break;
     case ANTSRL_Q_DEFERRED_UPDATE: *value = antsrl_update_move_supported(h->p); break;
+    case ANTSRL_Q_SWEEP_FLAGS: *value = h->p.blk_flags[0] != nullptr; break;
     default: return fail(ANTSRL_E_INVALID, "bad query selector %d", what);
     }
     return ANTSRL_OK;
@@ -736,6 +784,32 @@
         return fail(ANTSRL_E_INVALID, "bench_copy: 16-byte aligned pointers and a multiple of 16 bytes");
     hipError_t e = antsrl_launch_copy16(dst, src, bytes, (hipStream_t)stream);
     if (e != hipSuccess) return hip_fail(e, "bench_copy");
+    return ANTSRL_OK;
+}
+
+extern "C" int antsrl_set_sweep_skip(AntsHandle *h, int on)
+{
+    if (!h) return fail(ANTSRL_E_INVALID, "NULL handle");
+    h->skip_on = on != 0;
+    return ANTSRL_OK;
+}
+
+extern "C" int antsrl_read_sweep_flags(AntsHandle *h, int which, uint8_t *flags, float *cells, void *stream)
+{
+    if (!h || !flags) return fail(ANTSRL_E_INVALID, "NULL handle or flags");
+    if (!h->is_reset) return not_reset(h);
+    if (which != 0 && which != 1) return fail(ANTSRL_E_INVALID, "which: 0 (the current buffer) or 1 (the other one)");
+    if (h->p.scaled) return fail(ANTSRL_E_UNSUPPORTED, "antsrl_read_sweep_flags needs an explicit sweep (ANTSRL_Q_SCALED_UNITS is 1)");
+    hipStream_t st = (hipStream_t)stream;
+    int frc = flush_pending(h, st);
+    if (frc) return frc;
+    const int buf = h->cur ^ which;
+    const size_t fb = (size_t)h->p.E * phflag_nbx(h->p.W) * phflag_nby(h->p.H);
+    hipError_t e = h->p.blk_flags[buf] ? hipMemcpyAsync(flags, h->p.blk_flags[buf], fb, hipMemcpyDeviceToDevice, st)
+                                       : hipMemsetAsync(flags, 1, fb, st);
+    if (e == hipSuccess && cells)
+        e = hipMemcpyAsync(cells, h->p.s.phero[buf], 4 * (size_t)h->p.E * h->p.W * h->p.H * h->p.C, hipMemcpyDeviceToDevice, st);
+    if (e != hipSuccess) return hip_fail(e, "read_sweep_flags");
     return ANTSRL_OK;
 }
 
diff --git a/antsrl_amd/csrc/antsrl_device.h b/antsrl_amd/csrc/antsrl_device.h
--- a/antsrl_amd/csrc/antsrl_device.h
+++ b/antsrl_amd/csrc/antsrl_device.h
@@ -1,6 +1,7 @@
 #pragma once
 #include <stdint.h>
 #include "../../include/antsrl.h"
+#include "antsrl_layout.h"
 
 #define META_PRES_MASK 0xFFFFu
 #define META_WALL 0x10000u
@@ -86,6 +87,7 @@
     float ftap[2 * ANTSRL_MAX_FILTER_TAPS];
     int32_t filter_sep, _pad2;
     float fsep_u[2 * (2 * ANTSRL_MAX_FILTER_RADIUS + 1)], fsep_v[2 * (2 * ANTSRL_MAX_FILTER_RADIUS + 1)];
+    uint8_t *blk_flags[2];
 };
 
 #define ACT_STEP 1
diff --git a/antsrl_amd/csrc/antsrl_layout.h b/antsrl_amd/csrc/antsrl_layout.h
--- a/antsrl_amd/csrc/antsrl_layout.h
+++ b/antsrl_amd/csrc/antsrl_layout.h
@@ -15,3 +15,12 @@
 {
     return (uint32_t)((((x >> 2) * (H >> 2) + (y >> 2)) << 4) + ((x & 3) << 2) + (y & 3));
 }
+
+#define PHFLAG_ROWS 8
+#define PHFLAG_COLS 16
+__host__ __device__ inline int phflag_nbx(const int W) { return (W + PHFLAG_ROWS - 1) / PHFLAG_ROWS; }
+__host__ __device__ inline int phflag_nby(const int H) { return (H + PHFLAG_COLS - 1) / PHFLAG_COLS; }
+__host__ __device__ inline uint32_t phflag_slot(const int x, const int y, const int H)
+{
+    return (uint32_t)((x / PHFLAG_ROWS) * phflag_nby(H) + y / PHFLAG_COLS);
+}
diff --git a/antsrl_amd/csrc/antsrl_sweep.hip b/antsrl_amd/csrc/antsrl_sweep.hip
--- a/antsrl_amd/csrc/antsrl_sweep.hip
+++ b/antsrl_amd/csrc/antsrl_sweep.hip
@@ -358,14 +358,28 @@
 }
 
 #define SEP2_HL 4
-template <int R>
+template <int R, bool FL>
 __global__ void __launch_bounds__(256)
-k_sweep_sep2(const KP p, const float *__restrict__ in, float *__restrict__ out, const int seg_rows, const int nstrips, const int nsegs)
+k_sweep_sep2(const KP p, const float *__restrict__ in, float *__restrict__ out, const int seg_rows, const int nstrips, const int nsegs,
+             const uint8_t *__restrict__ fin, uint8_t *__restrict__ fout)
 {
     constexpr int HL = SEP2_HL, S = 2 * R + 1, OUTW = 128 - 4 * HL;
+    static_assert(OUTW == 7 * PHFLAG_COLS && 2 * 8 == PHFLAG_COLS, "a strip is seven blocks, a block eight lanes");
     const int lane = threadIdx.x & 63, wave = threadIdx.x >> 6;
     const int e = blockIdx.y, W = p.W, H = p.H;
     const int unit = blockIdx.x * 4 + wave, strip = unit % nstrips, segi = unit / nstrips;
+    const int x_lo = segi * seg_rows, x_hi = min(x_lo + seg_rows, W), nrows = x_hi - x_lo;
+    const int nby = phflag_nby(H), obr0 = x_lo / PHFLAG_ROWS, obc0 = strip * (OUTW / PHFLAG_COLS);
+    const int onbc = min(OUTW / PHFLAG_COLS, nby - obc0);
+    const size_t fenv = (size_t)e * ((size_t)phflag_nbx(W) * nby);
+    uint8_t f = 0;
+    if constexpr (FL) {
+        const int br0 = max(x_lo - R, 0) / PHFLAG_ROWS, nbr = (min(x_hi + R, W) - 1) / PHFLAG_ROWS - br0 + 1;
+        const int bc0 = max(strip * OUTW - R, 0) / PHFLAG_COLS;
+        const int nbc = (min(strip * OUTW + OUTW + R, H) - 1) / PHFLAG_COLS - bc0 + 1;
+        const int fr = lane / 9, fc = lane - 9 * fr;
+        if (segi < nsegs && fr < nbr && fc < nbc) f = fin[fenv + (size_t)(br0 + fr) * nby + (bc0 + fc)];
+    }
     __shared__ float taps[4 * S];
     if (threadIdx.x < 2 * S) {
         taps[threadIdx.x] = p.fsep_u[threadIdx.x];
@@ -384,6 +398,26 @@
     const uint32_t *walls = p.s.walls_bits + (size_t)e * p.words;
     const bool clip = p.has_max_val && p.N > 0;
     const float thr = (float)p.threshold, mx = (float)p.max_val;
+    if constexpr (FL) {
+        if (__ballot(f != 0) == 0ull) {
+            const int onbr = (x_hi - 1) / PHFLAG_ROWS - obr0 + 1;
+            const int orw = lane / 7, ocl = lane - 7 * orw;
+            const bool mine = orw < onbr && ocl < onbc;
+            const size_t fi = fenv + (size_t)(obr0 + orw) * nby + (obc0 + ocl);
+            const uint8_t fo = mine ? fout[fi] : (uint8_t)0;
+            unsigned long long stale = __ballot(fo != 0);
+            if (fo != 0) fout[fi] = 0;
+            while (stale) {
+                const int l = __builtin_ctzll(stale);
+                stale &= stale - 1;
+                const int x = (obr0 + l / 7) * PHFLAG_ROWS + (lane >> 3), yb = (obc0 + l % 7) * PHFLAG_COLS + 2 * (lane & 7);
+                if (x < x_hi && yb < H)
+                    store_stream(reinterpret_cast<float4 *>(dst + ((size_t)x * H + yb) * 2), make_float4(0.0f, 0.0f, 0.0f, 0.0f));
+            }
+            return;
+        }
+    }
+    uint32_t live = 0;
     float uh[S], ul[S], vh[S], vl[S];
 #pragma unroll
     for (int a = 0; a < S; ++a) {
@@ -399,7 +433,6 @@
     v2f acc[S][2];
 #pragma unroll
     for (int j = 0; j < S; ++j) acc[j][0] = acc[j][1] = (v2f)(0.0f);
-    const int x_lo = segi * seg_rows, x_hi = min(x_lo + seg_rows, W), nrows = x_hi - x_lo;
     const int x0 = x_lo - R;
     float4 nv[S];
     uint32_t nword[S], ncell[S];
@@ -464,9 +497,19 @@
                         if (clip) r[c] = fminf(r[c], mx);
                     }
                     store_stream(reinterpret_cast<float4 *>(dst + ((size_t)x * H + y) * 2), make_float4(r[0], r[1], r[2], r[3]));
+                    if constexpr (FL) {
+                        const uint32_t bits = (__float_as_uint(r[0]) | __float_as_uint(r[1])) | (__float_as_uint(r[2]) | __float_as_uint(r[3]));
+                        live |= min(bits, 1u) << (io >> 3);
+                    }
                 }
                 acc[slot][0] = acc[slot][1] = (v2f)(0.0f);
             }
+        }
+    }
+    if constexpr (FL) {
+        for (int b = 0; b * PHFLAG_ROWS < nrows; ++b) {
+            const unsigned long long nz = __ballot(((live >> b) & 1u) != 0);
+            if (lane < onbc) fout[fenv + (size_t)(obr0 + b) * nby + (obc0 + lane)] = ((nz >> (HL + 8 * lane)) & 0xFFull) != 0 ? 1 : 0;
         }
     }
 #undef FMA2
@@ -476,7 +519,7 @@
 }
 
 template <int C>
-static hipError_t launch_sweep_c(const KP &p, int cur, hipStream_t st)
+static hipError_t launch_sweep_c(const KP &p, int cur, hipStream_t st, bool skip)
 {
     const float *in = p.s.phero[cur];
     float *out = p.s.phero[cur ^ 1];
@@ -506,8 +549,15 @@
                 const int outw = 128 - 4 * SEP2_HL;
                 const int strips2 = (p.H + outw - 1) / outw;
                 const dim3 grid2((strips2 * nsegs + 3) / 4, p.E);
-                if (fr == 2) hipLaunchKernelGGL((k_sweep_sep2<2>), grid2, dim3(256), 0, st, p, in, out, seg_rows, strips2, nsegs);
-                else hipLaunchKernelGGL((k_sweep_sep2<3>), grid2, dim3(256), 0, st, p, in, out, seg_rows, strips2, nsegs);
+                const bool fl = skip && p.blk_flags[0] && p.blk_flags[1] && (nsegs == 1 || seg_rows % PHFLAG_ROWS == 0) &&
+                                seg_rows <= 4 * PHFLAG_ROWS;
+                if (skip && !fl) return hipErrorInvalidValue;
+                const uint8_t *fin = fl ? p.blk_flags[cur] : nullptr;
+                uint8_t *fout = fl ? p.blk_flags[cur ^ 1] : nullptr;
+#define SEP2_GO(RR, FLV) hipLaunchKernelGGL((k_sweep_sep2<RR, FLV>), grid2, dim3(256), 0, st, p, in, out, seg_rows, strips2, nsegs, fin, fout)
+                if (fr == 2) { if (fl) SEP2_GO(2, true); else SEP2_GO(2, false); }
+                else { if (fl) SEP2_GO(3, true); else SEP2_GO(3, false); }
+#undef SEP2_GO
                 return hipGetLastError();
             }
         }
@@ -526,13 +576,18 @@
     return hipGetLastError();
 }
 
-hipError_t antsrl_launch_sweep(const KP &p, int cur, hipStream_t st)
+bool antsrl_sweep_has_flags(const KP &p)
+{
+    return !p.scaled && p.C == 2 && (p.H & 1) == 0 && p.filter_radius >= 2 && p.filter_sep;
+}
+
+hipError_t antsrl_launch_sweep(const KP &p, int cur, hipStream_t st, bool skip)
 {
     switch (p.C) {
-    case 1: return launch_sweep_c<1>(p, cur, st);
-    case 2: return launch_sweep_c<2>(p, cur, st);
-    case 3: return launch_sweep_c<3>(p, cur, st);
-    case 4: return launch_sweep_c<4>(p, cur, st);
+    case 1: return launch_sweep_c<1>(p, cur, st, false);
+    case 2: return launch_sweep_c<2>(p, cur, st, skip);
+    case 3: return launch_sweep_c<3>(p, cur, st, false);
+    case 4: return launch_sweep_c<4>(p, cur, st, false);
     default: return hipErrorInvalidValue;
     }
 }
diff --git a/antsrl_amd/csrc/antsrl_update_env.h b/antsrl_amd/csrc/antsrl_update_env.h
--- a/antsrl_amd/csrc/antsrl_update_env.h
+++ b/antsrl_amd/csrc/antsrl_update_env.h
@@ -151,14 +151,19 @@
         const uint32_t cell = prec_xy(p, (int)p.s.x[eN + i], (int)p.s.y[eN + i]);
         if (lww_winner(hkeys, hvals, (uint32_t)p.HT - 1, cell) == (uint32_t)i) {
             if (!p.scaled) {
+                bool dep = false;
                 for (int c = 0; c < C; ++c) {
                     const float a = p.s.activation[(eN + i) * C + c];
                     if (a != 0.0f) {
                         float v = out[(size_t)cell * PS + c] + a;
                         if (p.has_max_val) v = fminf(v, (float)p.max_val);
                         out[(size_t)cell * PS + c] = v;
+                        dep = true;
                     }
                 }
+                uint8_t *fl = p.blk_flags[out_buf];
+                if (dep && fl)
+                    fl[(size_t)e * (phflag_nbx(W) * phflag_nby(H)) + phflag_slot((int)p.s.x[eN + i], (int)p.s.y[eN + i], H)] = 1;
             } else {
                 const bool on_wall = test_bit(walls, cell_id);
                 bool wrote = false;
diff --git a/antsrl_amd/csrc/antsrl_update_one.h b/antsrl_amd/csrc/antsrl_update_one.h
--- a/antsrl_amd/csrc/antsrl_update_one.h
+++ b/antsrl_amd/csrc/antsrl_update_one.h
@@ -196,13 +196,19 @@
         if (fw && winner) fw->m |= UMFWD_WIN;
         if (winner) {
             if (!p.scaled) {
+                bool dep = false;
 #pragma unroll
                 for (int c = 0; c < C; ++c) {
                     if (act[c] != 0.0f) {
                         float v = pold[c] + act[c];
                         if (p.has_max_val) v = fminf(v, (float)p.max_val);
                         out[(size_t)cell * PS + c] = v;
+                        dep = true;
                     }
+                }
+                if constexpr (!fw_rec) {
+                    uint8_t *fl = p.blk_flags[out_buf];
+                    if (dep && fl) fl[(size_t)e * (phflag_nbx(W) * phflag_nby(H)) + phflag_slot((int)x, (int)y, H)] = 1;
                 }
             } else {
                 bool on_wall;
diff --git a/include/antsrl.h b/include/antsrl.h
--- a/include/antsrl.h
+++ b/include/antsrl.h
@@ -187,11 +187,15 @@
     ANTSRL_Q_PERCEIVE_RUN = 4,
     ANTSRL_Q_TIMESTEP = 5,
     ANTSRL_Q_DEFERRED_UPDATE = 6,
+    ANTSRL_Q_SWEEP_FLAGS = 7,
     ANTSRL_Q_COUNT_
 };
 int antsrl_query(const AntsHandle *h, int what, long long *value);
 
 int antsrl_bench_copy(void *dst, const void *src, size_t bytes, void *stream);
+
+int antsrl_set_sweep_skip(AntsHandle *h, int on);
+int antsrl_read_sweep_flags(AntsHandle *h, int which, uint8_t *flags, float *cells, void *stream);
 
 #define ANTSRL_MEM_PIECE_BYTES ((size_t)16 << 20)
 int antsrl_mem_alloc(size_t bytes, int device, void **ptr);
diff --git a/profiles/sweep_skip_probe.py b/profiles/sweep_skip_probe.py
--- /dev/null
+++ b/profiles/sweep_skip_probe.py
@@ -0,0 +1,116 @@
+import argparse
+import json
+import os
+import sys
+
+import numpy as np
+
+ROOT = os.path.dirname(os.path.dirname(os.path.abspath(__file__)))
+sys.path.insert(0, ROOT)
+
+STEPS, DROP = 20, 2
+
+
+def shares(cfg, f_in, f_out):
+    W, H, R = cfg.w, cfg.h, cfg.filter_radius
+    seg, ow = min(W, 32), 112
+    nsegs, nstrips = (W + seg - 1) // seg, (H + ow - 1) // ow
+    skipped = filled = blocks = 0
+    for s in range(nsegs):
+        x_lo, x_hi = s * seg, min(s * seg + seg, W)
+        r0, r1 = max(x_lo - R, 0) // 8, (min(x_hi + R, W) - 1) // 8
+        for k in range(nstrips):
+            y_lo, y_hi = k * ow, min(k * ow + ow, H)
+            c0, c1 = max(y_lo - R, 0) // 16, (min(y_lo + ow + R, H) - 1) // 16
+            skip = ~f_in[:, r0:r1 + 1, c0:c1 + 1].any(axis=(1, 2))
+            own = f_out[:, x_lo // 8:(x_hi - 1) // 8 + 1, y_lo // 16:(y_hi - 1) // 16 + 1]
+            skipped += int(skip.sum())
+            filled += int(own[skip].sum())
+            blocks += own[0].size * own.shape[0]
+    units = nsegs * nstrips * f_in.shape[0]
+    return dict(units=units, units_skipped_share=skipped / units, blocks=blocks, blocks_zero_filled_share=filled / blocks,
+                blocks_flagged_share=float(f_in.mean()))
+
+
+def main():
+    ap = argparse.ArgumentParser()
+    ap.add_argument("--out", default=None)
+    ap.add_argument("--ages", default="150,400,800,1200,1800")
+    ap.add_argument("--envs", type=int, default=1024)
+    args = ap.parse_args()
+    import torch
+    import bench
+    from antsrl_amd import config as cm
+    from antsrl_amd._lib import HipEvents
+    from antsrl_amd.batched import BatchedAntsEnv
+    from antsrl_amd.synth import synth_init
+
+    dev = torch.device("cuda", 0)
+    W_ = bench.CONFIGS["c4"]
+    E = args.envs
+    ax = np.arange(-3, 4)
+    g = np.exp(-(ax[:, None] ** 2 + ax[None, :] ** 2) / 4.5)
+    cfg = cm.make_cfg(E, W_["N"], W_["W"], W_["H"], n_rocks=W_["R"], deposit_strength=256.0, max_time=1 << 30,
+                      filt=g / g.sum() * (1 - 0.001), n_envs_total=E)
+    env = BatchedAntsEnv(cfg, dev)
+    assert env.query(cm.Q_SWEEP_FLAGS) == 1 and env.query(cm.Q_DEFERRED_UPDATE) == 1
+    env.reset(synth_init(cfg, seed=1234))
+    RING = 8
+    gen = torch.Generator(device=dev)
+    gen.manual_seed(99)
+    rot = torch.randint(-1, 2, (RING, E, cfg.n_ants), generator=gen, device=dev, dtype=torch.int8)
+    ph = torch.randint(0, 3, (RING, E, cfg.n_ants), generator=gen, device=dev, dtype=torch.int8)
+    NEV = cm.TIMING_EVENTS
+    evs = HipEvents(NEV * STEPS)
+    t = 0
+
+    def step():
+        nonlocal t
+        env.step_update(rot[t % RING], ph[t % RING], None)
+        t += 1
+
+    def timed():
+        for _ in range(DROP):
+            step()
+        torch.cuda.synchronize(dev)
+        sweep = []
+        e0, e1 = torch.cuda.Event(enable_timing=True), torch.cuda.Event(enable_timing=True)
+        e0.record()
+        for k in range(STEPS):
+            env.set_timing_events([evs.ev[NEV * k + i].value for i in range(NEV)])
+            step()
+        e1.record()
+        e1.synchronize()
+        for k in range(STEPS):
+            sweep.append(evs.elapsed_ms(NEV * k + 3, NEV * k + 4))
+        return float(np.median(sweep)), e0.elapsed_time(e1) / STEPS
+
+    rows = []
+    for age in [int(a) for a in args.ages.split(",")]:
+        while t < age:
+            step()
+        f_in = env.read_sweep_flags(0).cpu().numpy()
+        f_out = env.read_sweep_flags(1).cpu().numpy()
+        row = dict(age=t, **shares(cfg, f_in, f_out))
+        row["sweep_ms_skip_on"], row["step_ms_skip_on"] = timed()
+        env.set_sweep_skip(False)
+        row["sweep_ms_skip_off"], row["step_ms_skip_off"] = timed()
+        env.set_sweep_skip(True)
+        for _ in range(DROP):
+            step()
+        rows.append(row)
+        print(json.dumps(row), file=sys.stderr)
+    evs.destroy()
+    out = dict(config="c4: %d envs x %d ants, %dx%d, separable radius-3 filter (bench.py's inputs)" % (E, cfg.n_ants, cfg.w, cfg.h),
+               device=torch.cuda.get_device_name(0), device_unique_id=bench.device_identity(torch, 0),
+               steps_per_figure=STEPS, sweep_ms="median of the HIP-event interval [3] -> [4] of antsrl_set_timing_events (events on every "
+               "step: the step_ms figures carry their stream idle time, the same in both arms)", by_age=rows)
+    line = json.dumps(out, indent=1)
+    if args.out:
+        os.makedirs(os.path.dirname(os.path.abspath(args.out)), exist_ok=True)
+        open(args.out, "w").write(line + "\n")
+    print(line)
+
+
+if __name__ == "__main__":
+    main()
```
